# tonyzyl/ladcast

Measured on AMD Instinct MI355X. Metric: ensemble-member-steps/sec, higher is better.
Workload: dtype f32

## Files before the change

### include/ladcast_hip.h

```cpp
#ifndef LADCAST_HIP_H
#define LADCAST_HIP_H

#ifdef __cplusplus
extern "C" {
#endif

#define LDC_ABI_VERSION 5

#define LDC_OK 0
#define LDC_ERR_ARG (-1)
#define LDC_ERR_ALIGN (-2)
#define LDC_ERR_UNSUPPORTED (-3)

enum ldc_act { LDC_ACT_NONE = 0, LDC_ACT_SILU = 1, LDC_ACT_GELU_TANH = 2, LDC_ACT_RELU = 3 };
#define LDC_ACT_IN_TIMESTEP_SINCOS 16

int ldc_abi_version(void);
const char* ldc_build_arch(void);

typedef struct ldc_gemm_desc {
  int M, N, K, batch;
  int lda, ldw, ldc, ldr;
  long long a_bs, c_bs, r_bs;
  int gate_bs;
  int act;
  int flags;
  int reserved;
} ldc_gemm_desc;
#define LDC_GEMM_A_SPLIT 1
#define LDC_GEMM_C_SPLIT 2
#define LDC_GEMM_BF16_1TERM 4
#define LDC_GEMM_F32_REGSTAGE 8
#define LDC_FMT_F32 0
#define LDC_FMT_SPLIT 1
#define LDC_FMT_BF16 2
int ldc_sizeof_gemm_desc(void);
int ldc_gemm_bias_act(const float* A, const float* W, const float* bias, const float* gate,
                      const float* R, float* C, const ldc_gemm_desc* d, void* stream);

#define LDC_GEMM_MAX_PROBLEMS 4
typedef struct ldc_gemm_problem {
  const float* A;
  const float* W;
  const float* bias;
  const float* gate;
  const float* R;
  float* C;
  ldc_gemm_desc d;
} ldc_gemm_problem;
int ldc_sizeof_gemm_problem(void);
long long ldc_gemm_grouped_workspace_bytes(void);
int ldc_gemm_grouped_workspace_init(void* workspace, long long workspace_bytes, void* stream);
int ldc_gemm_grouped(const ldc_gemm_problem* problems, int n, void* workspace, long long workspace_bytes,
                     void* stream);

int ldc_gemm_grouped_bf16x3(const ldc_gemm_problem* problems, int n, void* workspace, long long workspace_bytes,
                            void* stream);
int ldc_pack_weight_bf16x2(const float* W, void* out, int N, int K, int ldw, void* stream);
int ldc_pack_weight_bf16(const float* W, void* out, int N, int K, int ldw, void* stream);

int ldc_linear_small(const float* x, int x_rows, const float* W, const float* bias,
                     const float* add, int add_rows, float* y, int rows, int N, int K,
                     int act_in, int act_out, void* stream);

int ldc_linear_small_mod(const float* x, int x_rows, const float* W, const float* bias, const float* add, int add_rows,
                         const float* mod, int mod_rows, float* y, int rows, int N, int K, int act_in, int act_out,
                         void* stream);

#define LDC_LINEAR_SMALL_MAX_GROUPED 4
typedef struct ldc_linear_small_problem {
  const float* x;
  const float* W;
  const float* bias;
  const float* add;
  float* y;
  int x_rows, add_rows, rows, N, K, act_in, act_out, reserved;
} ldc_linear_small_problem;
int ldc_linear_small_grouped(const ldc_linear_small_problem* problems, int n, void* stream);

int ldc_attn_fwd(const float* Q, const float* K, const float* V, float* O, int B, int S, int H,
                 int ld_qkv, long long qkv_bs, int ldo, long long o_bs, const float* key_bias, void* stream);
long long ldc_attn_fwd_workspace_bytes(void);
int ldc_attn_fwd_ws(const float* Q, const float* K, const float* V, float* O, int B, int S, int H, int ld_qkv, long long qkv_bs,
                    int ldo, long long o_bs, const float* key_bias, void* workspace, long long workspace_bytes, void* stream);
int ldc_attn_fwd_qrows(const float* Q, const float* K, const float* V, float* O, int B, int S, int Sq, int H, int ld_qkv,
                       long long qkv_bs, int ldo, long long o_bs, const float* key_bias, void* stream);
int ldc_attn_fwd_ws_qrows(const float* Q, const float* K, const float* V, float* O, int B, int S, int Sq, int H, int ld_qkv,
                          long long qkv_bs, int ldo, long long o_bs, const float* key_bias, void* workspace, long long workspace_bytes,
                          void* stream);

#define LDC_ATTN_OUT_SPLIT 1
#define LDC_ATTN_BF16_1TERM 2
#define LDC_ATTN_OUT_BF16 4

typedef struct ldc_qkv_epilogue {
  const float* wq;
  const float* wk;
  const float* rope;
  const float* reserved;
  float eps, qscale;
  int heads, rope_row0;
} ldc_qkv_epilogue;
int ldc_sizeof_qkv_epilogue(void);
int ldc_gemm_grouped_bf16x3_qkv(const ldc_gemm_problem* problems, const ldc_qkv_epilogue* epi, int n, void* workspace,
                                long long workspace_bytes, void* stream);
int ldc_gemm_grouped_qkv_f32(const ldc_gemm_problem* problems, const ldc_qkv_epilogue* epi, int n, void* workspace,
                             long long workspace_bytes, void* stream);
int ldc_attn_qkv_prepare_split(float* Q, float* K, float* V, int B, int S, int H, int ld_qkv, long long qkv_bs, int split_row,
                               const float* wq0, const float* wk0, const float* cos0, const float* sin0, const float* wq1,
                               const float* wk1, const float* cos1, const float* sin1, float eps, void* stream);
long long ldc_attn_fwd_split_workspace_bytes(int B, int S, int H);
long long ldc_attn_fwd_split_workspace_max_bytes(void);
int ldc_attn_fwd_split(const float* Q, const float* K, const float* V, float* O, int B, int S, int H, int ld_qkv,
                       long long qkv_bs, int ldo, long long o_bs, const float* key_bias, int flags, void* workspace,
                       long long workspace_bytes, void* stream);
long long ldc_attn_fwd_split_qrows_workspace_bytes(int B, int S, int Sq, int H);
int ldc_attn_fwd_split_qrows(const float* Q, const float* K, const float* V, float* O, int B, int S, int Sq, int H, int ld_qkv,
                             long long qkv_bs, int ldo, long long o_bs, const float* key_bias, int flags, void* workspace,
                             long long workspace_bytes, void* stream);

int ldc_qk_rmsnorm_rope(float* q, float* k, int B, int row0, int rows, int H, int ld, long long bs,
                        const float* wq, const float* wk, float eps, const float* cos_tab,
                        const float* sin_tab, void* stream);

int ldc_layernorm_mod(const float* x, float* y, int B, int rows, int D, int ldx, long long x_bs,
                      int ldy, long long y_bs, const float* scale, const float* shift, int mod_bs,
                      int mode, float eps, int out_split, void* stream);
int ldc_layernorm_mod2(const float* x, float* y, int B, int rows, int D, int ldx, long long x_bs,
                       int ldy, long long y_bs, const float* scale, const float* shift, int split_row,
                       const float* scale2, const float* shift2, int mod_bs, int mode, float eps,
                       int out_split, void* stream);

int ldc_mean_rows(const float* x, float* y, int B, int rows, int D, int ldx, long long x_bs, void* stream);
int ldc_mean_rows_split(const float* x, float* y, float* x_split, int B, int rows, int D, int ldx,
                        long long x_bs, int lds, long long s_bs, int fmt , void* stream);

int ldc_gate_residual(const float* resid, const float* y, const float* gate, float* out, int B,
                      int rows, int D, int ld_res, long long res_bs, int ld_y, long long y_bs,
                      int gate_bs, void* stream);
int ldc_gate_residual_layernorm(float* resid, const float* y, const float* gate, float* out, int B, int rows, int D, int ld_res,
                                long long res_bs, int ld_y, long long y_bs, int gate_bs, int ld_out, long long out_bs,
                                const float* weight, const float* bias, float eps, int out_split, void* stream);

int ldc_chan_to_token(const float* in, float* out, int B, int C, int N, int ldo, int fill_cols, void* stream);
int ldc_chan_to_token_split(const float* in, float* out, int B, int C, int N, int ldo, int fill_cols,
                            int out_split, void* stream);
int ldc_token_to_chan(const float* in, float* out, int B, int C, int N, int ldi, void* stream);

int ldc_timestep_embedding(const float* t, float* out, int n, void* stream);

int ldc_temb_modulate(float* temb, const float* te, int B, int D, int te_rows, void* stream);

int ldc_chan_affine(const float* x, float* y, const float* mean, const float* std_, float target_std,
                    long long outer, int C, long long inner, int inverse, void* stream);

int ldc_edm_scale_f64_to_f32(const double* x, double c_in, float* out, long long n, void* stream);
int ldc_edm_init_state(const float* noise, double sigma0, double* x, long long n, void* stream);
int ldc_edm_churn(const double* x_cur, const double* noise, double coef, double* x_hat, long long n, void* stream);
int ldc_edm_euler(const double* x_hat, const float* F, double c_skip, double c_out, double t_hat,
                  double dt, double* x_next, double* d_cur, long long n, void* stream);
int ldc_edm_heun(const double* x_hat, double* x_next, const float* F, const double* d_cur,
                 double c_skip, double c_out, double t_next, double dt, long long n, void* stream);
int ldc_f64_to_f32(const double* x, float* y, long long n, void* stream);
int ldc_dpm_step(const float* sample, const float* F, const float* m1, float* x0, float* prev,
                 float c_skip, float c_out, float a, float b, float inv_r0, int order, long long n,
                 void* stream);
int ldc_ddim_step(const float* sample, const float* F, const float* noise, float* x0, float* prev, float sqrt_alpha_t,
                  float sqrt_beta_t, float sqrt_alpha_prev, float dir_coef, float std_dev, float clip_range,
                  int prediction_type, int use_clipped_model_output, long long n, void* stream);
int ldc_ddpm_step(const float* sample, const float* F, const float* noise, float* x0, float* prev, float sqrt_alpha_t,
                  float sqrt_beta_t, float x0_coef, float sample_coef, float std_dev, float clip_range, int prediction_type,
                  long long n, void* stream);
int ldc_scale_f32(const float* x, float s, float* y, long long n, void* stream);
int ldc_axpby_f32(const float* x, float a, const float* y, float b, float* out, long long n, void* stream);

int ldc_edm_noise_inputs(const float* clean, const float* noise, const float* sigma, const float* c_in, float* noisy,
                         float* x_in, int B, long long n_per_sample, void* stream);
int ldc_edm_denoise(const float* noisy, const float* F, const float* c_skip, const float* c_out, float* denoised, int B,
                    int C, int T, int plane, int noisy_frames, int f_frames, int denoised_frames, void* stream);
int ldc_edm_denoise_loss(const float* noisy, const float* F, const float* target, const float* c_skip, const float* c_out,
                         const float* weight, const float* lat_weight, float* table, float* denoised, int B, int C, int T,
                         int H, int W, void* stream);

int ldc_sphere_conv_nhwc(const float* X, const float* Wt, const float* bias, const float* R, float* Y, int B,
                         int H, int W, int cin, int ldx, int cout, int ldy, int ldr, int ksize, int act,
                         void* stream);
int ldc_sphere_dwconv_nhwc(const float* x, const float* wt, const float* bias, float* y, int B, int H, int W,
                           int C, int ldx, int ldy, int ksize, int glu, void* stream);
int ldc_grouped_conv1x1_nhwc(const float* x, const float* wt, float* y, long long M, int groups, int ldx, int ldy,
                             void* stream);
int ldc_relu_linear_attn_nhwc(const float* qkv, float* y, int B, int P, int groups, int ldq, int ldy, float eps,
                              void* workspace, long long workspace_bytes, void* stream);
long long ldc_relu_linear_attn_workspace_bytes(int B, int P, int groups);
int ldc_rmsnorm_rows(const float* x, const float* w, const float* b, const float* resid, float* y, long long rows,
                     int C, int ldx, int ldr, int ldy, float eps, int act, void* stream);
int ldc_pixel_unshuffle_shortcut(const float* cv, const float* x, float* y, int B, int H2, int W2, int cout, int cin,
                                 void* stream);
int ldc_pixel_shuffle_shortcut(const float* cv, const float* x, float* y, int B, int H, int W, int cout, int cin,
                               void* stream);
int ldc_chan_regroup(const float* x, float* y, long long M, int cin, int cout, void* stream);

int ldc_sphere_conv_nhwc_split(const float* X, const void* Wp, const float* bias, const float* R, float* Y, int B, int H, int W,
                               int cin, int ldx, int cout, int ldy, int ldr, int ksize, int act, int in_fmt, int out_fmt,
                               void* workspace, long long workspace_bytes, void* stream);
int ldc_sphere_conv_plan(int B, int H, int W, int cin, int cout, int ksize, int in_fmt, int* tile_rows, int* tile_w);
int ldc_rmsnorm_rows_split(const float* x, const float* w, const float* b, const float* resid, float* y, float* ys, long long rows,
                           int C, int ldx, int ldr, int ldy, int lds, int fmt, float eps, int act, void* stream);
int ldc_pixel_unshuffle_shortcut_split(const float* cv, const float* x, float* y, float* ys, int B, int H2, int W2, int cout,
                                       int cin, int lds, int fmt, void* stream);
int ldc_pixel_shuffle_shortcut_split(const float* cv, const float* x, float* y, float* ys, int B, int H, int W, int cout, int cin,
                                     int lds, int fmt, void* stream);
int ldc_upsample_nearest2x_rows(const float* x, float* y, float* ys, int B, int H, int W, int C, int ldx, int ldy, int lds, int fmt, void* stream);
int ldc_pixel_shuffle_to_chan(const float* cv, float* out, int B, int H, int W, int cout, int keep, void* stream);
int ldc_split_rows(const float* x, float* ys, long long rows, int C, int ldx, int lds, int fmt, void* stream);
int ldc_sphere_dwconv_nhwc_fmt(const float* x, const float* wt, const float* bias, float* y, int B, int H, int W, int C, int ldx,
                               int ldy, int ksize, int glu, int out_fmt, void* stream);
int ldc_relu_linear_attn_nhwc_fmt(const float* qkv, float* y, int B, int P, int groups, int ldq, int ldy, float eps, int out_fmt,
                                  void* workspace, long long workspace_bytes, void* stream);

long long ldc_ensemble_scores_workspace_bytes(int C, int H, int W);
int ldc_ensemble_scores(const float* forecast, long long member_stride, long long channel_stride,
                        const float* truth, long long truth_channel_stride, const float* clim,
                        long long clim_channel_stride, const float* lat_weight, int M, int C, int H, int W,
                        int nan_channel, float* out, float* skill_map, float* spread_map, void* workspace,
                        long long workspace_bytes, void* stream);
long long ldc_rollout_scores_workspace_bytes(int C, int L, int H, int W);
int ldc_rollout_scores(const float* forecast, long long member_stride, long long lead_stride, long long channel_stride,
                       const float* mean, const float* std_, float target_std, const float* truth, long long truth_slot_stride,
                       long long truth_channel_stride, const int* truth_slot, const float* clim, long long clim_slot_stride,
                       long long clim_channel_stride, const int* clim_slot, const float* lat_weight, int M, int C, int L, int H,
                       int W, int nan_channel, float* out, int L_total, int l_off, void* workspace, long long workspace_bytes,
                       void* stream);
long long ldc_validation_scores_workspace_bytes(int C, int L, int H, int W);
int ldc_validation_scores(const float* forecast, long long member_stride, long long lead_stride, long long channel_stride,
                          const float* mean, const float* std_, float target_std, const float* truth, long long truth_slot_stride,
                          long long truth_channel_stride, const int* truth_slot, const float* lat_weight, int M, int C, int L, int H,
                          int W, float* out, int L_total, int l_off, void* workspace, long long workspace_bytes, void* stream);
long long ldc_rollout_reliability_workspace_bytes(int M, int C, int L, int H, int W);
int ldc_rollout_reliability(const float* forecast, long long member_stride, long long lead_stride, long long channel_stride,
                            const float* mean, const float* std_, float target_std, const float* truth, long long truth_slot_stride,
                            long long truth_channel_stride, const int* truth_slot, const float* lat_weight, int M, int C, int L, int H,
                            int W, int nan_channel, float* out, int* hist_count, float* hist_weight, int* n_invalid, int L_total,
                            int l_off, void* workspace, long long workspace_bytes, void* stream);
long long ldc_rollout_spectrum_workspace_bytes(int M, int C, int L, int H, int W);
int ldc_rollout_spectrum(const float* forecast, long long member_stride, long long lead_stride, long long channel_stride,
                         const float* mean, const float* std_, float target_std, const float* truth, long long truth_slot_stride,
                         long long truth_channel_stride, const int* truth_slot, const float* row_weight, int M, int C, int L, int H,
                         int W, float* out, int* n_invalid, int L_total, int l_off, void* workspace, long long workspace_bytes,
                         void* stream);
#define LDC_PRODUCTS_MAX_QUANTILES 16
#define LDC_PRODUCTS_MAX_THRESHOLDS 8
typedef struct ldc_products_desc {
  int n_quant;
  int n_thr;
  int q_lo[LDC_PRODUCTS_MAX_QUANTILES];
  float q_t[LDC_PRODUCTS_MAX_QUANTILES];
  int thr_dir[LDC_PRODUCTS_MAX_THRESHOLDS];
} ldc_products_desc;
int ldc_sizeof_products_desc(void);
int ldc_rollout_products(const float* forecast, long long member_stride, long long lead_stride, long long channel_stride,
// ... 54 lines not shown
```

### ladcast_amd/csrc/gemm_bf16x3_v3.hip

```cpp
#include <math.h>
#include <stdio.h>
#include <stdlib.h>

#include "common.h"

namespace {

#include "gemm_v3_common.inc"
#include "gemm_v3_kstep_f32.inc"

struct SKArgs {
  DevProblem pr[MAXP];
  int np;
  int G;
  long long U;
  long long tiles;
  float* ws;
  unsigned* counters;
  unsigned upg, urem;
};

__device__ __forceinline__ long long range_start(long long g, const SKArgs& a) {
  const unsigned gu = static_cast<unsigned>(g);
  return static_cast<long long>(gu * a.upg + (gu < a.urem ? gu : a.urem));
}

__device__ __forceinline__ int find_problem_by_unit(const SKArgs& a, long long u) {
  int pi = 0;
#pragma unroll
  for (int k = 1; k < MAXP; ++k)
    if (k < a.np && u >= a.pr[k].unit0) pi = k;
  return pi;
}

#ifdef LDC_GEMM_STAMPS
#define LDC_STAMP(i)                                                                                        \
  if (threadIdx.x == 0)                                                                                     \
    reinterpret_cast<unsigned long long*>(a.counters)[65536 + blockIdx.x * 16 + (i)] = __builtin_amdgcn_s_memrealtime();
#define LDC_STAMP_CLK(i)                                                                                    \
  if (threadIdx.x == 0)                                                                                     \
    reinterpret_cast<unsigned long long*>(a.counters)[65536 + blockIdx.x * 16 + (i)] = __builtin_amdgcn_s_memtime();
#else
#define LDC_STAMP(i)
#define LDC_STAMP_CLK(i)
#endif

template <int BM, int TERMS, bool CONV = false>
__global__ __launch_bounds__(512) void gemm_bf16x3_v3_kernel(SKArgs a) {
  constexpr int CPK = TERMS == 1 ? 2 * BK : BK;
  constexpr int RT = BM / 128;
  constexpr int NACC = RT * 8;
  constexpr int STAGE_B = (BM + BN) * ROW_B;
  constexpr int SLOT_FLOATS = BM * BN;
  constexpr int NAI = BM / 64;
  constexpr int ND = NAI + 2;
  constexpr int NDH = ND / 2;
  extern __shared__ __attribute__((aligned(16))) unsigned char smem[];
  const int wave = __builtin_amdgcn_readfirstlane(static_cast<int>(threadIdx.x) >> 6);
  LDC_STAMP(0)
  int seg_ = 0;
  (void)seg_;
  int g;
  {
    const int bid = blockIdx.x, G = a.G;
    const int q = G >> 3, r = G & 7, xcd = bid & 7;
    g = (xcd < r ? xcd * (q + 1) : r * (q + 1) + (xcd - r) * q) + (bid >> 3);
  }
  auto uniform64 = [](long long v) {
    const unsigned lo = __builtin_amdgcn_readfirstlane(static_cast<unsigned>(v));
    const unsigned hi = __builtin_amdgcn_readfirstlane(static_cast<unsigned>(static_cast<unsigned long long>(v) >> 32));
    return static_cast<long long>((static_cast<unsigned long long>(hi) << 32) | lo);
  };
  const long long u_begin = uniform64(range_start(g, a));
  const long long u_end = uniform64(range_start(g + 1, a));
  const unsigned smem_lds = lds_addr(smem);

  struct Seg {
    int pi, tile, k0, k1, b, bm, bn;
  };
  auto decode = [&](long long u_) {
    Seg sg;
    sg.pi = find_problem_by_unit(a, u_);
    const DevProblem& Q = a.pr[sg.pi];
    const unsigned local = static_cast<unsigned>(u_ - Q.unit0), kt_u = static_cast<unsigned>(Q.kt);
    sg.tile = __builtin_amdgcn_readfirstlane(static_cast<int>(local / kt_u));
    sg.k0 = static_cast<int>(local - static_cast<unsigned>(sg.tile) * kt_u);
    const long long left = u_end - u_;
    sg.k1 = (Q.kt - sg.k0 <= left) ? Q.kt : sg.k0 + static_cast<int>(left);
    const unsigned per_b = static_cast<unsigned>(Q.tm * Q.tn), tile_u = static_cast<unsigned>(sg.tile);
    const unsigned b_ = tile_u / per_b;
    const unsigned t_in = tile_u - b_ * per_b;
    const unsigned strip = static_cast<unsigned>(Q.rm * Q.tn);
    const unsigned sr = t_in / strip;
    const unsigned r_in = t_in - sr * strip;
    const int rest = Q.tm - static_cast<int>(sr) * Q.rm;
    const unsigned h_sr = static_cast<unsigned>(rest < Q.rm ? rest : Q.rm);
    const unsigned bn_ = r_in / h_sr;
    sg.b = __builtin_amdgcn_readfirstlane(static_cast<int>(b_));
    sg.bn = __builtin_amdgcn_readfirstlane(static_cast<int>(bn_));
    sg.bm = __builtin_amdgcn_readfirstlane(static_cast<int>(sr) * Q.rm + static_cast<int>(r_in - bn_ * h_sr));
    return sg;
  };
  auto prefetch_next = [&](const Seg& sg) __attribute__((always_inline)) {
    const DevProblem& Q = a.pr[sg.pi];
    const int ln = fresh_lane();
    const int lr_ = ln >> 3, lp_ = ln & 7;
    const float* __restrict__ An = Q.A + static_cast<long long>(sg.b) * Q.d.a_bs;
    const long long wrb = static_cast<long long>(Q.d.K) * (TERMS == 1 ? 2 : 4);
    unsigned char* dump = smem + NSTAGE * STAGE_B + wave * 1024;
#pragma unroll
    for (int j = 0; j < 2; ++j) {
      const bool live = sg.k0 + j < sg.k1;
      const long long koff = static_cast<long long>(live ? sg.k0 + j : sg.k1 - 1) * (BK * 4);
      unsigned char* sA = smem + j * STAGE_B;
      unsigned char* sW = sA + BM * ROW_B;
#pragma unroll
      for (int i = 0; i < NAI; ++i) {
        const int r = 8 * (wave + 8 * i) + lr_;
        int gm = sg.bm * BM + r;
        gm = gm < Q.d.M ? gm : Q.d.M - 1;
        dma16(reinterpret_cast<const unsigned char*>(An + static_cast<long long>(gm) * Q.d.lda) + ((lp_ ^ swz(r)) << 4) + koff,
              live ? sA + (wave + 8 * i) * 1024 : dump);
      }
#pragma unroll
      for (int i = 0; i < 2; ++i) {
        const int r = 8 * (wave + 8 * i) + lr_;
        int gn = sg.bn * BN + r;
        gn = gn < Q.d.N ? gn : Q.d.N - 1;
        dma16(Q.W + static_cast<long long>(gn) * wrb + ((lp_ ^ swz(r)) << 4) + koff, live ? sW + (wave + 8 * (i)) * 1024 : dump);
      }
    }
  };
  long long u = u_begin;
  Seg cur{};
  if (u < u_end) cur = decode(u);
  bool prefetched = false;
  while (u < u_end) {
    const int pi = cur.pi;
    const DevProblem& P = a.pr[pi];
    const int tile = cur.tile, k0 = cur.k0, k1 = cur.k1, b = cur.b, bm = cur.bm, bn = cur.bn;
    const int lane = fresh_lane();
    const int fr = lane & 15;
    const int kg = lane >> 4;
    const int lr = lane >> 3, lp = lane & 7;
    const unsigned f_r = swz(fr);
    const unsigned off_hi = fr * ROW_B + (((2 * kg) ^ f_r) << 4);
    const unsigned off_lo = fr * ROW_B + (((2 * kg + 1) ^ f_r) << 4);
    const unsigned a_hi = smem_lds + (16 * RT * wave) * ROW_B + off_hi;
    const unsigned a_lo = smem_lds + (16 * RT * wave) * ROW_B + off_lo;
    const unsigned w_hi = smem_lds + BM * ROW_B + off_hi;
    const unsigned w_lo = smem_lds + BM * ROW_B + off_lo;
    const int M = P.d.M, N = P.d.N, K = P.d.K;
    const bool wave_rows = bm * BM + 16 * RT * wave < M;
    const float* __restrict__ A = P.A + static_cast<long long>(b) * P.d.a_bs;
    const int lda = P.d.lda;
    const long long w_row_bytes = static_cast<long long>(K) * (TERMS == 1 ? 2 : 4);

#ifdef LDC_GEMM_STAMPS_PROLOGUE
    if (seg_ == 0) { LDC_STAMP(9) }
#endif
    const unsigned char* a_src[NAI];
    const unsigned char* w_src[2];
    int pix_b[NAI], pix_hw[NAI];
    const int cslot = lp ^ swz(8 * (wave & 1) + lr);
    auto conv_tap_base = [&](int i, int tap) {
      const int ky = tap / P.ks, kx = tap - ky * P.ks;
      const int src = pix_b[i] + ldc_sphere_src_pixel(pix_hw[i] >> 16, pix_hw[i] & 0xffff, ky, kx, P.cH, P.cW, P.ks);
      return reinterpret_cast<const unsigned char*>(A + static_cast<long long>(src) * lda) + (cslot << 4);
    };
#pragma unroll
    for (int i = 0; i < NAI; ++i) {
      const int r = 8 * (wave + 8 * i) + lr;
      int gm = bm * BM + r;
      gm = gm < M ? gm : M - 1;
      if constexpr (CONV) {
        const int hw = P.cH * P.cW;
        const int bimg = gm / hw;
        const int rem = gm - bimg * hw;
        const int h = rem / P.cW;
        pix_b[i] = bimg * hw;
        pix_hw[i] = (h << 16) | (rem - h * P.cW);
        a_src[i] = conv_tap_base(i, k0 >> P.kshift);
      } else {
        a_src[i] = reinterpret_cast<const unsigned char*>(A + static_cast<long long>(gm) * lda) + ((lp ^ swz(r)) << 4);
      }
    }
#pragma unroll
    for (int i = 0; i < 2; ++i) {
      const int r = 8 * (wave + 8 * i) + lr;
      int gn = bn * BN + r;
      gn = gn < N ? gn : N - 1;
      w_src[i] = P.W + static_cast<long long>(gn) * w_row_bytes + ((lp ^ swz(r)) << 4);
    }
    auto issue_one = [&](int kt_, int stage, int i) {
      const bool live = kt_ < k1;
      unsigned char* sA = smem + stage * STAGE_B;
      unsigned char* sW = sA + BM * ROW_B;
      unsigned char* dump = smem + NSTAGE * STAGE_B + wave * 1024;
      const int kt = live ? kt_ : k1 - 1;
      const long long koff = static_cast<long long>(kt) * (BK * 4);
#ifdef LDC_GEMM_DIAG_NODMA
      if (kt >= 0) return;
#endif
      if (i < NAI) {
        if constexpr (CONV) {
          const int chunk = kt & ((1 << P.kshift) - 1);
          if (chunk == 0) a_src[i] = conv_tap_base(i, kt >> P.kshift);
          const unsigned char* src = a_src[i] + chunk * (BK * 4);
          if (chunk * CPK + CPK > P.cin) {
            if (chunk * CPK + (TERMS == 0 ? 4 * cslot : 8 * (TERMS == 3 ? (cslot >> 1) : cslot)) >= P.cin) src = P.zero16;
          }
          dma16(src, live ? sA + (wave + 8 * i) * 1024 : dump);
        } else {
          dma16(a_src[i] + koff, live ? sA + (wave + 8 * i) * 1024 : dump);
        }
      } else {
        dma16(w_src[i - NAI] + koff, live ? sW + (wave + 8 * (i - NAI)) * 1024 : dump);
      }
    };

    f32x4 acc[NACC];
#pragma unroll
    for (int i = 0; i < NACC; ++i) acc[i] = f32x4{0.f, 0.f, 0.f, 0.f};

    i32x4v wh0, wl0, wh1, wl1, wh2, wl2, wh3, wl3;
    i32x4v ah0[RT], al0[RT], ah1[RT], al1[RT];

#define LDC_SB __builtin_amdgcn_sched_barrier(0)
#define LDC_RD_W(WH, WL, SBH, SBL, CT)                                           \
  {                                                                              \
    LDC_DS_READ(WH, SBH, (CT) * (16 * ROW_B));                                   \
    LDC_DS_READ(WL, SBL, (CT) * (16 * ROW_B));                                   \
  }
#define LDC_RD_A(AH, AL, SBH, SBL)                                               \
  {                                                                              \
    LDC_DS_READ(AH[0], SBH, 0);                                                  \
    LDC_DS_READ(AL[0], SBL, 0);                                                  \
    if constexpr (RT == 2) {                                                     \
      LDC_DS_READ(AH[RT - 1], SBH, 16 * ROW_B);                                  \
      LDC_DS_READ(AL[RT - 1], SBL, 16 * ROW_B);                                  \
    }                                                                            \
  }
#define LDC_MM(ACC, WF, AF)                                                                                  \
  ACC = __builtin_amdgcn_mfma_f32_16x16x32_bf16(__builtin_bit_cast(bf16x8, WF), __builtin_bit_cast(bf16x8, AF), ACC, 0, 0, 0); \
  LDC_SB;
#define LDC_MMF(ACC, WF, AF, J)                                                                               \
  ACC = __builtin_amdgcn_mfma_f32_16x16x4f32(__int_as_float(WF[J]), __int_as_float(AF[J]), ACC, 0, 0, 0);     \
  LDC_SB;
#define LDC_CT(CT, WH, WL, AH, AL)                                               \
  if (wave_rows) {                                                               \
    if constexpr (TERMS == 0) {                                                  \
      _Pragma("unroll") for (int j_ = 0; j_ < 4; ++j_) {                         \
        LDC_MMF(acc[(CT)], WH, AH[0], j_)                                        \
        if constexpr (RT == 2) {                                                 \
          LDC_MMF(acc[8 + (CT)], WH, AH[RT - 1], j_)                             \
        }                                                                        \
      }                                                                          \
      _Pragma("unroll") for (int j_ = 0; j_ < 4; ++j_) {                         \
        LDC_MMF(acc[(CT)], WL, AL[0], j_)                                        \
        if constexpr (RT == 2) {                                                 \
          LDC_MMF(acc[8 + (CT)], WL, AL[RT - 1], j_)                             \
        }                                                                        \
      }                                                                          \
    } else if constexpr (TERMS == 1) {                                           \
      LDC_MM(acc[(CT)], WH, AH[0])                                               \
      if constexpr (RT == 2) {                                                   \
        LDC_MM(acc[8 + (CT)], WH, AH[RT - 1])                                    \
      }                                                                          \
      LDC_MM(acc[(CT)], WL, AL[0])                                               \
      if constexpr (RT == 2) {                                                   \
        LDC_MM(acc[8 + (CT)], WL, AL[RT - 1])                                    \
      }                                                                          \
    } else if constexpr (RT == 2) {                                              \
      LDC_MM(acc[(CT)], WH, AL[0])                                               \
      LDC_MM(acc[8 + (CT)], WH, AL[RT - 1])                                      \
      LDC_MM(acc[(CT)], WL, AH[0])                                               \
      LDC_MM(acc[8 + (CT)], WL, AH[RT - 1])                                      \
      LDC_MM(acc[(CT)], WH, AH[0])                                               \
      LDC_MM(acc[8 + (CT)], WH, AH[RT - 1])                                      \
    } else {                                                                     \
      LDC_MM(acc[(CT)], WH, AL[0])                                               \
      LDC_MM(acc[(CT)], WL, AH[0])                                               \
      LDC_MM(acc[(CT)], WH, AH[0])                                               \
    }                                                                            \
  }
#ifdef LDC_GEMM_DIAG_NOBARRIER
#define LDC_KSTEP_BARRIER
#else
#define LDC_KSTEP_BARRIER __builtin_amdgcn_s_barrier();
#endif
#define LDC_WAIT(N, X, Y)                                                        \
  asm volatile("s_waitcnt lgkmcnt(6)" : "+v"(X), "+v"(Y));                       \
  LDC_SB;
#define LDC_KSTEP(AH, AL, AHN, ALN)                                                                          \
  {                                                                                                          \
    const int st1 = st == NSTAGE - 1 ? 0 : st + 1;                                                           \
    const int st2 = st1 == NSTAGE - 1 ? 0 : st1 + 1;                                                         \
    const unsigned sb1 = st1 * STAGE_B;                                                                      \
    const unsigned wch = w_hi + sb, wcl = w_lo + sb, wnh = w_hi + sb1, wnl = w_lo + sb1;                     \
    const unsigned anh = a_hi + sb1, anl = a_lo + sb1;                                                       \
    constexpr bool dma2 = true;              \
    constexpr bool dma3 = true;  \
        \
    if constexpr (RT == 2) {                                                                                 \
      asm volatile("s_waitcnt lgkmcnt(6)" : "+v"(AH[0]), "+v"(AL[0]), "+v"(AH[1]), "+v"(AL[1]), "+v"(wh0), "+v"(wl0)); \
    } else {                                                                                                 \
      asm volatile("s_waitcnt lgkmcnt(6)" : "+v"(AH[0]), "+v"(AL[0]), "+v"(wh0), "+v"(wl0));                 \
    }                                                                                                        \
    LDC_SB;                                                                                                  \
    LDC_CT(0, wh0, wl0, AH, AL)                                                                              \
    LDC_RD_W(wh0, wl0, wch, wcl, 4)                                                                                \
    if (dma2) issue_one(kt + 2, st2, NDH + 0);                                                               \
    LDC_WAIT(6, wh1, wl1)                                                                                    \
    LDC_CT(1, wh1, wl1, AH, AL)                                                                              \
    LDC_RD_W(wh1, wl1, wch, wcl, 5)                                                                                \
    if (dma2) issue_one(kt + 2, st2, NDH + 1);                                                               \
    LDC_WAIT(6, wh2, wl2)                                                                                    \
    LDC_CT(2, wh2, wl2, AH, AL)                                                                              \
    LDC_RD_W(wh2, wl2, wch, wcl, 6)                                                                                \
    if constexpr (NDH == 3) {                                                                                \
      if (dma2) issue_one(kt + 2, st2, NDH + 2);                                                             \
    }                                                                                                        \
    LDC_WAIT(6, wh3, wl3)                                                                                    \
    LDC_CT(3, wh3, wl3, AH, AL)                                                                              \
    LDC_RD_W(wh3, wl3, wch, wcl, 7)                                                                          \
    LDC_WAIT(6, wh0, wl0)                                                                                    \
    LDC_CT(4, wh0, wl0, AH, AL)                                                                              \
                                                                         \
    asm volatile("s_waitcnt lgkmcnt(0)" : "+v"(wh1), "+v"(wl1), "+v"(wh2), "+v"(wl2), "+v"(wh3), "+v"(wl3)); \
    if constexpr (ND == 6) {                                                                                 \
      asm volatile("s_waitcnt vmcnt(6)" ::: "memory");                                                       \
    } else {                                                                                                 \
      asm volatile("s_waitcnt vmcnt(4)" ::: "memory");                                                       \
    }                                                                                                        \
    LDC_KSTEP_BARRIER                                                                                        \
    LDC_SB;                                                                                                  \
                          \
    LDC_RD_A(AHN, ALN, anh, anl)                                                                             \
    LDC_RD_W(wh0, wl0, wnh, wnl, 0)                                                                          \
    if (dma3) issue_one(kt + 3, st, 0);                                                                      \
    LDC_SB;                                                                                                  \
    LDC_CT(5, wh1, wl1, AH, AL)                                                                              \
    LDC_RD_W(wh1, wl1, wnh, wnl, 1)                                                                               \
    if (dma3) issue_one(kt + 3, st, 1);                                                                      \
    LDC_SB;                                                                                                  \
    LDC_CT(6, wh2, wl2, AH, AL)                                                                              \
    LDC_RD_W(wh2, wl2, wnh, wnl, 2)                                                                               \
    if constexpr (NDH == 3) {                                                                                \
      if (dma3) issue_one(kt + 3, st, 2);                                                                    \
    }                                                                                                        \
    LDC_SB;                                                                                                  \
    LDC_CT(7, wh3, wl3, AH, AL)                                                                              \
    LDC_RD_W(wh3, wl3, wnh, wnl, 3)                                                                               \
    LDC_SB;                                                                                                  \
    st = st1;                                                                                                \
    sb = sb1;                                                                                                \
  }

#define LDC_MM_ON(ACC, WF, AF, J) LDC_MMF(ACC, WF, AF, J)
#define LDC_MM_OFF(ACC, WF, AF, J)
#if defined(LDC_AB_BUILD) && defined(LDC_GEMM_F32_NO_PAIRS)
  constexpr bool PAIRED = false;
#else
  constexpr bool PAIRED = TERMS == 0 && RT == 1;
#endif

#ifdef LDC_GEMM_STAMPS_PROLOGUE
    if (seg_ == 0) { LDC_STAMP(10) }
#endif
    if (!prefetched) {
#pragma unroll
      for (int i = 0; i < ND; ++i) issue_one(k0, 0, i);
#pragma unroll
      for (int i = 0; i < ND; ++i) issue_one(k0 + 1, 1, i);
    }
#ifdef LDC_GEMM_STAMPS_PROLOGUE
    if (seg_ == 0) { LDC_STAMP(11) }
#endif
    const long long u_next = u + (k1 - k0);
    Seg nxt = cur;
    if (u_next < u_end) nxt = decode(u_next);
    if constexpr (ND == 6) {
      asm volatile("s_waitcnt vmcnt(6)" ::: "memory");
    } else {
      asm volatile("s_waitcnt vmcnt(4)" ::: "memory");
    }
    __builtin_amdgcn_s_barrier();
    LDC_STAMP(1 + 4 * seg_)
    if (seg_ == 0) { LDC_STAMP_CLK(13) }
    if constexpr (PAIRED) {
      LDC_KSTEP_Q_PROLOGUE(ah0, al0)
    } else {
      LDC_RD_A(ah0, al0, a_hi, a_lo)
      LDC_RD_W(wh0, wl0, w_hi, w_lo, 0)
      LDC_RD_W(wh1, wl1, w_hi, w_lo, 1)
      LDC_RD_W(wh2, wl2, w_hi, w_lo, 2)
      LDC_RD_W(wh3, wl3, w_hi, w_lo, 3)
    }
#pragma unroll
    for (int i = 0; i < NDH; ++i) issue_one(k0 + 2, 2, i);
    LDC_SB;

    unsigned sb = 0;
    int st = 0;
    if constexpr (PAIRED) {
      static_assert(!PAIRED || ND == 4, "the interleaved k-step is written for the 128-row tile's 4 DMA pieces");
      if (wave_rows) {
        for (int kt = k0; kt < k1; ++kt) {
          LDC_KSTEP_Q(ah0, al0, ah1, al1, LDC_MM_ON)
          ++kt;
          if (kt >= k1) break;
          LDC_KSTEP_Q(ah1, al1, ah0, al0, LDC_MM_ON)
        }
      } else {
        for (int kt = k0; kt < k1; ++kt) {
          LDC_KSTEP_Q(ah0, al0, ah1, al1, LDC_MM_OFF)
          ++kt;
          if (kt >= k1) break;
          LDC_KSTEP_Q(ah1, al1, ah0, al0, LDC_MM_OFF)
        }
      }
    } else {
      for (int kt = k0; kt < k1; ++kt) {
        LDC_KSTEP(ah0, al0, ah1, al1)
        ++kt;
        if (kt >= k1) break;
        LDC_KSTEP(ah1, al1, ah0, al0)
      }
    }
    asm volatile("s_waitcnt lgkmcnt(0)" : "+v"(wh0), "+v"(wl0), "+v"(wh1), "+v"(wl1), "+v"(wh2), "+v"(wl2), "+v"(wh3), "+v"(wl3));
#pragma unroll
    for (int rt = 0; rt < RT; ++rt) asm volatile("" : "+v"(ah0[rt]), "+v"(al0[rt]), "+v"(ah1[rt]), "+v"(al1[rt]));
#undef LDC_KSTEP
#undef LDC_MM_ON
#undef LDC_MM_OFF
#undef LDC_WAIT
#undef LDC_CT
#undef LDC_MMF
#undef LDC_MM
#undef LDC_RD_A
#undef LDC_RD_W
#undef LDC_SB
    __builtin_amdgcn_s_barrier();
    prefetched = false;
    if constexpr (!CONV && TERMS == 0) {
#if !defined(LDC_GEMM_DIAG_NODMA) && !defined(LDC_GEMM_NO_PREFETCH)
      if (u_next < u_end) {
        prefetch_next(nxt);
        prefetched = true;
      }
#endif
    }
    if (seg_ == 0) { LDC_STAMP_CLK(14) }
    LDC_STAMP(2 + 4 * seg_)

    if (k0 == 0 && k1 == P.kt) {
      tile_epilogue<BM, !CONV, LinearRows<BM>, true, TERMS == 0>(P, b, bm, bn, acc, wave, lane);
    } else {
      const int lane_h = fresh_lane();
      float* slot = a.ws + (static_cast<long long>(2 * g) + (k0 > 0 ? 0 : 1)) * SLOT_FLOATS + lane_h;
#pragma unroll
      for (int i = 0; i < NACC; ++i)
#pragma unroll
        for (int r = 0; r < 4; ++r)
          __hip_atomic_store(slot + ((wave * NACC + i) * 4 + r) * 64, acc[i][r], __ATOMIC_RELAXED, __HIP_MEMORY_SCOPE_AGENT);
      asm volatile("s_waitcnt vmcnt(0)" ::: "memory");
      __builtin_amdgcn_s_barrier();
      const long long f = P.unit0 + static_cast<long long>(tile) * P.kt;
      const long long l = f + P.kt;
      long long g_first = g;
      while (g_first > 0 && range_start(g_first, a) > f) --g_first;
      long long g_last = g;
      while (g_last + 1 < a.G && range_start(g_last + 1, a) < l) ++g_last;
      const unsigned pieces = static_cast<unsigned>(g_last - g_first + 1);
      unsigned* cnt = a.counters + (P.tile0 + tile);
      unsigned* flag = reinterpret_cast<unsigned*>(smem + NSTAGE * STAGE_B);
      if (wave == 0 && lane_h == 0) {
        const unsigned ticket = __hip_atomic_fetch_add(cnt, 1u, __ATOMIC_RELAXED, __HIP_MEMORY_SCOPE_AGENT);
        const unsigned last = (ticket == pieces - 1) ? 1u : 0u;
        if (last) {
          __builtin_amdgcn_fence(__ATOMIC_ACQUIRE, "agent");
          asm volatile("s_waitcnt vmcnt(0)" ::: "memory");
          __hip_atomic_store(cnt, 0u, __ATOMIC_RELAXED, __HIP_MEMORY_SCOPE_AGENT);
        }
        *flag = last;
      }
      __syncthreads();
      LDC_STAMP(3 + 4 * seg_)
      const unsigned is_last = *flag;
      __syncthreads();
      if (is_last) {
#pragma unroll
        for (int i = 0; i < NACC; ++i) acc[i] = f32x4{0.f, 0.f, 0.f, 0.f};
        for (long long gp = g_first; gp <= g_last; ++gp) {
          const long long s = range_start(gp, a);
          const float* sl = a.ws + (2 * gp + (s > f ? 0 : 1)) * SLOT_FLOATS;
#pragma unroll
          for (int i = 0; i < NACC; ++i) {
#pragma unroll
            for (int r = 0; r < 4; ++r) acc[i][r] += sl[((wave * NACC + i) * 4 + r) * 64 + lane_h];
          }
        }
        tile_epilogue<BM, !CONV, LinearRows<BM>, true, TERMS == 0>(P, b, bm, bn, acc, wave, lane);
      }
    }
    u = u_next;
    cur = nxt;
    LDC_STAMP(4 + 4 * seg_)
#ifdef LDC_GEMM_STAMPS
    if (seg_ < 2) ++seg_;
#endif
  }
  LDC_STAMP(15)
}

struct ConvParams {
  int H, W, cin, ks, kshift;
};

constexpr int LDC_SPLIT_GROUP = -100;

template <int BM, int TERMS, bool CONV = false>
int launch_v3(const ldc_gemm_problem* problems, const ldc_qkv_epilogue* epi, int n, void* workspace, long long workspace_bytes,
              void* stream, const ConvParams* cp = nullptr, bool may_split_group = false) {
  constexpr int SLOT_FLOATS = BM * BN;
  constexpr int STAGE_B = (BM + BN) * ROW_B;
  constexpr int CUS = 256;
  SKArgs a{};
  a.np = n;
  long long U = 0, tiles = 0;
  for (int i = 0; i < n; ++i) {
    const ldc_gemm_problem& q = problems[i];
    LDC_CHECK_PTR(q.A);
    LDC_CHECK_PTR(q.W);
    LDC_CHECK_PTR(q.C);
    const ldc_gemm_desc& d = q.d;
    if (d.M <= 0 || d.N <= 0 || d.K <= 0 || d.batch <= 0) return LDC_ERR_ARG;
    if (d.K % (TERMS == 1 ? 2 * BK : BK)) return LDC_ERR_UNSUPPORTED;
    if constexpr (TERMS == 0) {
      if (d.flags != 0 || d.ldw != d.K) return LDC_ERR_UNSUPPORTED;
    } else {
      if (!(d.flags & LDC_GEMM_A_SPLIT)) return LDC_ERR_UNSUPPORTED;
    }
    LDC_CHECK_ALIGN16(q.A);
    LDC_CHECK_ALIGN16(q.W);
    if constexpr (TERMS == 0) {
      if ((d.lda & 3) || (d.a_bs & 3)) return LDC_ERR_UNSUPPORTED;
    } else {
      if ((d.lda & 7) || (d.a_bs & 7) || (reinterpret_cast<unsigned long long>(q.A) & 31ull)) return LDC_ERR_ALIGN;
    }
    if (d.act < LDC_ACT_NONE || d.act > LDC_ACT_RELU) return LDC_ERR_UNSUPPORTED;
    DevProblem& P = a.pr[i];
    P.A = q.A;
    P.W = reinterpret_cast<const unsigned char*>(q.W);
    P.bias = q.bias;
    P.gate = q.gate;
    P.R = q.R;
    P.C = q.C;
    P.d = d;
    {
      auto al16 = [](const void* q_) { return (reinterpret_cast<unsigned long long>(q_) & 15ull) == 0; };
      bool v4 = (d.N % 4 == 0) && (d.ldc % 4 == 0) && (d.c_bs % 4 == 0) && al16(q.C);
      if (q.bias) v4 = v4 && al16(q.bias);
      if (q.gate) v4 = v4 && al16(q.gate) && (d.gate_bs % 4 == 0);
      if (q.R) v4 = v4 && al16(q.R) && (d.ldr % 4 == 0) && (d.r_bs % 4 == 0);
      P.vec4 = v4 ? 1 : 0;
      P.c_split = (TERMS != 0 && (d.flags & LDC_GEMM_C_SPLIT)) ? (TERMS == 3 ? LDC_FMT_SPLIT : LDC_FMT_BF16) : 0;
      if (P.c_split && !(v4 && d.ldc % 8 == 0 && d.ldc >= ((d.N + 7) & ~7) &&
                         d.c_bs % 8 == 0 && (reinterpret_cast<unsigned long long>(q.C) & 31ull) == 0))
        return LDC_ERR_ALIGN;
    }
    if (epi != nullptr && epi[i].heads > 0) {
      const ldc_qkv_epilogue& e = epi[i];
      auto al16 = [](const void* q_) { return (reinterpret_cast<unsigned long long>(q_) & 15ull) == 0; };
      if (d.N != 3 * e.heads * BN || d.act != LDC_ACT_NONE || q.gate != nullptr || q.R != nullptr) return LDC_ERR_ARG;
      if ((e.wq == nullptr) != (e.wk == nullptr) || e.reserved != nullptr || e.rope_row0 < 0) return LDC_ERR_ARG;
      if constexpr (TERMS == 0) {
        if ((d.ldc & 3) || (d.c_bs & 3) || !al16(q.C)) return LDC_ERR_ALIGN;
      } else {
        if ((d.ldc & 7) || (d.c_bs & 7) || (reinterpret_cast<unsigned long long>(q.C) & 31ull)) return LDC_ERR_ALIGN;
      }
      if (!al16(e.wq) || !al16(e.wk) || !al16(e.rope) || (q.bias && !al16(q.bias))) return LDC_ERR_ALIGN;
      P.qkv_heads = e.heads;
      P.rope_row0 = e.rope_row0;
      P.qk_w[0] = e.wq;
      P.qk_w[1] = e.wk;
      P.rope_cs = e.rope;
      P.eps = e.eps;
      P.qscale = e.qscale != 0.f ? e.qscale : 0.08838834764831845f * 1.4426950408889634f;
    }
    if constexpr (CONV) {
      P.cH = cp->H; P.cW = cp->W; P.cin = cp->cin; P.ks = cp->ks; P.kshift = cp->kshift;
      P.zero16 = static_cast<const unsigned char*>(workspace) + LDC_GEMM_COUNTER_BYTES - 64;
    }
    P.tm = ldc_cdiv(d.M, BM);
    P.tn = ldc_cdiv(d.N, BN);
    P.kt = d.K / (TERMS == 1 ? 2 * BK : BK);
    P.unit0 = U;
    P.tile0 = tiles;
    {
      P.rm = P.tm;
      const double a_bytes = CONV ? static_cast<double>(d.M) * d.lda * 4.0 : static_cast<double>(d.batch) * d.M * d.K * 4.0;
      if (a_bytes >= 48e6) {
        const double t8 = static_cast<double>(d.batch) * P.tm * P.tn / 8.0;
        const double want = sqrt(t8 * BN / BM);
        int nsr = static_cast<int>(P.tm / (want > 1.0 ? want : 1.0) + 0.5);
        if (nsr < 1) nsr = 1;
        if (nsr > P.tm) nsr = P.tm;
        P.rm = ldc_cdiv(P.tm, nsr);
      }
      if (const char* e = LDC_AB_GETENV("LDC_BF16X3_RM")) {
        const int f = atoi(e);
        if (f >= 0) P.rm = (f == 0 || f > P.tm) ? P.tm : f;
      }
    }
    const long long t = static_cast<long long>(d.batch) * P.tm * P.tn;
    tiles += t;
    U += t * P.kt;
  }
  if (tiles > LDC_GEMM_COUNTER_BYTES / 4 - 16) return LDC_ERR_UNSUPPORTED;
  const long long slot_bytes = SLOT_FLOATS * static_cast<long long>(sizeof(float));
  long long G = CUS;
  {
    bool same_kt = true;
    for (int i = 1; i < n; ++i) same_kt = same_kt && (a.pr[i].kt == a.pr[0].kt);
    long long best = 0;
    if (same_kt) {
      const int kt = a.pr[0].kt;
      double best_score = 0.0;
      for (int sfac = 1; sfac <= 8; ++sfac) {
        if (kt % sfac || (sfac > 1 && kt / sfac < 8)) continue;
        const long long items = tiles * sfac;
        long long gd = items < CUS ? items : CUS;
        while (gd > 1 && items % gd) --gd;
        const double score = static_cast<double>(gd) * (1.0 - 0.02 * (sfac - 1));
        if (score > best_score) {
          best_score = score;
          best = gd;
        }
      }
    }
    long long few = 0;
    if (same_kt && best < 160) {
      const int kt = a.pr[0].kt;
      for (int sfac = 8; sfac >= 2; --sfac)
        if (kt % sfac == 0 && kt / sfac >= 8 && tiles * sfac <= CUS) {
          few = tiles * sfac;
          break;
        }
    }
    if (may_split_group && TERMS != 0 && n > 1 && best < 160 && few == 0) return LDC_SPLIT_GROUP;
    if (best >= 160) {
      G = best;
    } else if (few > 0) {
      G = few;
    } else {
      const double kt_avg = static_cast<double>(U) / static_cast<double>(tiles);
      long long umin = static_cast<long long>(sqrt(kt_avg * 8.0) + 0.5);
      if (umin < 1) umin = 1;
      const long long gmax = U / umin > 0 ? U / umin : 1;
      if (gmax < G) G = gmax;
    }
  }
  if constexpr (TERMS == 0) {
    if (U >= 4 * CUS) G = CUS;
  }
  static const char* const force_g = LDC_AB_GETENV("LDC_BF16X3_G");
  if (force_g) {
    const long long g_ = atoll(force_g);
    if (g_ > 0 && g_ <= CUS) G = g_;
  }
  if (U < G) G = U;
  if (workspace == nullptr) return LDC_ERR_ARG;
  if (workspace_bytes < LDC_GEMM_COUNTER_BYTES + 2 * slot_bytes) return LDC_ERR_ARG;
  {
    const long long fit = (workspace_bytes - LDC_GEMM_COUNTER_BYTES) / (2 * slot_bytes);
    if (fit < G) G = fit;
  }
  LDC_CHECK_ALIGN16(workspace);
  if (U >= (1LL << 31)) return LDC_ERR_UNSUPPORTED;
#ifdef LDC_AB_BUILD
  {
    static const bool dbg = getenv("LDC_GEMM_DEBUG_G") != nullptr;
    if (dbg)
      fprintf(stderr, "ldc_gemm cut: terms %d conv %d n %d tiles %lld kt0 %d BM %d G %lld U %lld %s\n", TERMS, int(CONV), n, tiles, a.pr[0].kt, BM, G, U,
              (U % G == 0 && (U / G) % a.pr[0].kt == 0) ? "whole tiles" : (U % G == 0 ? "equal ranges" : "UNALIGNED"));
  }
#endif
  a.G = static_cast<int>(G);
  a.U = U;
  a.upg = static_cast<unsigned>(U / G);
  a.urem = static_cast<unsigned>(U % G);
  a.tiles = tiles;
  a.ws = reinterpret_cast<float*>(static_cast<unsigned char*>(workspace) + LDC_GEMM_COUNTER_BYTES);
  a.counters = static_cast<unsigned*>(workspace);
  const size_t lds = NSTAGE * STAGE_B + 8 * 1024;
  static const bool attr_set = [&] {
    (void)hipFuncSetAttribute(reinterpret_cast<const void*>(gemm_bf16x3_v3_kernel<BM, TERMS, CONV>),
                              hipFuncAttributeMaxDynamicSharedMemorySize, static_cast<int>(lds));
    return true;
  }();
  (void)attr_set;
  hipLaunchKernelGGL((gemm_bf16x3_v3_kernel<BM, TERMS, CONV>), dim3(a.G), dim3(512), lds, static_cast<hipStream_t>(stream), a);
  return ldc_launch_status();
}

}

static int gemm_v3_dispatch(const ldc_gemm_problem* problems, const ldc_qkv_epilogue* epi, int n, void* workspace,
                            long long workspace_bytes, void* stream) {
  LDC_CHECK_PTR(problems);
  if (n <= 0 || n > MAXP) return LDC_ERR_ARG;
  long long tiles256 = 0;
  for (int i = 0; i < n; ++i) {
    const ldc_gemm_desc& d = problems[i].d;
    if (d.M <= 0 || d.N <= 0 || d.batch <= 0) return LDC_ERR_ARG;
    if (!(d.flags & LDC_GEMM_A_SPLIT)) return LDC_ERR_UNSUPPORTED;
    if (((d.flags ^ problems[0].d.flags) & LDC_GEMM_BF16_1TERM) != 0) return LDC_ERR_ARG;
    tiles256 += static_cast<long long>(d.batch) * ldc_cdiv(d.M, 256) * ldc_cdiv(d.N, BN);
  }
  static const char* const force_thr = LDC_AB_GETENV("LDC_BF16X3_SMALL_TILES");
  bool small = tiles256 < (force_thr ? atoll(force_thr) : 400);
  static const char* const force_bm = LDC_AB_GETENV("LDC_BF16X3_BM");
  if (force_bm) small = (atoi(force_bm) == 128);
  const bool one = (problems[0].d.flags & LDC_GEMM_BF16_1TERM) != 0;
  auto launch = [&](const ldc_gemm_problem* pr, const ldc_qkv_epilogue* ep, int cnt, bool sm, bool may_split) {
    if (one)
      return sm ? launch_v3<128, 1>(pr, ep, cnt, workspace, workspace_bytes, stream, nullptr, may_split)
                : launch_v3<256, 1>(pr, ep, cnt, workspace, workspace_bytes, stream, nullptr, may_split);
    return sm ? launch_v3<128, 3>(pr, ep, cnt, workspace, workspace_bytes, stream, nullptr, may_split)
              : launch_v3<256, 3>(pr, ep, cnt, workspace, workspace_bytes, stream, nullptr, may_split);
  };
  const int st = launch(problems, epi, n, small, true);
  if (st != LDC_SPLIT_GROUP) return st;
  for (int i = 0; i < n; ++i) {
    const ldc_gemm_desc& d = problems[i].d;
    bool sm = static_cast<long long>(d.batch) * ldc_cdiv(d.M, 256) * ldc_cdiv(d.N, BN) < (force_thr ? atoll(force_thr) : 400);
    if (force_bm) sm = (atoi(force_bm) == 128);
    const int sti = launch(problems + i, epi ? epi + i : nullptr, 1, sm, false);
    if (sti != LDC_OK) return sti;
  }
  return LDC_OK;
}

static int gemm_f32_ring(const ldc_gemm_problem* problems, const ldc_qkv_epilogue* epi, int n, void* workspace, long long workspace_bytes,
                         void* stream) {
  LDC_CHECK_PTR(problems);
  if (n <= 0 || n > MAXP) return LDC_ERR_ARG;
  for (int i = 0; i < n; ++i)
    if (problems[i].d.flags & LDC_GEMM_F32_REGSTAGE) return LDC_ERR_UNSUPPORTED;
  auto al16 = [](const void* q_) { return q_ != nullptr && (reinterpret_cast<unsigned long long>(q_) & 15ull) == 0; };
  if (!al16(workspace) || workspace_bytes < LDC_GEMM_COUNTER_BYTES + 2ll * 256 * BN * static_cast<long long>(sizeof(float)))
    return LDC_ERR_UNSUPPORTED;
  for (int i = 0; i < n; ++i) {
    const ldc_gemm_desc& d = problems[i].d;
    if (d.M <= 0 || d.N <= 0 || d.K <= 0 || d.batch <= 0) return LDC_ERR_ARG;
    if (!al16(problems[i].A) || !al16(problems[i].W)) return LDC_ERR_UNSUPPORTED;
  }
#ifdef LDC_AB_BUILD
  static const char* const force_bm = getenv("LDC_F32_RING_BM");
  if (force_bm && atoi(force_bm) == 256) return launch_v3<256, 0>(problems, epi, n, workspace, workspace_bytes, stream);
#endif
  return launch_v3<128, 0>(problems, epi, n, workspace, workspace_bytes, stream);
}

int ldc_gemm_grouped_f32_ring(const ldc_gemm_problem* problems, int n, void* workspace, long long workspace_bytes, void* stream) {
  return gemm_f32_ring(problems, nullptr, n, workspace, workspace_bytes, stream);
}

extern "C" int ldc_gemm_grouped_qkv_f32(const ldc_gemm_problem* problems, const ldc_qkv_epilogue* epi, int n, void* workspace,
                                        long long workspace_bytes, void* stream) {
  LDC_CHECK_PTR(epi);
  return gemm_f32_ring(problems, epi, n, workspace, workspace_bytes, stream);
}

int ldc_gemm_grouped_bf16x3_v3(const ldc_gemm_problem* problems, int n, void* workspace, long long workspace_bytes,
                               void* stream) {
  return gemm_v3_dispatch(problems, nullptr, n, workspace, workspace_bytes, stream);
}

extern "C" int ldc_gemm_grouped_bf16x3_qkv(const ldc_gemm_problem* problems, const ldc_qkv_epilogue* epi, int n, void* workspace,
                                           long long workspace_bytes, void* stream) {
  LDC_CHECK_PTR(epi);
  return gemm_v3_dispatch(problems, epi, n, workspace, workspace_bytes, stream);
}

extern "C" int ldc_sphere_conv_nhwc_split(const float* X, const void* Wp, const float* bias, const float* R, float* Y, int B, int H,
                                          int W, int cin, int ldx, int cout, int ldy, int ldr, int ksize, int act, int in_fmt,
                                          int out_fmt, void* workspace, long long workspace_bytes, void* stream) {
  LDC_CHECK_PTR(X);
  LDC_CHECK_PTR(Wp);
  LDC_CHECK_PTR(Y);
  if (B <= 0 || H <= 0 || W <= 0 || cin <= 0 || cout <= 0) return LDC_ERR_ARG;
  if (ksize != 1 && ksize != 3 && ksize != 5) return LDC_ERR_UNSUPPORTED;
  if (ksize > 1 && ((W & 1) || H < 2 || H < ksize / 2 || W / 2 < ksize / 2 || H > 32767 || W > 65535)) return LDC_ERR_UNSUPPORTED;
  if (in_fmt != LDC_FMT_SPLIT && in_fmt != LDC_FMT_BF16 && in_fmt != LDC_FMT_F32) return LDC_ERR_UNSUPPORTED;
  if (out_fmt != LDC_FMT_F32 && out_fmt != in_fmt) return LDC_ERR_UNSUPPORTED;
  if (in_fmt == LDC_FMT_F32) {
    if ((ldx & 3) || (cin & 3) || ldx < cin || ldy < cout) return LDC_ERR_ALIGN;
  } else if ((ldx & 7) || ldx < ((cin + 7) & ~7) || ldy < cout) {
    return LDC_ERR_ALIGN;
  }
  const long long M = static_cast<long long>(B) * H * W;
  if (M > 0x7fffffffLL) return LDC_ERR_UNSUPPORTED;
  const bool one = in_fmt == LDC_FMT_BF16;
  const int cpk = one ? 2 * BK : BK;
  ConvParams cp{H, W, cin, ksize, 0};
  int ktpt = ldc_cdiv(cin, cpk);
  while ((1 << cp.kshift) < ktpt) ++cp.kshift;
  ktpt = 1 << cp.kshift;
  ldc_gemm_problem q{};
  q.A = X;
  q.W = static_cast<const float*>(Wp);
  q.bias = bias;
  q.R = R;
  q.C = Y;
  q.d.M = static_cast<int>(M);
  q.d.N = cout;
  q.d.K = ksize * ksize * ktpt * cpk;
  q.d.batch = 1;
  q.d.lda = ldx;
  q.d.ldw = q.d.K;
  q.d.ldc = ldy;
  q.d.ldr = ldr;
  q.d.act = act;
  q.d.flags = LDC_GEMM_A_SPLIT | (out_fmt != LDC_FMT_F32 ? LDC_GEMM_C_SPLIT : 0) | (one ? LDC_GEMM_BF16_1TERM : 0);
  if (in_fmt == LDC_FMT_F32) {
    q.d.flags = 0;
    return launch_v3<128, 0, true>(&q, nullptr, 1, workspace, workspace_bytes, stream, &cp);
  }
  if (ksize == 3) {
    static const char* const halo_sw = LDC_AB_GETENV("LDC_CONV_HALO");
    if (!(halo_sw && atoi(halo_sw) == 0)) {
      if (workspace == nullptr || workspace_bytes < LDC_GEMM_COUNTER_BYTES) return LDC_ERR_ARG;
      const int hs = ldc_conv_halo_dispatch(X, Wp, bias, R, Y, B, H, W, cin, ldx, cout, ldy, ldr, act, in_fmt, out_fmt, workspace, workspace_bytes, stream);
      if (hs != LDC_ERR_UNSUPPORTED) return hs;
    }
  }
  const long long tiles256 = static_cast<long long>(ldc_cdiv(M, 256)) * ldc_cdiv(cout, BN);
  static const char* const force_thr = LDC_AB_GETENV("LDC_CONV_SMALL_TILES");
  const bool small = tiles256 < (force_thr ? atoll(force_thr) : 200);
  if (one)
    return small ? launch_v3<128, 1, true>(&q, nullptr, 1, workspace, workspace_bytes, stream, &cp)
                 : launch_v3<256, 1, true>(&q, nullptr, 1, workspace, workspace_bytes, stream, &cp);
  return small ? launch_v3<128, 3, true>(&q, nullptr, 1, workspace, workspace_bytes, stream, &cp)
               : launch_v3<256, 3, true>(&q, nullptr, 1, workspace, workspace_bytes, stream, &cp);
}
```

### ladcast_amd/csrc/gemm_streamk.hip

```cpp
#include <math.h>
#include <stdlib.h>
#include <string.h>

#include "common.h"

namespace {

constexpr int BM = 128, BN = 128, BK = 32;
constexpr int LDP = 36;
constexpr int STAGE_FLOATS = (BM + BN) * LDP;
constexpr int SLOT_FLOATS = BM * BN;
constexpr int MAXP = LDC_GEMM_MAX_PROBLEMS;

struct DevProblem {
  const float* A;
  const float* W;
  const float* bias;
  const float* gate;
  const float* R;
  float* C;
  ldc_gemm_desc d;
  int tm, tn, kt;
  long long unit0;
  long long tile0;
// ... 273 lines not shown

    const int srow0 = tid >> 2, srow1 = srow0 + 64, skc = tid & 3;
    const bool am0 = bm * BM + srow0 < M, am1 = bm * BM + srow1 < M;
    const bool wn0 = bn * BN + srow0 < N, wn1 = bn * BN + srow1 < N;
    const float* a_src0 = A + static_cast<long long>(am0 ? bm * BM + srow0 : 0) * lda + skc * 8;
    const float* a_src1 = A + static_cast<long long>(am1 ? bm * BM + srow1 : 0) * lda + skc * 8;
    const uint4* w_src0 = Wp + (static_cast<long long>(wn0 ? bn * BN + srow0 : 0) * kchunks + skc) * 2;
    const uint4* w_src1 = Wp + (static_cast<long long>(wn1 ? bn * BN + srow1 : 0) * kchunks + skc) * 2;
    float4 ra00, ra01, ra10, ra11;
    uint4 rw00, rw01, rw10, rw11;
    auto gload = [&](int kt) {
      const bool kin = kt * BK + skc * 8 < K;
      const int ko = kin ? kt * BK : 0;
      const float4* pa0 = reinterpret_cast<const float4*>(a_src0 + ko);
      const float4* pa1 = reinterpret_cast<const float4*>(a_src1 + ko);
      const uint4* pw0 = w_src0 + (ko >> 3) * 2;
      const uint4* pw1 = w_src1 + (ko >> 3) * 2;
      ra00 = pa0[0];
      ra01 = pa0[1];
      ra10 = pa1[0];
      ra11 = pa1[1];
      rw00 = pw0[0];
      rw01 = pw0[1];
      rw10 = pw1[0];
      rw11 = pw1[1];
      const unsigned m0a = (kin && am0) ? 0xffffffffu : 0u, m1a = (kin && am1) ? 0xffffffffu : 0u;
      const unsigned m0w = (kin && wn0) ? 0xffffffffu : 0u, m1w = (kin && wn1) ? 0xffffffffu : 0u;
#define LDC_MASKF4(v, m)                                 \
  v.x = __uint_as_float(__float_as_uint(v.x) & (m));     \
  v.y = __uint_as_float(__float_as_uint(v.y) & (m));     \
  v.z = __uint_as_float(__float_as_uint(v.z) & (m));     \
  v.w = __uint_as_float(__float_as_uint(v.w) & (m));
#define LDC_MASKU4(v, m) \
  v.x &= (m);            \
  v.y &= (m);            \
  v.z &= (m);            \
  v.w &= (m);
      LDC_MASKF4(ra00, m0a) LDC_MASKF4(ra01, m0a) LDC_MASKF4(ra10, m1a) LDC_MASKF4(ra11, m1a)
      LDC_MASKU4(rw00, m0w) LDC_MASKU4(rw01, m0w) LDC_MASKU4(rw10, m1w) LDC_MASKU4(rw11, m1w)
    };
    auto sstore = [&](int stage) {
      unsigned char* As = smem_b + stage * STAGE_BYTES_B;
      unsigned char* Bs = As + BM * PITCH_B;
      uint4 h, l;
      split8(ra00, ra01, h, l);
      *reinterpret_cast<uint4*>(As + srow0 * PITCH_B + skc * 16) = h;
      *reinterpret_cast<uint4*>(As + srow0 * PITCH_B + 64 + skc * 16) = l;
      split8(ra10, ra11, h, l);
      *reinterpret_cast<uint4*>(As + srow1 * PITCH_B + skc * 16) = h;
      *reinterpret_cast<uint4*>(As + srow1 * PITCH_B + 64 + skc * 16) = l;
      *reinterpret_cast<uint4*>(Bs + srow0 * PITCH_B + skc * 16) = rw00;
      *reinterpret_cast<uint4*>(Bs + srow0 * PITCH_B + 64 + skc * 16) = rw01;
      *reinterpret_cast<uint4*>(Bs + srow1 * PITCH_B + skc * 16) = rw10;
      *reinterpret_cast<uint4*>(Bs + srow1 * PITCH_B + 64 + skc * 16) = rw11;
    };

    f32x16 acc[2][2];
#pragma unroll
    for (int i = 0; i < 2; ++i)
#pragma unroll
      for (int j = 0; j < 2; ++j)
#pragma unroll
        for (int r = 0; r < 16; ++r) acc[i][j][r] = 0.f;

    gload(k0);
    sstore(0);
    __syncthreads();
    for (int kt = k0; kt < k1; ++kt) {
      const int st = (kt - k0) & 1;
      if (kt + 1 < k1) gload(kt + 1);
      const unsigned char* As = smem_b + st * STAGE_BYTES_B;
      const unsigned char* Bs = As + BM * PITCH_B;
      const unsigned char* a_base = As + (wm * 64 + frag_row) * PITCH_B + frag_h * 16;
      const unsigned char* b_base = Bs + (wn * 64 + frag_row) * PITCH_B + frag_h * 16;
#pragma unroll
      for (int s2 = 0; s2 < 2; ++s2) {
        const bf16x8 ah0 = *reinterpret_cast<const bf16x8*>(a_base + s2 * 32);
        const bf16x8 al0 = *reinterpret_cast<const bf16x8*>(a_base + 64 + s2 * 32);
        const bf16x8 ah1 = *reinterpret_cast<const bf16x8*>(a_base + 32 * PITCH_B + s2 * 32);
        const bf16x8 al1 = *reinterpret_cast<const bf16x8*>(a_base + 32 * PITCH_B + 64 + s2 * 32);
        const bf16x8 wh0 = *reinterpret_cast<const bf16x8*>(b_base + s2 * 32);
        const bf16x8 wl0 = *reinterpret_cast<const bf16x8*>(b_base + 64 + s2 * 32);
        const bf16x8 wh1 = *reinterpret_cast<const bf16x8*>(b_base + 32 * PITCH_B + s2 * 32);
        const bf16x8 wl1 = *reinterpret_cast<const bf16x8*>(b_base + 32 * PITCH_B + 64 + s2 * 32);
#define LDC_MFMA3(ACC, AH, AL, WH, WL)                                        \
  ACC = __builtin_amdgcn_mfma_f32_32x32x16_bf16(AL, WH, ACC, 0, 0, 0);        \
  ACC = __builtin_amdgcn_mfma_f32_32x32x16_bf16(AH, WL, ACC, 0, 0, 0);        \
  ACC = __builtin_amdgcn_mfma_f32_32x32x16_bf16(AH, WH, ACC, 0, 0, 0);
        LDC_MFMA3(acc[0][0], ah0, al0, wh0, wl0)
        LDC_MFMA3(acc[0][1], ah0, al0, wh1, wl1)
        LDC_MFMA3(acc[1][0], ah1, al1, wh0, wl0)
        LDC_MFMA3(acc[1][1], ah1, al1, wh1, wl1)
      }
      if (kt + 1 < k1) sstore(st ^ 1);
      __syncthreads();
    }

    if (k0 == 0 && k1 == P.kt) {
      tile_epilogue(P, b, bm, bn, acc, wm, wn, lane);
    } else {
      publish_or_reduce(a, P, g, tile, k0, b, bm, bn, acc, wave, wm, wn, lane, reinterpret_cast<unsigned*>(smem_b));
    }
    u += k1 - k0;
  }
}

__global__ __launch_bounds__(256) void pack_weight_bf16x2_kernel(const float* __restrict__ W, uint4* __restrict__ out,
                                                                 int N, int K, int ldw) {
  const long long idx = static_cast<long long>(blockIdx.x) * 256 + threadIdx.x;
  const int kchunks = K >> 3;
  if (idx >= static_cast<long long>(N) * kchunks) return;
  const int n = static_cast<int>(idx / kchunks), kc = static_cast<int>(idx - static_cast<long long>(n) * kchunks);
  const float4* src = reinterpret_cast<const float4*>(W + static_cast<long long>(n) * ldw + kc * 8);
  uint4 h, l;
  split8(src[0], src[1], h, l);
  out[idx * 2] = h;
  out[idx * 2 + 1] = l;
}

}

extern "C" int ldc_sizeof_gemm_problem(void) { return static_cast<int>(sizeof(ldc_gemm_problem)); }

extern "C" long long ldc_gemm_grouped_workspace_bytes(void) {
  return LDC_GEMM_COUNTER_BYTES + 2LL * 512 * SLOT_FLOATS * static_cast<long long>(sizeof(float));
}

extern "C" int ldc_gemm_grouped_workspace_init(void* workspace, long long workspace_bytes, void* stream) {
  LDC_CHECK_PTR(workspace);
  if (workspace_bytes < LDC_GEMM_COUNTER_BYTES) return LDC_ERR_ARG;
  hipError_t e = hipMemsetAsync(workspace, 0, LDC_GEMM_COUNTER_BYTES, static_cast<hipStream_t>(stream));
  return e == hipSuccess ? LDC_OK : -(1000 + static_cast<int>(e));
}

static int gemm_grouped_impl(const ldc_gemm_problem* problems, int n, void* workspace, long long workspace_bytes,
                             void* stream, bool split_bf16) {
  LDC_CHECK_PTR(problems);
  if (n <= 0 || n > MAXP) return LDC_ERR_ARG;
  SKArgs a{};
  a.np = n;
  long long U = 0, tiles = 0;
  for (int i = 0; i < n; ++i) {
    const ldc_gemm_problem& q = problems[i];
    LDC_CHECK_PTR(q.A);
    LDC_CHECK_PTR(q.W);
    LDC_CHECK_PTR(q.C);
    const ldc_gemm_desc& d = q.d;
    if (d.M <= 0 || d.N <= 0 || d.K <= 0 || d.batch <= 0) return LDC_ERR_ARG;
    LDC_CHECK_ALIGN16(q.A);
    LDC_CHECK_ALIGN16(q.W);
    if ((d.K & 3) || (d.lda & 3) || (d.a_bs & 3)) return LDC_ERR_ALIGN;
    if (split_bf16 ? (d.K & 7) != 0 : (d.ldw & 3) != 0) return LDC_ERR_ALIGN;
    if (d.act < LDC_ACT_NONE || d.act > LDC_ACT_RELU) return LDC_ERR_UNSUPPORTED;
    if ((d.flags & ~LDC_GEMM_F32_REGSTAGE) != 0) return LDC_ERR_UNSUPPORTED;
    DevProblem& P = a.pr[i];
    P.A = q.A;
    P.W = q.W;
    P.bias = q.bias;
    P.gate = q.gate;
    P.R = q.R;
    P.C = q.C;
    P.d = d;
    P.tm = ldc_cdiv(d.M, BM);
    P.tn = ldc_cdiv(d.N, BN);
    P.kt = ldc_cdiv(d.K, BK);
    P.unit0 = U;
    P.tile0 = tiles;
    const long long t = static_cast<long long>(d.batch) * P.tm * P.tn;
    tiles += t;
    U += t * P.kt;
  }
  if (tiles > LDC_GEMM_COUNTER_BYTES / 4 - 16) return LDC_ERR_UNSUPPORTED;
  const long long slot_bytes = SLOT_FLOATS * static_cast<long long>(sizeof(float));
  long long G = 512;
  {
    const double kt_avg = static_cast<double>(U) / static_cast<double>(tiles);
    long long umin = static_cast<long long>(sqrt(kt_avg * (split_bf16 ? 7.0 : 2.0)) + 0.5);
    if (umin < 1) umin = 1;
    const long long gmax = U / umin > 0 ? U / umin : 1;
    if (gmax < G) G = gmax;
  }
  if (U < G) G = U;
  if (workspace == nullptr || workspace_bytes < LDC_GEMM_COUNTER_BYTES + 2 * slot_bytes) return LDC_ERR_ARG;
  {
    const long long fit = (workspace_bytes - LDC_GEMM_COUNTER_BYTES) / (2 * slot_bytes);
    if (fit < G) G = fit;
  }
  LDC_CHECK_ALIGN16(workspace);
  a.G = static_cast<int>(G);
  a.U = U;
  a.tiles = tiles;
  a.ws = reinterpret_cast<float*>(static_cast<unsigned char*>(workspace) + LDC_GEMM_COUNTER_BYTES);
  a.counters = static_cast<unsigned*>(workspace);
  const size_t lds = split_bf16 ? 2 * STAGE_BYTES_B : 2 * STAGE_FLOATS * sizeof(float);
  static const bool attr_set = [&] {
    (void)hipFuncSetAttribute(reinterpret_cast<const void*>(gemm_streamk_kernel),
                              hipFuncAttributeMaxDynamicSharedMemorySize, static_cast<int>(2 * STAGE_FLOATS * sizeof(float)));
    (void)hipFuncSetAttribute(reinterpret_cast<const void*>(gemm_streamk_bf16x3_kernel),
                              hipFuncAttributeMaxDynamicSharedMemorySize, 2 * STAGE_BYTES_B);
    return true;
  }();
  (void)attr_set;
  hipStream_t s = static_cast<hipStream_t>(stream);
  if (split_bf16) hipLaunchKernelGGL(gemm_streamk_bf16x3_kernel, dim3(a.G), dim3(256), lds, s, a);
  else hipLaunchKernelGGL(gemm_streamk_kernel, dim3(a.G), dim3(256), lds, s, a);
  return ldc_launch_status();
}

int ldc_gemm_grouped_f32_ring(const ldc_gemm_problem* problems, int n, void* workspace, long long workspace_bytes,
                              void* stream);

extern "C" int ldc_gemm_grouped(const ldc_gemm_problem* problems, int n, void* workspace, long long workspace_bytes,
                                void* stream) {
  const int st = ldc_gemm_grouped_f32_ring(problems, n, workspace, workspace_bytes, stream);
  if (st != LDC_ERR_UNSUPPORTED) return st;
  return gemm_grouped_impl(problems, n, workspace, workspace_bytes, stream, false);
}

int ldc_gemm_grouped_bf16x3_v3(const ldc_gemm_problem* problems, int n, void* workspace, long long workspace_bytes,
                               void* stream);

extern "C" int ldc_gemm_grouped_bf16x3(const ldc_gemm_problem* problems, int n, void* workspace,
                                       long long workspace_bytes, void* stream) {
  int force = 0;
#ifdef LDC_AB_BUILD
  static const int force_env = [] {
    const char* e = getenv("LDC_BF16X3_KERNEL");
    return (e != nullptr && strcmp(e, "regstage") == 0) ? 1 : 0;
  }();
  force = force_env;
#endif
  if (force == 0) {
    const int st = ldc_gemm_grouped_bf16x3_v3(problems, n, workspace, workspace_bytes, stream);
    if (st != LDC_ERR_UNSUPPORTED) return st;
  }
  return gemm_grouped_impl(problems, n, workspace, workspace_bytes, stream, true);
}

namespace {
__global__ __launch_bounds__(256) void pack_weight_bf16_kernel(const float* __restrict__ W, uint2* __restrict__ out, long long N, int K4, int ldw) {
  const long long idx = static_cast<long long>(blockIdx.x) * 256 + threadIdx.x;
  if (idx >= N * K4) return;
  const long long n = idx / K4;
  const int c = static_cast<int>(idx - n * K4);
  const float4 v = reinterpret_cast<const float4*>(W + n * ldw)[c];
  out[idx] = make_uint2(ldc_pack_pair(v.x, v.y), ldc_pack_pair(v.z, v.w));
}
}

extern "C" int ldc_pack_weight_bf16(const float* W, void* out, int N, int K, int ldw, void* stream) {
  LDC_CHECK_PTR(W);
  LDC_CHECK_PTR(out);
  if (N <= 0 || K <= 0) return LDC_ERR_ARG;
  if ((K & 7) || (ldw & 3)) return LDC_ERR_ALIGN;
  LDC_CHECK_ALIGN16(W);
  LDC_CHECK_ALIGN16(out);
  const long long total = static_cast<long long>(N) * (K >> 2);
  hipLaunchKernelGGL(pack_weight_bf16_kernel, dim3(ldc_cdiv(total, 256)), dim3(256), 0, static_cast<hipStream_t>(stream), W,
                     static_cast<uint2*>(out), static_cast<long long>(N), K >> 2, ldw);
  return ldc_launch_status();
}

extern "C" int ldc_pack_weight_bf16x2(const float* W, void* out, int N, int K, int ldw, void* stream) {
  LDC_CHECK_PTR(W);
  LDC_CHECK_PTR(out);
  if (N <= 0 || K <= 0) return LDC_ERR_ARG;
  if ((K & 7) || (ldw & 3)) return LDC_ERR_ALIGN;
  LDC_CHECK_ALIGN16(W);
  LDC_CHECK_ALIGN16(out);
  const long long total = static_cast<long long>(N) * (K >> 3);
  hipLaunchKernelGGL(pack_weight_bf16x2_kernel, dim3(ldc_cdiv(total, 256)), dim3(256), 0, static_cast<hipStream_t>(stream),
                     W, static_cast<uint4*>(out), N, K, ldw);
  return ldc_launch_status();
}
```

### ladcast_amd/csrc/gemm_v3_common.inc

```
constexpr int BN = 128, BK = 32;
constexpr int ROW_B = 128;
constexpr int NSTAGE = 3;
constexpr int MAXP = LDC_GEMM_MAX_PROBLEMS;

typedef __bf16 bf16x8 __attribute__((ext_vector_type(8)));
typedef float f32x4 __attribute__((ext_vector_type(4)));
typedef int i32x4v __attribute__((ext_vector_type(4)));

template <int BM>
struct LinearRows {
  __device__ __forceinline__ int operator()(int bm, int r) const { return bm * BM + r; }
};

struct DevProblem {
  const float* A;
  const unsigned char* W;
  const float* bias;
  const float* gate;
  const float* R;
  float* C;
  ldc_gemm_desc d;
  int tm, tn, kt;
  int rm;
  long long unit0;
  long long tile0;
  int vec4;
  int c_split;
  int qkv_heads;
  int rope_row0;
  const float* qk_w[2];
  const float* rope_cs;
  float eps, qscale;
  int cH, cW, cin, ks, kshift;
  const unsigned char* zero16;
};


#ifdef LDC_GEMM_DIAG_NOLDS
#define LDC_DS_READ(dst, addr, off) asm volatile("; no read %0 %1" : "=v"(dst) : "v"(addr))
#else
#define LDC_DS_READ(dst, addr, off) asm volatile("ds_read_b128 %0, %1 offset:%2" : "=v"(dst) : "v"(addr), "n"(off))
#endif

__device__ __forceinline__ unsigned lds_addr(const void* p) {
  return static_cast<unsigned>(reinterpret_cast<unsigned long long>(p));
}
__device__ __forceinline__ void dma16(const void* gsrc, unsigned char* lds_dst_wave_base) {
  __builtin_amdgcn_global_load_lds((const __attribute__((address_space(1))) void*)gsrc,
                                   (__attribute__((address_space(3))) void*)lds_dst_wave_base, 16, 0, 0);
}
__device__ __forceinline__ int swz(int r) { return ((r >> 1) & 7) ^ ((((r >> 2) ^ (r >> 3)) & 1) << 1); }

__device__ __forceinline__ float xor16_add(float x) {
  const auto r = __builtin_amdgcn_permlane16_swap(__float_as_uint(x), __float_as_uint(x), false, false);
  return __uint_as_float(r[0]) + __uint_as_float(r[1]);
}
__device__ __forceinline__ float xor32_add(float x) {
  const auto r = __builtin_amdgcn_permlane32_swap(__float_as_uint(x), __float_as_uint(x), false, false);
  return __uint_as_float(r[0]) + __uint_as_float(r[1]);
}

__device__ __forceinline__ int fresh_lane() {
  int l;
  asm volatile("v_mbcnt_lo_u32_b32 %0, -1, 0\n\tv_mbcnt_hi_u32_b32 %0, -1, %0" : "=v"(l));
  return l;
}

template <int BM, bool F32OUT = false>
__device__ __forceinline__ void qkv_epilogue(const DevProblem& P, int b, int bm, int bn, const f32x4 (&acc)[BM / 16], int wave,
                                             int lane) {
  constexpr int RT = BM / 128;
  lane = fresh_lane();
  const int M = P.d.M;
  float* __restrict__ C = P.C + static_cast<long long>(b) * P.d.c_bs;
  const int which = bn / P.qkv_heads;
  const int nl = 4 * (lane >> 4);
  const float* __restrict__ w = which < 2 ? P.qk_w[which] : nullptr;
  const float* __restrict__ rope = which < 2 ? P.rope_cs : nullptr;
  float4 bv[8], wv[8];
  if (P.bias) {
#pragma unroll
    for (int ct = 0; ct < 8; ++ct) bv[ct] = *reinterpret_cast<const float4*>(P.bias + bn * BN + nl + 16 * ct);
  } else {
#pragma unroll
    for (int ct = 0; ct < 8; ++ct) bv[ct] = make_float4(0.f, 0.f, 0.f, 0.f);
  }
  if (w) {
#pragma unroll
    for (int ct = 0; ct < 8; ++ct) wv[ct] = *reinterpret_cast<const float4*>(w + 16 * ct + nl);
  } else {
#pragma unroll
    for (int ct = 0; ct < 8; ++ct) wv[ct] = make_float4(1.f, 1.f, 1.f, 1.f);
  }
  const float qs = which == 0 ? P.qscale : 1.f;
#pragma unroll
  for (int rt = 0; rt < RT; ++rt) {
    const int m = bm * BM + 16 * (RT * wave + rt) + (lane & 15);
#ifndef LDC_QKV_EPI_HOIST
    asm volatile("" ::: "memory");
#endif
    if (m >= M) continue;
    float4 tv[8];
    if (rope) {
      const float* __restrict__ cs = rope + static_cast<long long>(P.rope_row0 + m) * 128 + nl;
#pragma unroll
      for (int ct = 0; ct < 8; ++ct) tv[ct] = *reinterpret_cast<const float4*>(cs + 16 * ct);
    }
    float r = 1.f;
    if (w) {
      float ss = 0.f;
#pragma unroll
      for (int ct = 0; ct < 8; ++ct) {
        const f32x4 av = acc[rt * 8 + ct];
        const float a0 = av[0] + bv[ct].x, a1 = av[1] + bv[ct].y, a2 = av[2] + bv[ct].z, a3 = av[3] + bv[ct].w;
        ss += a0 * a0 + a1 * a1 + a2 * a2 + a3 * a3;
      }
      ss = xor32_add(xor16_add(ss));
      r = rsqrtf(ss * (1.0f / 128.0f) + P.eps);
    }
    unsigned char* row = reinterpret_cast<unsigned char*>(C + static_cast<long long>(m) * P.d.ldc + bn * BN);
#pragma unroll
    for (int ct = 0; ct < 8; ++ct) {
      const f32x4 av = acc[rt * 8 + ct];
      float x0 = av[0] + bv[ct].x, x1 = av[1] + bv[ct].y, x2 = av[2] + bv[ct].z, x3 = av[3] + bv[ct].w;
      if (w) {
        x0 = x0 * r * wv[ct].x; x1 = x1 * r * wv[ct].y; x2 = x2 * r * wv[ct].z; x3 = x3 * r * wv[ct].w;
      }
      if (rope) {
        const float4 t = tv[ct];
        const float o0 = x0 * t.x + (-x1) * t.y, o1 = x1 * t.x + x0 * t.y;
        const float o2 = x2 * t.z + (-x3) * t.w, o3 = x3 * t.z + x2 * t.w;
        x0 = o0; x1 = o1; x2 = o2; x3 = o3;
      }
      if (which == 0) { x0 *= qs; x1 *= qs; x2 *= qs; x3 *= qs; }
      const int n = 16 * ct + nl;
      if constexpr (F32OUT) {
        *reinterpret_cast<float4*>(reinterpret_cast<float*>(row) + n) = make_float4(x0, x1, x2, x3);
        continue;
      }
      float r0, r1, r2, r3;
      const unsigned hx = ldc_split_pair(x0, x1, r0, r1), hy = ldc_split_pair(x2, x3, r2, r3);
      const unsigned lx = ldc_pack_pair(r0, r1), ly = ldc_pack_pair(r2, r3);
      const auto sx = __builtin_amdgcn_permlane16_swap(hx, lx, false, false);
      const auto sy = __builtin_amdgcn_permlane16_swap(hy, ly, false, false);
      unsigned char* dst = which < 2 ? row + 4 * (n & ~7) + 4 * (n & 4)
                                     : row + 2 * (n & ~7) + ((n & 4) ? 256 : 0);
      *reinterpret_cast<uint4*>(dst) = make_uint4(sx[0], sy[0], sx[1], sy[1]);
    }
  }
}

template <int BM, int ACT, int FMT, class RM, bool GATE>
__device__ __forceinline__ void tile_epilogue_fast(const DevProblem& P, int b, int bm, int bn, const f32x4 (&acc)[BM / 16], int wave,
                                                   int lane, const RM& rowmap) {
  constexpr int RT = BM / 128;
  lane = fresh_lane();
  const int M = P.d.M;
  float* __restrict__ C = P.C + static_cast<long long>(b) * P.d.c_bs;
  const float* __restrict__ R = P.R ? P.R + static_cast<long long>(b) * P.d.r_bs : nullptr;
  const float* __restrict__ gate = P.gate ? P.gate + static_cast<long long>(b) * P.d.gate_bs : nullptr;
  const int n0 = bn * BN + 4 * (lane >> 4);
  float4 bv[8], gv[8];
  if (P.bias) {
#pragma unroll
    for (int ct = 0; ct < 8; ++ct) bv[ct] = *reinterpret_cast<const float4*>(P.bias + n0 + 16 * ct);
  } else {
#pragma unroll
    for (int ct = 0; ct < 8; ++ct) bv[ct] = make_float4(0.f, 0.f, 0.f, 0.f);
  }
  const bool mod = (GATE && gate != nullptr) || R != nullptr;
  if constexpr (GATE) {
    if (gate) {
#pragma unroll
      for (int ct = 0; ct < 8; ++ct) gv[ct] = *reinterpret_cast<const float4*>(gate + n0 + 16 * ct);
    } else {
#pragma unroll
// ... 151 lines not shown
```

### ladcast_amd/csrc/gemm_v3_kstep_f32.inc

```
#define LDC_KSTEP_Q(AH, AL, AHN, ALN, MM) \
  { \
    const int st1 = st == NSTAGE - 1 ? 0 : st + 1; \
    const int st2 = st1 == NSTAGE - 1 ? 0 : st1 + 1; \
    (void)st2; \
    const unsigned sb1 = st1 * STAGE_B; \
    const unsigned wch = w_hi + sb, wcl = w_lo + sb, wnh = w_hi + sb1, wnl = w_lo + sb1; \
    const unsigned anh = a_hi + sb1, anl = a_lo + sb1; \
    asm volatile("s_waitcnt lgkmcnt(2)" : "+v"(AH[0]), "+v"(AL[0]), "+v"(wh0), "+v"(wl0), "+v"(wh1), "+v"(wl1)); \
    LDC_SB; \
    MM(acc[0], wh0, AH[0], 0) \
    LDC_DS_READ(wl2, wcl, 2 * (16 * ROW_B)); \
    LDC_SB; \
    MM(acc[1], wh1, AH[0], 0) \
    MM(acc[0], wh0, AH[0], 1) \
    LDC_DS_READ(wl3, wcl, 3 * (16 * ROW_B)); \
    LDC_SB; \
    MM(acc[1], wh1, AH[0], 1) \
    MM(acc[0], wh0, AH[0], 2) \
    MM(acc[1], wh1, AH[0], 2) \
    MM(acc[0], wh0, AH[0], 3) \
    MM(acc[1], wh1, AH[0], 3) \
    MM(acc[0], wl0, AL[0], 0) \
    LDC_DS_READ(wh0, wch, 4 * (16 * ROW_B)); \
    LDC_SB; \
    MM(acc[1], wl1, AL[0], 0) \
    MM(acc[0], wl0, AL[0], 1) \
    LDC_DS_READ(wh1, wch, 5 * (16 * ROW_B)); \
    LDC_SB; \
    MM(acc[1], wl1, AL[0], 1) \
    MM(acc[0], wl0, AL[0], 2) \
    issue_one(kt + 2, st2, NDH + 0); \
    LDC_SB; \
    MM(acc[1], wl1, AL[0], 2) \
    MM(acc[0], wl0, AL[0], 3) \
    issue_one(kt + 2, st2, NDH + 1); \
    LDC_SB; \
    MM(acc[1], wl1, AL[0], 3) \
    asm volatile("s_waitcnt lgkmcnt(2)" : "+v"(wh2), "+v"(wh3), "+v"(wl2), "+v"(wl3)); \
    LDC_SB; \
    MM(acc[2], wh2, AH[0], 0) \
    LDC_DS_READ(wl0, wcl, 4 * (16 * ROW_B)); \
    LDC_SB; \
    MM(acc[3], wh3, AH[0], 0) \
    MM(acc[2], wh2, AH[0], 1) \
    LDC_DS_READ(wl1, wcl, 5 * (16 * ROW_B)); \
    LDC_SB; \
    MM(acc[3], wh3, AH[0], 1) \
    MM(acc[2], wh2, AH[0], 2) \
    MM(acc[3], wh3, AH[0], 2) \
    MM(acc[2], wh2, AH[0], 3) \
    MM(acc[3], wh3, AH[0], 3) \
    MM(acc[2], wl2, AL[0], 0) \
    LDC_DS_READ(wh2, wch, 6 * (16 * ROW_B)); \
    LDC_SB; \
    MM(acc[3], wl3, AL[0], 0) \
    MM(acc[2], wl2, AL[0], 1) \
    LDC_DS_READ(wh3, wch, 7 * (16 * ROW_B)); \
    LDC_SB; \
    MM(acc[3], wl3, AL[0], 1) \
    MM(acc[2], wl2, AL[0], 2) \
    MM(acc[3], wl3, AL[0], 2) \
    MM(acc[2], wl2, AL[0], 3) \
    MM(acc[3], wl3, AL[0], 3) \
    asm volatile("s_waitcnt lgkmcnt(2)" : "+v"(wh0), "+v"(wh1), "+v"(wl0), "+v"(wl1)); \
    LDC_SB; \
    MM(acc[4], wh0, AH[0], 0) \
    LDC_DS_READ(wl2, wcl, 6 * (16 * ROW_B)); \
    LDC_SB; \
    MM(acc[5], wh1, AH[0], 0) \
    MM(acc[4], wh0, AH[0], 1) \
    LDC_DS_READ(wl3, wcl, 7 * (16 * ROW_B)); \
    LDC_SB; \
    MM(acc[5], wh1, AH[0], 1) \
    MM(acc[4], wh0, AH[0], 2) \
    MM(acc[5], wh1, AH[0], 2) \
    MM(acc[4], wh0, AH[0], 3) \
    MM(acc[5], wh1, AH[0], 3) \
    MM(acc[4], wl0, AL[0], 0) \
    MM(acc[5], wl1, AL[0], 0) \
    MM(acc[4], wl0, AL[0], 1) \
    MM(acc[5], wl1, AL[0], 1) \
    MM(acc[4], wl0, AL[0], 2) \
    MM(acc[5], wl1, AL[0], 2) \
    MM(acc[4], wl0, AL[0], 3) \
    MM(acc[5], wl1, AL[0], 3) \
     \
    asm volatile("s_waitcnt lgkmcnt(0)" : "+v"(wh2), "+v"(wh3), "+v"(wl2), "+v"(wl3)); \
    asm volatile("s_waitcnt vmcnt(4)" ::: "memory"); \
    LDC_KSTEP_BARRIER \
    LDC_SB; \
    MM(acc[6], wh2, AH[0], 0) \
    LDC_DS_READ(AHN[0], anh, 0 * (16 * ROW_B)); \
    LDC_SB; \
    MM(acc[7], wh3, AH[0], 0) \
    LDC_DS_READ(ALN[0], anl, 0 * (16 * ROW_B)); \
    LDC_SB; \
    MM(acc[6], wh2, AH[0], 1) \
    LDC_DS_READ(wh0, wnh, 0 * (16 * ROW_B)); \
    LDC_SB; \
    MM(acc[7], wh3, AH[0], 1) \
    LDC_DS_READ(wl0, wnl, 0 * (16 * ROW_B)); \
    LDC_SB; \
    MM(acc[6], wh2, AH[0], 2) \
    LDC_DS_READ(wh1, wnh, 1 * (16 * ROW_B)); \
    LDC_SB; \
    MM(acc[7], wh3, AH[0], 2) \
    LDC_DS_READ(wl1, wnl, 1 * (16 * ROW_B)); \
    LDC_SB; \
    MM(acc[6], wh2, AH[0], 3) \
    issue_one(kt + 3, st, 0); \
    LDC_SB; \
    MM(acc[7], wh3, AH[0], 3) \
    issue_one(kt + 3, st, 1); \
    LDC_SB; \
    MM(acc[6], wl2, AL[0], 0) \
    LDC_DS_READ(wh2, wnh, 2 * (16 * ROW_B)); \
    LDC_SB; \
    MM(acc[7], wl3, AL[0], 0) \
    MM(acc[6], wl2, AL[0], 1) \
    LDC_DS_READ(wh3, wnh, 3 * (16 * ROW_B)); \
    LDC_SB; \
    MM(acc[7], wl3, AL[0], 1) \
    MM(acc[6], wl2, AL[0], 2) \
    MM(acc[7], wl3, AL[0], 2) \
    MM(acc[6], wl2, AL[0], 3) \
    MM(acc[7], wl3, AL[0], 3) \
    st = st1; \
    sb = sb1; \
  }
#define LDC_KSTEP_Q_PROLOGUE(AH, AL) \
  { \
    LDC_DS_READ(AH[0], a_hi, 0 * (16 * ROW_B)); \
    LDC_DS_READ(AL[0], a_lo, 0 * (16 * ROW_B)); \
    LDC_DS_READ(wh0, w_hi, 0 * (16 * ROW_B)); \
    LDC_DS_READ(wl0, w_lo, 0 * (16 * ROW_B)); \
    LDC_DS_READ(wh1, w_hi, 1 * (16 * ROW_B)); \
    LDC_DS_READ(wl1, w_lo, 1 * (16 * ROW_B)); \
    LDC_DS_READ(wh2, w_hi, 2 * (16 * ROW_B)); \
    LDC_DS_READ(wh3, w_hi, 3 * (16 * ROW_B)); \
  }
```

### ladcast_amd/hip.py

```python
from __future__ import annotations

import ctypes
import os
from ctypes import POINTER, Structure, c_char_p, c_double, c_float, c_int, c_longlong, c_void_p

import torch

_HERE = os.path.dirname(os.path.abspath(__file__))
LIB_PATH = os.environ.get("LDC_LIB_PATH") or os.path.join(_HERE, "libladcast_hip.so")

ACT_NONE, ACT_SILU, ACT_GELU_TANH, ACT_RELU = 0, 1, 2, 3
ACT_IN_TIMESTEP_SINCOS = 16
GEMM_A_SPLIT, GEMM_C_SPLIT, GEMM_BF16_1TERM = 1, 2, 4
GEMM_F32_REGSTAGE = 8
ATTN_OUT_SPLIT, ATTN_BF16_1TERM, ATTN_OUT_BF16 = 1, 2, 4
ABI_VERSION = 5
FMT_F32, FMT_SPLIT, FMT_BF16 = 0, 1, 2


class GemmDesc(Structure):
    _fields_ = [
        ("M", c_int), ("N", c_int), ("K", c_int), ("batch", c_int),
        ("lda", c_int), ("ldw", c_int), ("ldc", c_int), ("ldr", c_int),
        ("a_bs", c_longlong), ("c_bs", c_longlong), ("r_bs", c_longlong),
        ("gate_bs", c_int), ("act", c_int), ("flags", c_int), ("reserved", c_int),
    ]


class GemmProblem(Structure):
    _fields_ = [("A", c_void_p), ("W", c_void_p), ("bias", c_void_p), ("gate", c_void_p), ("R", c_void_p), ("C", c_void_p), ("d", GemmDesc)]


MAX_GROUPED = 4


class QkvEpilogue(Structure):
    _fields_ = [("wq", c_void_p), ("wk", c_void_p), ("rope", c_void_p), ("reserved", c_void_p), ("eps", c_float), ("qscale", c_float),
                ("heads", c_int), ("rope_row0", c_int)]


class LinearSmallProblem(Structure):
    _fields_ = [("x", c_void_p), ("W", c_void_p), ("bias", c_void_p), ("add", c_void_p), ("y", c_void_p), ("x_rows", c_int), ("add_rows", c_int),
                ("rows", c_int), ("N", c_int), ("K", c_int), ("act_in", c_int), ("act_out", c_int), ("reserved", c_int)]


PRODUCTS_MAX_QUANTILES, PRODUCTS_MAX_THRESHOLDS, PRODUCTS_MAX_MEMBERS, PRODUCTS_MAX_SORT_MEMBERS = 16, 8, 1024, 64


class ProductsDesc(Structure):
    _fields_ = [("n_quant", c_int), ("n_thr", c_int), ("q_lo", c_int * PRODUCTS_MAX_QUANTILES), ("q_t", c_float * PRODUCTS_MAX_QUANTILES),
                ("thr_dir", c_int * PRODUCTS_MAX_THRESHOLDS)]


EVENTS_MAX, EVENTS_MAX_MEMBERS = 32, 1024


class EventsDesc(Structure):
    _fields_ = [("n_events", c_int), ("channel", c_int * EVENTS_MAX), ("dir", c_int * EVENTS_MAX), ("anomaly", c_int * EVENTS_MAX),
                ("thr", c_float * EVENTS_MAX)]


def _load():
    if not os.path.exists(LIB_PATH):
        raise RuntimeError(
            f"{LIB_PATH} is missing: build it with `python -c 'import __graft_entry__ as g; g.build()'` "
            "(or `make -C ladcast_amd/csrc`).  ladcast_amd has no CPU fallback."
        )
    lib = ctypes.CDLL(LIB_PATH)
    P, I, L, F, D = c_void_p, c_int, c_longlong, c_float, c_double
    sig = {
        "ldc_abi_version": (I, []),
        "ldc_build_arch": (c_char_p, []),
        "ldc_sizeof_gemm_desc": (I, []),
        "ldc_gemm_bias_act": (I, [P, P, P, P, P, P, POINTER(GemmDesc), P]),
        "ldc_sizeof_gemm_problem": (I, []),
        "ldc_gemm_grouped_workspace_bytes": (L, []),
        "ldc_gemm_grouped_workspace_init": (I, [P, L, P]),
        "ldc_gemm_grouped": (I, [POINTER(GemmProblem), I, P, L, P]),
        "ldc_gemm_grouped_bf16x3": (I, [POINTER(GemmProblem), I, P, L, P]),
        "ldc_sizeof_qkv_epilogue": (I, []),
        "ldc_gemm_grouped_bf16x3_qkv": (I, [POINTER(GemmProblem), POINTER(QkvEpilogue), I, P, L, P]),
        "ldc_gemm_grouped_qkv_f32": (I, [POINTER(GemmProblem), POINTER(QkvEpilogue), I, P, L, P]),
        "ldc_attn_qkv_prepare_split": (I, [P, P, P, I, I, I, I, L, I, P, P, P, P, P, P, P, P, F, P]),
        "ldc_attn_fwd_split_workspace_bytes": (L, [I, I, I]),
        "ldc_attn_fwd_split_workspace_max_bytes": (L, []),
        "ldc_attn_fwd_split": (I, [P, P, P, P, I, I, I, I, L, I, L, P, I, P, L, P]),
        "ldc_attn_fwd_split_qrows_workspace_bytes": (L, [I, I, I, I]),
        "ldc_attn_fwd_split_qrows": (I, [P, P, P, P, I, I, I, I, I, L, I, L, P, I, P, L, P]),
        "ldc_pack_weight_bf16x2": (I, [P, P, I, I, I, P]),
        "ldc_pack_weight_bf16": (I, [P, P, I, I, I, P]),
        "ldc_linear_small": (I, [P, I, P, P, P, I, P, I, I, I, I, I, P]),
        "ldc_linear_small_grouped": (I, [POINTER(LinearSmallProblem), I, P]),
        "ldc_linear_small_mod": (I, [P, I, P, P, P, I, P, I, P, I, I, I, I, I, P]),
        "ldc_gate_residual_layernorm": (I, [P, P, P, P, I, I, I, I, L, I, L, I, I, L, P, P, F, I, P]),
        "ldc_attn_fwd": (I, [P, P, P, P, I, I, I, I, L, I, L, P, P]),
        "ldc_attn_fwd_ws": (I, [P, P, P, P, I, I, I, I, L, I, L, P, P, L, P]),
        "ldc_attn_fwd_qrows": (I, [P, P, P, P, I, I, I, I, I, L, I, L, P, P]),
        "ldc_attn_fwd_ws_qrows": (I, [P, P, P, P, I, I, I, I, I, L, I, L, P, P, L, P]),
        "ldc_attn_fwd_workspace_bytes": (L, []),
        "ldc_qk_rmsnorm_rope": (I, [P, P, I, I, I, I, I, L, P, P, F, P, P, P]),
        "ldc_sphere_conv_nhwc_split": (I, [P, P, P, P, P, I, I, I, I, I, I, I, I, I, I, I, I, P, L, P]),
        "ldc_sphere_conv_plan": (I, [I, I, I, I, I, I, I, P, P]),
        "ldc_rmsnorm_rows_split": (I, [P, P, P, P, P, P, L, I, I, I, I, I, I, F, I, P]),
        "ldc_pixel_unshuffle_shortcut_split": (I, [P, P, P, P, I, I, I, I, I, I, I, P]),
        "ldc_pixel_shuffle_shortcut_split": (I, [P, P, P, P, I, I, I, I, I, I, I, P]),
        "ldc_pixel_shuffle_to_chan": (I, [P, P, I, I, I, I, I, P]),
        "ldc_split_rows": (I, [P, P, L, I, I, I, I, P]),
        "ldc_upsample_nearest2x_rows": (I, [P, P, P, I, I, I, I, I, I, I, I, P]),
        "ldc_sphere_dwconv_nhwc_fmt": (I, [P, P, P, P, I, I, I, I, I, I, I, I, I, P]),
        "ldc_relu_linear_attn_nhwc_fmt": (I, [P, P, I, I, I, I, I, F, I, P, L, P]),
        "ldc_ensemble_scores_workspace_bytes": (L, [I, I, I]),
        "ldc_ensemble_scores": (I, [P, L, L, P, L, P, L, P, I, I, I, I, I, P, P, P, P, L, P]),
        "ldc_rollout_scores_workspace_bytes": (L, [I, I, I, I]),
        "ldc_rollout_scores": (I, [P, L, L, L, P, P, F, P, L, L, P, P, L, L, P, P, I, I, I, I, I, I, P, I, I, P, L, P]),
        "ldc_validation_scores_workspace_bytes": (L, [I, I, I, I]),
        "ldc_validation_scores": (I, [P, L, L, L, P, P, F, P, L, L, P, P, I, I, I, I, I, P, I, I, P, L, P]),
        "ldc_rollout_reliability_workspace_bytes": (L, [I, I, I, I, I]),
        "ldc_rollout_reliability": (I, [P, L, L, L, P, P, F, P, L, L, P, P, I, I, I, I, I, I, P, P, P, P, I, I, P, L, P]),
        "ldc_rollout_spectrum_workspace_bytes": (L, [I, I, I, I, I]),
        "ldc_rollout_spectrum": (I, [P, L, L, L, P, P, F, P, L, L, P, P, I, I, I, I, I, P, P, I, I, P, L, P]),
        "ldc_sizeof_products_desc": (I, []),
        "ldc_rollout_products": (I, [P, L, L, L, P, P, F, P, I, I, I, I, I, I, POINTER(ProductsDesc), P, P, P, P, I, I, P]),
        "ldc_sizeof_events_desc": (I, []),
        "ldc_rollout_events_workspace_bytes": (L, [I, I, I, I, I]),
        "ldc_rollout_events": (I, [P, L, L, L, P, P, F, P, L, L, P, P, L, L, P, P, I, I, I, I, I, POINTER(EventsDesc), P, P, P, I, I, P, L, P]),
        "ldc_layernorm_mod": (I, [P, P, I, I, I, I, L, I, L, P, P, I, I, F, I, P]),
        "ldc_layernorm_mod2": (I, [P, P, I, I, I, I, L, I, L, P, P, I, P, P, I, I, F, I, P]),
        "ldc_mean_rows": (I, [P, P, I, I, I, I, L, P]),
        "ldc_mean_rows_split": (I, [P, P, P, I, I, I, I, L, I, L, I, P]),
        "ldc_chan_to_token_split": (I, [P, P, I, I, I, I, I, I, P]),
        "ldc_gate_residual": (I, [P, P, P, P, I, I, I, I, L, I, L, I, P]),
        "ldc_chan_to_token": (I, [P, P, I, I, I, I, I, P]),
        "ldc_token_to_chan": (I, [P, P, I, I, I, I, P]),
        "ldc_timestep_embedding": (I, [P, P, I, P]),
        "ldc_temb_modulate": (I, [P, P, I, I, I, P]),
        "ldc_chan_affine": (I, [P, P, P, P, F, L, I, L, I, P]),
        "ldc_edm_scale_f64_to_f32": (I, [P, D, P, L, P]),
        "ldc_edm_init_state": (I, [P, D, P, L, P]),
        "ldc_edm_euler": (I, [P, P, D, D, D, D, P, P, L, P]),
        "ldc_edm_churn": (I, [P, P, c_double, P, L, P]),
        "ldc_edm_heun": (I, [P, P, P, P, D, D, D, D, L, P]),
        "ldc_f64_to_f32": (I, [P, P, L, P]),
        "ldc_dpm_step": (I, [P, P, P, P, P, F, F, F, F, F, I, L, P]),
        "ldc_ddim_step": (I, [P, P, P, P, P, F, F, F, F, F, F, I, I, L, P]),
        "ldc_ddpm_step": (I, [P, P, P, P, P, F, F, F, F, F, F, I, L, P]),
        "ldc_scale_f32": (I, [P, F, P, L, P]),
        "ldc_axpby_f32": (I, [P, F, P, F, P, L, P]),
        "ldc_edm_noise_inputs": (I, [P, P, P, P, P, P, I, L, P]),
        "ldc_edm_denoise": (I, [P, P, P, P, P, I, I, I, I, I, I, I, P]),
        "ldc_edm_denoise_loss": (I, [P, P, P, P, P, P, P, P, P, I, I, I, I, I, P]),
        "ldc_sphere_conv_nhwc": (I, [P, P, P, P, P, I, I, I, I, I, I, I, I, I, I, P]),
        "ldc_sphere_dwconv_nhwc": (I, [P, P, P, P, I, I, I, I, I, I, I, I, P]),
        "ldc_grouped_conv1x1_nhwc": (I, [P, P, P, L, I, I, I, P]),
        "ldc_relu_linear_attn_nhwc": (I, [P, P, I, I, I, I, I, F, P, L, P]),
        "ldc_relu_linear_attn_workspace_bytes": (L, [I, I, I]),
        "ldc_rmsnorm_rows": (I, [P, P, P, P, P, L, I, I, I, I, F, I, P]),
        "ldc_pixel_unshuffle_shortcut": (I, [P, P, P, I, I, I, I, I, P]),
        "ldc_pixel_shuffle_shortcut": (I, [P, P, P, I, I, I, I, I, P]),
        "ldc_chan_regroup": (I, [P, P, L, I, I, P]),
        "ldc_track_gather": (I, [P, L, L, L, I, I, L, POINTER(c_int), I, P, P, F, P, I, I, P]),
        "ldc_track_nanmean": (I, [P, L, I, L, P, P]),
        "ldc_track_storms": (I, [P, L, L, L, L, P, P, I, P, I, P, P, I, I, POINTER(c_int), I, I, P, P, P, P]),
        "ldc_track_local_min": (I, [P, L, P, P, I, P, I, P, P, P, I, P, P, P, P, P]),
        "ldc_recon_preprocess": (I, [P, L, L, L, I, I, I, I, P, P, I, P, P, P]),
        "ldc_recon_scores_workspace_bytes": (L, [I, I, I, I]),
        "ldc_recon_scores": (I, [P, P, P, L, P, P, P, P, I, I, I, I, I, I, P, P, P, P, L, P]),
        "ldc_field_moments_workspace_bytes": (L, [I, I, I, I]),
        "ldc_field_moments": (I, [P, L, L, L, I, I, I, I, P, I, P, L, P]),
    }
    for name, (res, args) in sig.items():
        fn = getattr(lib, name)
        fn.restype = res
        fn.argtypes = args
    if lib.ldc_abi_version() != ABI_VERSION:
        raise RuntimeError("libladcast_hip.so ABI version mismatch")
    if lib.ldc_sizeof_gemm_desc() != ctypes.sizeof(GemmDesc) or lib.ldc_sizeof_gemm_problem() != ctypes.sizeof(GemmProblem):
        raise RuntimeError("ldc_gemm_desc / ldc_gemm_problem layout mismatch between header and binding")
    if lib.ldc_sizeof_qkv_epilogue() != ctypes.sizeof(QkvEpilogue):
        raise RuntimeError("ldc_qkv_epilogue layout mismatch between header and binding")
    if lib.ldc_sizeof_products_desc() != ctypes.sizeof(ProductsDesc):
        raise RuntimeError("ldc_products_desc layout mismatch between header and binding")
    if lib.ldc_sizeof_events_desc() != ctypes.sizeof(EventsDesc):
        raise RuntimeError("ldc_events_desc layout mismatch between header and binding")
    return lib, sig


lib, SIGNATURES = _load()


def _check(status: int, what: str):
    if status != 0:
        raise RuntimeError(f"{what} failed with status {status}")


def upload_nonblocking(t, device):
    device = torch.device(device)
    if device.type != "cuda" or t.device.type != "cpu":
        return t.to(device)
    return (t if t.is_pinned() else t.pin_memory()).to(device, non_blocking=True)


def _p(t):
    return None if t is None else c_void_p(t.data_ptr())


def _stream():
    return c_void_p(torch.cuda.current_stream().cuda_stream)


def _dev(*ts):
    for t in ts:
        if t is not None and not t.is_cuda:
            raise RuntimeError("ladcast_amd kernels need device tensors (no CPU fallback)")


def gemm(A, W, C, *, M, N, K, batch=1, lda=None, ldw=None, ldc=None, a_bs=0, c_bs=0, bias=None, gate=None,
         gate_bs=0, R=None, ldr=0, r_bs=0, act=ACT_NONE):
    _dev(A, W, C, bias, gate, R)
    d = GemmDesc(M, N, K, batch, lda if lda is not None else K, ldw if ldw is not None else K,
                 ldc if ldc is not None else N, ldr, a_bs, c_bs, r_bs, gate_bs, act, 0, 0)
    _check(lib.ldc_gemm_bias_act(_p(A), _p(W), _p(bias), _p(gate), _p(R), _p(C), ctypes.byref(d), _stream()), "ldc_gemm_bias_act")


_workspaces = {}
_outgrown = []


def _workspace(name, device, nbytes, init=None, grow=False):
    key = (name, str(device), torch.cuda.current_stream(device).cuda_stream)
    ws = _workspaces.get(key)
    if ws is None or (grow and ws.numel() * 4 < nbytes):
        if not grow and torch.cuda.is_current_stream_capturing():
            raise RuntimeError(f"{name}: the first call on a stream must be made outside a graph capture (run one warm-up forward)")
        if ws is not None:
            _outgrown.append(ws)
# ... 669 lines not shown
```

### ladcast_amd/models/LaDCast_3D_model.py

```python
from __future__ import annotations

from types import SimpleNamespace
from typing import Optional, Tuple

import numpy as np
import torch
import torch.nn as nn

from .. import graphs, hip
from .embeddings import get_year_sincos_embedding, rope_tables_from_grid, rotary_1d
from .modeling_utils import ModelMixin


class _RMSNormP(nn.Module):
    def __init__(self, dim, eps):
        super().__init__()
        self.eps = eps
        self.weight = nn.Parameter(torch.ones(dim))

    def forward(self, x):
        var = x.to(torch.float32).pow(2).mean(-1, keepdim=True)
        return x * torch.rsqrt(var + self.eps) * self.weight


# ... 219 lines not shown
        assert sum(conditioning_tensor_rope_axes_dim) == hd
        self.transformer_blocks = nn.ModuleList([_DualBlockP(heads, hd, mlp_ratio) for _ in range(num_layers)])
        self.single_transformer_blocks = nn.ModuleList([_SingleBlockP(heads, hd, mlp_ratio) for _ in range(num_single_layers)])
        self.norm_out = _AdaLinearP(d, 2 * d)
        self.proj_out = nn.Linear(d, self._patch_vol * out_channels)
        self.requires_grad_(False)
        self.scale_attn_by_lat = bool(scale_attn_by_lat)
        self.attn_lat_weights = None
        if scale_attn_by_lat:
            w = np.cos(np.deg2rad(np.linspace(-83.25, 84.75, 15)))
            w = w / w.mean()
            self.attn_lat_weights = torch.from_numpy(w / w.sum()).float().repeat_interleave(30).view(1, 1, 1, -1)
        self._kbias = {}
        self._plan = None
        self._plan_gen = 0
        self._ws = {}
        self._rope = {}
        self._te_cache = None
        self._te_buf = {}
        self._graphs = {}
        self._capture_stream = None
        self.use_hip_graph = False
        self.gemm_precision = "fp32"

    def enable_hip_graph(self, flag: bool = True):
        if flag and self._foreign_processors():
            raise NotImplementedError("hipGraph capture is for the built-in attention path; a user-supplied attention processor runs eagerly")
        self.use_hip_graph = bool(flag)
        if not flag:
            self._drop_graphs()
        return self

    def _drop_graphs(self):
        self._graphs = {}

    def _drop_plan(self, device_caches=False):
        self._plan = None
        self._drop_graphs()
        if device_caches:
            self._ws, self._rope, self._te_buf, self._kbias = {}, {}, {}, {}
            self._te_cache = None

    def set_attn_lat_weights(self, weights: torch.Tensor):
        self.attn_lat_weights = weights.detach().float().reshape(1, 1, 1, -1).cpu()
        self._kbias = {}
        self._drop_graphs()
        return self

    def _key_bias(self, frames, dev):
        if not self.scale_attn_by_lat:
            return None
        key = (frames, str(dev))
        if key not in self._kbias:
            self._kbias[key] = hip.pad_key_bias(self.attn_lat_weights.reshape(-1).repeat(frames).to(dev))
        return self._kbias[key]

    def set_gemm_precision(self, mode: str):
        if mode not in ("fp32", "bf16x3", "bf16"):
            raise ValueError("gemm precision must be 'fp32', 'bf16x3' or 'bf16'")
        if mode != self.gemm_precision:
            self.gemm_precision = mode
            self._drop_plan()
        return self

    @property
    def attn_processors(self):
        out = {}
        for name, mod in self.named_modules():
            if isinstance(mod, _AttentionP):
                out[f"{name}.processor"] = mod.get_processor()
        return out

    def set_attn_processor(self, processor):
        mods = {f"{n}.processor": m for n, m in self.named_modules() if isinstance(m, _AttentionP)}
        if isinstance(processor, dict):
            if len(processor) != len(mods):
                raise ValueError(
                    f"A dict of processors was passed, but the number of processors {len(processor)} does not match the"
                    f" number of attention layers: {len(mods)}. Please make sure to pass {len(mods)} processor classes."
                )
            for k, m in mods.items():
                m.set_processor(processor[k])
        else:
            for m in mods.values():
                m.set_processor(processor)
        if self._foreign_processors():
            if self.use_hip_graph:
                self.enable_hip_graph(False)
            self._drop_graphs()

    def _foreign_processors(self):
        return [m for m in self.modules() if isinstance(m, _AttentionP) and m.foreign_processor is not None]

    def _call_processor(self, attn, hidden_states, encoder_hidden_states, attention_mask, image_rotary_emb, cond_image_rotary_emb):
        import inspect

        proc = attn.foreign_processor
        kw = dict(encoder_hidden_states=encoder_hidden_states, attention_mask=attention_mask, image_rotary_emb=image_rotary_emb,
                  cond_image_rotary_emb=cond_image_rotary_emb)
        params = inspect.signature(proc.__call__).parameters
        if not any(p.kind is inspect.Parameter.VAR_KEYWORD for p in params.values()):
            kw = {k: v for k, v in kw.items() if k in params}
        out = proc(attn, hidden_states, **kw)
        if not (isinstance(out, tuple) and len(out) == 2):
            raise TypeError("an attention processor must return (hidden_states, encoder_hidden_states) (models/LaDCast_3D_model.py:78-86,221)")
        return out

    def _apply(self, fn, *a, **k):
        self._drop_plan(device_caches=True)
        return super()._apply(fn, *a, **k)

    def load_state_dict(self, *a, **k):
        self._drop_plan()
        return super().load_state_dict(*a, **k)

    @staticmethod
    def _fuse_qkv(q, k, v):
        return (
            torch.cat([q.weight, k.weight, v.weight], dim=0).contiguous(),
            torch.cat([q.bias, k.bias, v.bias], dim=0).contiguous(),
        )

    def _build_plan(self):
        self._upcast_to_fp32()
        if not next(self.parameters()).is_cuda:
            raise RuntimeError("LaDCastTransformer3DModel must live on a HIP device (no CPU fallback)")
        plan = SimpleNamespace(attn={})
        for name, mod in self.named_modules():
            if isinstance(mod, _AttentionP):
                e = SimpleNamespace()
                e.wqkv, e.bqkv = self._fuse_qkv(mod.to_q, mod.to_k, mod.to_v)
                if mod.add_q_proj is not None:
                    e.wqkv_c, e.bqkv_c = self._fuse_qkv(mod.add_q_proj, mod.add_k_proj, mod.add_v_proj)
                plan.attn[id(mod)] = e
        d = self.inner_dim
        plan.wx = self.x_embedder.proj.weight.reshape(d, -1).contiguous()
        plan.wc = self.context_embedder.proj.weight.reshape(d, -1).contiguous()
        kq = 64 if self.gemm_precision == "bf16" else 32
        plan.kx_pad = -(-plan.wx.shape[1] // kq) * kq
        plan.kc_pad = -(-plan.wc.shape[1] // kq) * kq
        mods = []
        for blk in self.transformer_blocks:
            mods += [blk.norm1.linear, blk.norm1_context.linear]
        mods += [blk.norm.linear for blk in self.single_transformer_blocks]
        mods.append(self.norm_out.linear)
        plan.mod_w = torch.cat([m.weight for m in mods], dim=0).contiguous()
        plan.mod_b = torch.cat([m.bias for m in mods], dim=0).contiguous()
        plan.mod_off, off = {}, 0
        for m in mods:
            plan.mod_off[id(m)] = off
            off += m.weight.shape[0]
        plan.split = self.gemm_precision in ("bf16x3", "bf16")
        plan.one_term = self.gemm_precision == "bf16"
        plan.packed = {}
        if plan.split:
            ws = [e.wqkv for e in plan.attn.values()] + [e.wqkv_c for e in plan.attn.values() if hasattr(e, "wqkv_c")]
            ws.append(self.context_refiner.proj_in.weight)
            ws.append(self.proj_out.weight)
            for blk in self.context_refiner.token_refiner.refiner_blocks:
                ws += [blk.ff.net[0].proj.weight, blk.ff.net[2].weight]
            for blk in self.transformer_blocks:
                ws += [blk.attn.to_out[0].weight, blk.attn.to_add_out.weight, blk.ff.net[0].proj.weight, blk.ff.net[2].weight,
                       blk.ff_context.net[0].proj.weight, blk.ff_context.net[2].weight]
            for blk in self.single_transformer_blocks:
                ws += [blk.proj_mlp.weight, blk.proj_out.weight]
            pack = hip.pack_weight_bf16 if plan.one_term else hip.pack_weight_bf16x2
            for w in ws:
                plan.packed[id(w)] = pack(w)
            for w, kp in ((plan.wx, plan.kx_pad), (plan.wc, plan.kc_pad)):
                wp = torch.zeros(w.shape[0], kp, device=w.device, dtype=w.dtype)
                wp[:, : w.shape[1]] = w
                plan.packed[id(w)] = pack(wp)
        self._plan = plan
        self._plan_gen += 1

    def _patches(self, x):
        p, pt = self.config.patch_size, self.config.patch_size_t
        if p == 1 and pt == 1:
            return x
        B, C, T, H, W = x.shape
        if T % pt or H % p or W % p:
            raise ValueError(f"a (T, H, W) = {(T, H, W)} tensor is not a whole number of ({pt}, {p}, {p}) patches")
        return x.reshape(B, C, T // pt, pt, H // p, p, W // p, p).permute(0, 1, 3, 5, 7, 2, 4, 6).reshape(B, C * pt * p * p, T // pt, H // p, W // p).contiguous()

    def _unpatch(self, y, C_out):
        p, pt = self.config.patch_size, self.config.patch_size_t
        if p == 1 and pt == 1:
            return y
        B, _, T, H, W = y.shape
        return y.reshape(B, C_out, pt, p, p, T, H, W).permute(0, 1, 5, 2, 6, 3, 7, 4).reshape(B, C_out, T * pt, H * p, W * p).contiguous()

    def _rope_tables(self, r, t_in, h, w, dev):
        key = (r, t_in, h, w, str(dev))
        if key not in self._rope:
            c = self.config
            cond_t = torch.arange(-t_in + 1, 1, dtype=torch.float32)
            pred_t = torch.arange(1, r + 1, dtype=torch.float32)
            lat = torch.linspace(self.rope_spatial_grid_start_pos[0], self.rope_spatial_grid_end_pos[0], steps=h, dtype=torch.float32)
            lon = torch.linspace(self.rope_spatial_grid_start_pos[1], self.rope_spatial_grid_end_pos[1], steps=w, dtype=torch.float32)
            if getattr(c, "nope", False):
                n = h * w
                pc, ps = (t.repeat_interleave(n, dim=0).contiguous() for t in rotary_1d(c.attention_head_dim, pred_t, c.rope_theta))
                cc, cs = (t.repeat_interleave(n, dim=0).contiguous() for t in rotary_1d(c.attention_head_dim, cond_t, c.rope_theta))
            else:
                pc, ps = rope_tables_from_grid(c.rope_axes_dim, [pred_t, lat, lon], c.rope_theta)
                cc, cs = rope_tables_from_grid(c.conditioning_tensor_rope_axes_dim, [cond_t, lat, lon], c.rope_theta)
            pc, ps, cc, cs = (t.to(dev) for t in (pc, ps, cc, cs))
            pk, ck = hip.compact_rope_table(pc, ps), hip.compact_rope_table(cc, cs)
            jk = torch.cat([pk, ck], dim=0).contiguous()
            self._rope[key] = (pc, ps, cc, cs, pk, ck, jk)
        return self._rope[key]

    def _time_elapsed_embedding(self, time_elapsed, dev):
        key = (time_elapsed.data_ptr(), time_elapsed._version, tuple(time_elapsed.shape), str(time_elapsed.device))
        if self._te_cache is not None and self._te_cache[0] == key:
            return self._te_cache[1]
        stamps = getattr(time_elapsed, "host_values", None)
        if stamps is None or len(stamps) != time_elapsed.numel():
            stamps = time_elapsed.reshape(-1).tolist()
        stamps = [int(v) for v in stamps]
        n, d2 = len(stamps), 2 * self.inner_dim
        emb = get_year_sincos_embedding(stamps, 256)
        emb = hip.upload_nonblocking(emb, dev)
        te = self.time_elapsed_embed
        if n not in self._te_buf:
            self._te_buf[n] = (torch.empty(n, d2, device=dev, dtype=torch.float32), torch.empty(n, d2, device=dev, dtype=torch.float32))
        mid, out = self._te_buf[n]
        hip.linear_small(emb, te.linear_1.weight, mid, rows=n, N=d2, K=256, bias=te.linear_1.bias, act_out=hip.ACT_SILU)
        hip.linear_small(mid, te.linear_2.weight, out, rows=n, N=d2, K=d2, bias=te.linear_2.bias)
        self._te_cache = (key, out, time_elapsed)
        return out

    def _timestep_mlps(self, timestep, Bt, pooled, B, ws):
        D = self.inner_dim
        r, m = self.context_refiner.time_text_embed, self.time_text_embed
        P = hip.linear_small_problem
        TS = hip.ACT_IN_TIMESTEP_SINCOS
        hip.linear_small_grouped([
            P(timestep, r.timestep_embedder.linear_1.weight, ws.t1, rows=Bt, N=D, K=256, bias=r.timestep_embedder.linear_1.bias, act_in=TS, act_out=hip.ACT_SILU),
            P(timestep, m.timestep_embedder.linear_1.weight, ws.t1m, rows=Bt, N=D, K=256, bias=m.timestep_embedder.linear_1.bias, act_in=TS, act_out=hip.ACT_SILU),
            P(pooled, r.text_embedder.linear_1.weight, ws.p1, rows=B, N=D, K=D, bias=r.text_embedder.linear_1.bias, act_out=hip.ACT_SILU),
        ])
        hip.linear_small_grouped([
            P(ws.t1, r.timestep_embedder.linear_2.weight, ws.t2, rows=Bt, N=D, K=D, bias=r.timestep_embedder.linear_2.bias),
            P(ws.t1m, m.timestep_embedder.linear_2.weight, ws.t2m, rows=Bt, N=D, K=D, bias=m.timestep_embedder.linear_2.bias),
        ])
        tx = r.text_embedder
        hip.linear_small(ws.p1, tx.linear_2.weight, ws.temb_r, rows=B, N=D, K=D, bias=tx.linear_2.bias, add=ws.t2, add_rows=Bt)

    def _text_mlp(self, emb, pooled, B, Bt, t2, ws, out, te=None):
        D = self.inner_dim
        tx = emb.text_embedder
        hip.linear_small(pooled, tx.linear_1.weight, ws.p1, rows=B, N=D, K=D, bias=tx.linear_1.bias, act_out=hip.ACT_SILU)
        hip.linear_small(ws.p1, tx.linear_2.weight, out, rows=B, N=D, K=D, bias=tx.linear_2.bias, add=t2, add_rows=Bt, mod=te,
                         mod_rows=1 if te is None else te.shape[0])

    def _attention(self, ws, B, row0, Sx, Sc, out, ldo, o_bs, seg_x, seg_c, out_split=False, key_bias=None, normed=False, Sq=None):
        D, H = self.inner_dim, self.config.num_attention_heads
        qkv = ws.qkv
        full = qkv.shape[1]
        S = Sx + Sc
        q = qkv[:, row0:, 0:D]
        k = qkv[:, row0:, D : 2 * D]
        v = qkv[:, row0:, 2 * D : 3 * D]
        if self.gemm_precision in ("bf16x3", "bf16"):
            hip.attn_fwd_split(q, k, v, out, B=B, S=S, H=H, ld_qkv=3 * D, qkv_bs=full * 3 * D, ldo=ldo, o_bs=o_bs, out_split=out_split,
                               one_term=self.gemm_precision == "bf16", key_bias=key_bias, Sq=Sq)
            return
        segs = [] if normed else [sg for sg in ((Sx, seg_x), (Sc, seg_c)) if sg[0] > 0]
        r0 = row0
        for rows, (nq, nk, c, s_) in segs:
            hip.qk_rmsnorm_rope(qkv[:, :, 0:D], qkv[:, :, D : 2 * D], B=B, row0=r0, rows=rows, H=H, ld=3 * D, bs=full * 3 * D,
                                wq=nq.weight, wk=nk.weight, eps=nq.eps, cos=c, sin=s_)
            r0 += rows
        hip.attn_fwd(q, k, v, out, B=B, S=S, H=H, ld_qkv=3 * D, qkv_bs=full * 3 * D, ldo=ldo, o_bs=o_bs, key_bias=key_bias, Sq=Sq)

    def _qkv_epi(self, norm_q, norm_k, rope):
        if norm_q.eps != norm_k.eps:
            raise NotImplementedError("the fused QKV epilogue takes one RMSNorm eps for q and k")
        return hip.qkv_epilogue(norm_q.weight, norm_k.weight, rope, eps=norm_q.eps, heads=self.config.num_attention_heads,
                                qscale=0.0 if self.gemm_precision in ("bf16x3", "bf16") else 1.0)

    @torch.no_grad()
    def forward(
        self,
        hidden_states: torch.Tensor,
        timestep: torch.Tensor,
        conditioning_tensors: torch.Tensor,
        time_elapsed: Optional[torch.Tensor] = None,
        attention_kwargs=None,
        return_dict: bool = True,
        coords=None,
        conditioning=None,
    ):
        if self._plan is None:
            self._build_plan()
        plan = self._plan
        dev = self.device
        cfg = self.config
        D, H = self.inner_dim, cfg.num_attention_heads
        B, C_in, R, Hh, Ww = hidden_states.shape
        T_in = conditioning_tensors.shape[2]
        Cc = conditioning_tensors.shape[1]
        Nx, Nc = R * Hh * Ww, T_in * Hh * Ww
        S = Nx + Nc
        C_out = cfg.out_channels or cfg.in_channels
        hidden_states = hidden_states.to(device=dev, dtype=torch.float32).contiguous()
        conditioning_tensors = conditioning_tensors.to(device=dev, dtype=torch.float32)
        if conditioning_tensors.shape[0] != B:
            conditioning_tensors = conditioning_tensors.expand(B, -1, -1, -1, -1)
        conditioning_tensors = conditioning_tensors.contiguous()
        timestep = timestep.to(device=dev, dtype=torch.float32).reshape(-1).contiguous()
        Bt = timestep.shape[0]
        if Bt not in (1, B):
            raise ValueError(f"timestep must have 1 or {B} entries, got {Bt}")
        te = None
        if time_elapsed is not None and self.time_elapsed_embed is not None:
            te = self._time_elapsed_embedding(time_elapsed, dev)
            if te.shape[0] not in (1, B):
                raise ValueError("time_elapsed must have 1 or batch entries")

        if conditioning is not None:
            pack, idx = conditioning
            if tuple(pack.shape) != (B,) + tuple(conditioning_tensors.shape[1:]) or not 0 <= idx < pack.levels:
                raise ValueError("`conditioning` was prepared for another batch / conditioning shape")
            out = self._main_device(hidden_states, pack, idx)
            return (out,) if not return_dict else SimpleNamespace(sample=out)
        if self.use_hip_graph:
            gkey = (B, Bt, C_in, R, T_in, Hh, Ww, None if te is None else (te.data_ptr(), te.shape[0]), bool(self.skip_unread_rows))
            inputs = [hidden_states, timestep, conditioning_tensors]
            ent = self._graphs.get(gkey)
            if ent is None:
                ent = self._graphs[gkey] = graphs.capture(lambda x, t, k: self._forward_device(x, t, k, te), inputs, dev, self.capture_stream())
            out = ent.replay(*inputs)
        else:
            out = self._forward_device(hidden_states, timestep, conditioning_tensors, te)
        if not return_dict:
            return (out,)
        return SimpleNamespace(sample=out)

    def time_elapsed_embedding(self, time_elapsed):
        if time_elapsed is None or self.time_elapsed_embed is None:
            return None
        if self._plan is None:
            self._build_plan()
        return self._time_elapsed_embedding(time_elapsed, self.device)

    def plan_identity(self):
        if self._plan is None:
            self._build_plan()
        return self._plan_gen

    def capture_stream(self):
        if self._capture_stream is None:
            self._capture_stream = torch.cuda.Stream(device=self.device)
        return self._capture_stream

    @torch.no_grad()
    def forward_launch_only(self, hidden_states, timestep, conditioning_tensors, te, conditioning=None):
        if self._plan is None:
            self._build_plan()
        if hidden_states.dtype != torch.float32 or not hidden_states.is_cuda or not hidden_states.is_contiguous():
            raise TypeError("forward_launch_only takes a contiguous fp32 device tensor (use forward() for anything else)")
        if conditioning is not None:
            return self._main_device(hidden_states, conditioning[0], conditioning[1])
        return self._forward_device(hidden_states, timestep.reshape(-1), conditioning_tensors, te)

    batch_conditioning = True
    skip_unread_rows = True
    COND_MAX_ROWS = 96

    @torch.no_grad()
    def prepare_conditioning(self, timesteps, conditioning_tensors, te=None):
        if self._plan is None:
            self._build_plan()
        dev = self.device
        timesteps = timesteps.to(device=dev, dtype=torch.float32).reshape(-1)
        conditioning_tensors = conditioning_tensors.to(device=dev, dtype=torch.float32)
        if conditioning_tensors.dim() != 5:
            raise ValueError("conditioning_tensors must be (B, C, T_in, h, w)")
        N, B = timesteps.shape[0], conditioning_tensors.shape[0]
        shape = tuple(conditioning_tensors.shape)
        per = max(1, self.COND_MAX_ROWS // B)
        if per >= N:
            pk = self._conditioning_device(timesteps.repeat_interleave(B).contiguous(),
                                           conditioning_tensors.unsqueeze(0).expand(N, *shape).reshape(N * B, *shape[1:]).contiguous(), te)
            return SimpleNamespace(ctx=pk.ctx, mods=pk.mods, shape=shape, levels=N)
        Nc, D, NM = shape[2] * shape[3] * shape[4] // self._patch_vol, self.inner_dim, self._plan.mod_w.shape[0]
        key = ("pack", N, B, Nc)
        if key not in self._ws:
            self._ws[key] = (torch.empty(N * B, Nc, D, device=dev, dtype=torch.float32), torch.empty(N * B, NM, device=dev, dtype=torch.float32))
        ctx, mods = self._ws[key]
        for n0 in range(0, N, per):
            n = min(per, N - n0)
            pk = self._conditioning_device(timesteps[n0 : n0 + n].repeat_interleave(B).contiguous(),
                                           conditioning_tensors.unsqueeze(0).expand(n, *shape).reshape(n * B, *shape[1:]).contiguous(), te)
            ctx[n0 * B : (n0 + n) * B].copy_(pk.ctx)
            mods[n0 * B : (n0 + n) * B].copy_(pk.mods)
        return SimpleNamespace(ctx=ctx, mods=mods, shape=shape, levels=N)

    @staticmethod
    def _launchers(plan):
        split, packed = plan.split, plan.packed
        AS = (hip.GEMM_A_SPLIT | (hip.GEMM_BF16_1TERM if plan.one_term else 0)) if split else 0
        CS = hip.GEMM_C_SPLIT if split else 0
        fmt = hip.FMT_BF16 if plan.one_term else hip.FMT_SPLIT if split else hip.FMT_F32

        def G(A, W, C, **kw):
            return hip.gemm_problem(A, packed[id(W)] if split else W, C, **kw)

        def run(problems):
            hip.gemm_grouped(problems, split_bf16=split)

        def run1(A, W, C, **kw):
            hip.gemm_grouped([G(A, W, C, **kw)], split_bf16=split)

        def run_qkv(problems, epis):
            if split:
                hip.gemm_grouped_qkv(problems, epis)
                return True
            if hip.gemm_grouped_qkv_f32(problems, epis):
                return True
            hip.gemm_grouped(problems, split_bf16=False)
            return False

        return AS, CS, fmt, G, run, run1, run_qkv

    def _forward_device(self, hidden_states, timestep, conditioning_tensors, te):
        pack = self._conditioning_device(timestep, conditioning_tensors, te)
        return self._main_device(hidden_states, SimpleNamespace(ctx=pack.ctx, mods=pack.mods, shape=tuple(conditioning_tensors.shape), levels=1), 0)

    def _conditioning_device(self, timestep, conditioning_tensors, te):
        plan = self._plan
        dev = self.device
        cfg = self.config
        D, H = self.inner_dim, cfg.num_attention_heads
        conditioning_tensors = self._patches(conditioning_tensors)
        B, Cc, T_in, Hh, Ww = conditioning_tensors.shape
        Nx, Nc = 0, T_in * Hh * Ww
        S = Nc
        Bt = timestep.shape[0]
        kpad = max(plan.kx_pad, plan.kc_pad)
        key = ("cond", B, Bt, Nc, kpad)
        if key not in self._ws:
            self._ws[key] = _Workspace(dev, B, Bt, 0, Nc, D, kpad, 4, plan.mod_w.shape[0])
        ws = self._ws[key]
        _, _, cc, cs, _, ck, _ = self._rope_tables(1, T_in, Hh, Ww, dev)
        SD = S * D
        h_c, nh_c = ws.h, ws.nh
        split = plan.split

        AS, CS, fmt, G, run, run1, run_qkv = self._launchers(plan)

        if split:
            KC = plan.kc_pad
            ctok = ws.ctok.view(-1)[: B * Nc * KC].view(B, Nc, KC)
            hip.chan_to_token(conditioning_tensors, ctok, B=B, C=Cc, N=Nc, ldo=KC, fill_cols=KC, out_split=fmt)
            run1(ctok, plan.wc, ws.ctx0, M=Nc, N=D, K=KC, batch=B, a_bs=Nc * KC, c_bs=Nc * D, bias=self.context_embedder.proj.bias, flags=AS)
        else:
            hip.chan_to_token(conditioning_tensors, ws.ctok.view(-1)[: B * Nc * Cc].view(B, Nc, Cc), B=B, C=Cc, N=Nc, ldo=Cc)
            hip.gemm(ws.ctok, plan.wc, ws.ctx0, M=Nc, N=D, K=Cc, batch=B, a_bs=Nc * Cc, c_bs=Nc * D, bias=self.context_embedder.proj.bias)

        kb_cond = None
        if self.scale_attn_by_lat:
            if Hh * Ww != self.attn_lat_weights.numel():
                raise ValueError("scale_attn_by_lat is hard-wired to the 15 x 30 latent grid (models/LaDCast_3D_model.py:684-692)")
            kb_cond = self._key_bias(T_in, dev)
        foreign = bool(self._foreign_processors())
        m_cond = None
        if foreign:
            if split:
                raise NotImplementedError("a user-supplied attention processor runs on the fp32 path: call set_gemm_precision('fp32') "
                                          "(or change the attention arithmetic through the C ABI, include/ladcast_hip.h)")
            if torch.cuda.is_current_stream_capturing():
                raise NotImplementedError("a user-supplied attention processor cannot be captured into a hipGraph")
            if self.scale_attn_by_lat:
                w = self.attn_lat_weights.to(dev)
                m_cond = w.repeat(1, 1, 1, T_in)

        ref = self.context_refiner
        if split:
            hip.mean_rows(ws.ctx0, ws.pooled, B=B, rows=Nc, D=D, ldx=D, x_bs=Nc * D, x_split=nh_c, lds=D, s_bs=SD, fmt=fmt)
        else:
            hip.mean_rows(ws.ctx0, ws.pooled, B=B, rows=Nc, D=D, ldx=D, x_bs=Nc * D)
        self._timestep_mlps(timestep, Bt, ws.pooled, B, ws)
        if split:
            run1(nh_c, ref.proj_in.weight, h_c, M=Nc, N=D, K=D, batch=B, a_bs=SD, c_bs=SD, bias=ref.proj_in.bias, flags=AS)
        else:
            run1(ws.ctx0, ref.proj_in.weight, h_c, M=Nc, N=D, K=D, batch=B, a_bs=Nc * D, c_bs=SD, bias=ref.proj_in.bias)
        for blk in ref.token_refiner.refiner_blocks:
            pa = plan.attn[id(blk.attn)]
            hip.layernorm_mod(h_c, nh_c, B=B, rows=Nc, D=D, ldx=D, x_bs=SD, ldy=D, y_bs=SD, scale=blk.norm1.weight, shift=blk.norm1.bias, mode=1, eps=blk.norm1.eps, out_split=fmt)
            if blk.attn.foreign_processor is not None:
                a, _ = self._call_processor(blk.attn, nh_c, None, m_cond, (cc, cs), None)
                ws.att.copy_(a)
            else:
                nd = run_qkv([G(nh_c, pa.wqkv, ws.qkv, M=Nc, N=3 * D, K=D, batch=B, a_bs=SD, c_bs=S * 3 * D, bias=pa.bqkv, flags=AS)],
                             [self._qkv_epi(blk.attn.norm_q, blk.attn.norm_k, ck)])
                self._attention(ws, B, Nx, Nc, 0, ws.att, D, SD, (blk.attn.norm_q, blk.attn.norm_k, cc, cs), None, key_bias=kb_cond, normed=nd)
            hip.linear_small(ws.temb_r, blk.norm_out.linear.weight, ws.mod_a, rows=B, N=2 * D, K=D, bias=blk.norm_out.linear.bias, act_in=hip.ACT_SILU)
            hip.gate_residual_layernorm(h_c, ws.att, ws.mod_a, nh_c, B=B, rows=Nc, D=D, ld_res=D, res_bs=SD, ld_y=D, y_bs=SD, gate_bs=2 * D,
                                        ld_out=D, out_bs=SD, weight=blk.norm2.weight, bias=blk.norm2.bias, eps=blk.norm2.eps, out_split=fmt)
            f0, f2 = blk.ff.net[0].proj, blk.ff.net[2]
            F = f0.weight.shape[0]
            run1(nh_c, f0.weight, ws.cat, M=Nc, N=F, K=D, batch=B, a_bs=SD, c_bs=Nc * F, bias=f0.bias, act=hip.ACT_SILU, flags=AS | CS)
            run1(ws.cat, f2.weight, h_c, M=Nc, N=D, K=F, batch=B, a_bs=Nc * F, c_bs=SD, bias=f2.bias,
                        gate=ws.mod_a[:, D:], gate_bs=2 * D, R=h_c, ldr=D, r_bs=SD, flags=AS)

        hip.mean_rows(h_c, ws.pooled, B=B, rows=Nc, D=D, ldx=D, x_bs=SD)
        self._text_mlp(self.time_text_embed, ws.pooled, B, Bt, ws.t2m, ws, ws.temb, te=te)
        NM = plan.mod_w.shape[0]
        hip.linear_small(ws.temb, plan.mod_w, ws.mods, rows=B, N=NM, K=D, bias=plan.mod_b, act_in=hip.ACT_SILU)

        return SimpleNamespace(ctx=ws.h, mods=ws.mods, rows=B, shape=(B, Cc, T_in, Hh, Ww))

    def _main_device(self, hidden_states, pack, idx):
        plan = self._plan
        dev = self.device
        cfg = self.config
        D, H = self.inner_dim, cfg.num_attention_heads
        hidden_states = self._patches(hidden_states)
        B, C_in, R, Hh, Ww = hidden_states.shape
        T_in = pack.shape[2] // cfg.patch_size_t
        Nx, Nc = R * Hh * Ww, T_in * Hh * Ww
        S = Nx + Nc
        C_out = (cfg.out_channels or cfg.in_channels) * self._patch_vol
        kpad = max(plan.kx_pad, plan.kc_pad)
        key = (B, Nx, Nc, kpad)
        if key not in self._ws:
            self._ws[key] = _Workspace(dev, B, 1, Nx, Nc, D, kpad, C_out, 4)
        ws = self._ws[key]
        pc, ps, cc, cs, pk, ck, jk = self._rope_tables(R, T_in, Hh, Ww, dev)
        SD = S * D
        h_x, h_c = ws.h[:, :Nx], ws.h[:, Nx:]
        nh_x, nh_c = ws.nh[:, :Nx], ws.nh[:, Nx:]
        NM = plan.mod_w.shape[0]
        mods = pack.mods[idx * B : (idx + 1) * B]
        split = plan.split

        AS, CS, fmt, G, run, run1, run_qkv = self._launchers(plan)

        if split:
            KX = plan.kx_pad
            xtok = ws.xtok.view(-1)[: B * Nx * KX].view(B, Nx, KX)
            hip.chan_to_token(hidden_states, xtok, B=B, C=C_in, N=Nx, ldo=KX, fill_cols=KX, out_split=fmt)
            run1(xtok, plan.wx, h_x, M=Nx, N=D, K=KX, batch=B, a_bs=Nx * KX, c_bs=SD, bias=self.x_embedder.proj.bias, flags=AS)
        else:
            hip.chan_to_token(hidden_states, ws.xtok.view(-1)[: B * Nx * C_in].view(B, Nx, C_in), B=B, C=C_in, N=Nx, ldo=C_in)
            hip.gemm(ws.xtok, plan.wx, h_x, M=Nx, N=D, K=C_in, batch=B, a_bs=Nx * C_in, c_bs=SD, bias=self.x_embedder.proj.bias)
        h_c.copy_(pack.ctx[idx * B : (idx + 1) * B])

        kb_all = None
        if self.scale_attn_by_lat:
            if Hh * Ww != self.attn_lat_weights.numel():
                raise ValueError("scale_attn_by_lat is hard-wired to the 15 x 30 latent grid (models/LaDCast_3D_model.py:684-692)")
            kb_all = self._key_bias(R + T_in, dev)
        foreign = bool(self._foreign_processors())
        m_all = None
        if foreign:
            if split:
                raise NotImplementedError("a user-supplied attention processor runs on the fp32 path: call set_gemm_precision('fp32') "
# ... 80 lines not shown
```

Before: 3.221.

## Skip padded MFMA slabs in ragged last row tile and cost-weight stream-K cut

For the f32 GEMM path with 128-row tiles, the last partial row tile now runs specialized k-step loops that only compute the 16-row slabs actually present (1-7), using a transposed accumulator layout fixed up through shared memory before the epilogue. The stream-K split across workgroups is also reweighted with per-k-step cost estimates so ragged tiles, which are cheaper, receive proportionally more units. The aim is to stop spending MFMA and LDS work on padded rows and to balance the load across CUs. In exchange the kernel gains code size and register pressure, an extra transpose with barriers, and hand-tuned cost constants that may not match real timings.

```diff
diff --git a/include/ladcast_hip.h b/include/ladcast_hip.h
--- a/include/ladcast_hip.h
+++ b/include/ladcast_hip.h
@@ -31,6 +31,8 @@
 #define LDC_GEMM_C_SPLIT 2
 #define LDC_GEMM_BF16_1TERM 4
 #define LDC_GEMM_F32_REGSTAGE 8
+#define LDC_GEMM_F32_RAGGED_LEGACY 16
+#define LDC_GEMM_F32_RAGGED_UNIT_CUT 32
 #define LDC_FMT_F32 0
 #define LDC_FMT_SPLIT 1
 #define LDC_FMT_BF16 2
@@ -106,6 +108,7 @@
                                 long long workspace_bytes, void* stream);
 int ldc_gemm_grouped_qkv_f32(const ldc_gemm_problem* problems, const ldc_qkv_epilogue* epi, int n, void* workspace,
                              long long workspace_bytes, void* stream);
+int ldc_gemm_f32_ring_cut(const ldc_gemm_desc* descs, int n, unsigned* starts, int starts_len, long long* run_units, int* run_cost);
 int ldc_attn_qkv_prepare_split(float* Q, float* K, float* V, int B, int S, int H, int ld_qkv, long long qkv_bs, int split_row,
                                const float* wq0, const float* wk0, const float* cos0, const float* sin0, const float* wq1,
                                const float* wk1, const float* cos1, const float* sin1, float eps, void* stream);
diff --git a/ladcast_amd/csrc/gemm_bf16x3_v3.hip b/ladcast_amd/csrc/gemm_bf16x3_v3.hip
--- a/ladcast_amd/csrc/gemm_bf16x3_v3.hip
+++ b/ladcast_amd/csrc/gemm_bf16x3_v3.hip
@@ -8,6 +8,11 @@
 
 #include "gemm_v3_common.inc"
 #include "gemm_v3_kstep_f32.inc"
+
+constexpr int MAX_RANGES = 256;
+
+constexpr int WHOLE_KSTEP_COST = 64;
+constexpr int RAGGED_KSTEP_COST[8] = {0, 18, 22, 29, 37, 45, 52, 60};
 
 struct SKArgs {
   DevProblem pr[MAXP];
@@ -18,11 +23,23 @@
   float* ws;
   unsigned* counters;
   unsigned upg, urem;
+  int ragged_cols;
+  int weighted;
+  unsigned starts[MAX_RANGES + 1];
 };
 
+template <bool WEIGHTED = false>
 __device__ __forceinline__ long long range_start(long long g, const SKArgs& a) {
   const unsigned gu = static_cast<unsigned>(g);
+  if constexpr (WEIGHTED) {
+    if (a.weighted) return static_cast<long long>(a.starts[gu]);
+  }
   return static_cast<long long>(gu * a.upg + (gu < a.urem ? gu : a.urem));
+}
+
+inline long long range_start_host(long long g, const SKArgs& a) {
+  if (a.weighted) return static_cast<long long>(a.starts[g]);
+  return g * a.upg + (g < a.urem ? g : a.urem);
 }
 
 __device__ __forceinline__ int find_problem_by_unit(const SKArgs& a, long long u) {
@@ -55,6 +72,7 @@
   constexpr int NAI = BM / 64;
   constexpr int ND = NAI + 2;
   constexpr int NDH = ND / 2;
+  constexpr bool RAGGED = BM == 128 && TERMS == 0 && !CONV;
   extern __shared__ __attribute__((aligned(16))) unsigned char smem[];
   const int wave = __builtin_amdgcn_readfirstlane(static_cast<int>(threadIdx.x) >> 6);
   LDC_STAMP(0)
@@ -71,8 +89,8 @@
     const unsigned hi = __builtin_amdgcn_readfirstlane(static_cast<unsigned>(static_cast<unsigned long long>(v) >> 32));
     return static_cast<long long>((static_cast<unsigned long long>(hi) << 32) | lo);
   };
-  const long long u_begin = uniform64(range_start(g, a));
-  const long long u_end = uniform64(range_start(g + 1, a));
+  const long long u_begin = uniform64(range_start<RAGGED>(g, a));
+  const long long u_end = uniform64(range_start<RAGGED>(g + 1, a));
   const unsigned smem_lds = lds_addr(smem);
 
   struct Seg {
@@ -87,13 +105,24 @@
     sg.k0 = static_cast<int>(local - static_cast<unsigned>(sg.tile) * kt_u);
     const long long left = u_end - u_;
     sg.k1 = (Q.kt - sg.k0 <= left) ? Q.kt : sg.k0 + static_cast<int>(left);
-    const unsigned per_b = static_cast<unsigned>(Q.tm * Q.tn), tile_u = static_cast<unsigned>(sg.tile);
+    if constexpr (RAGGED) {
+      if (sg.tile >= Q.wt) {
+        const unsigned t_ = static_cast<unsigned>(sg.tile - Q.wt), tn_ = static_cast<unsigned>(Q.tn);
+        const unsigned b_ = t_ / tn_;
+        sg.b = __builtin_amdgcn_readfirstlane(static_cast<int>(b_));
+        sg.bn = __builtin_amdgcn_readfirstlane(static_cast<int>(t_ - b_ * tn_));
+        sg.bm = __builtin_amdgcn_readfirstlane(Q.tm - 1);
+        return sg;
+      }
+    }
+    const int tm_ = RAGGED ? Q.tmw : Q.tm;
+    const unsigned per_b = static_cast<unsigned>(tm_ * Q.tn), tile_u = static_cast<unsigned>(sg.tile);
     const unsigned b_ = tile_u / per_b;
     const unsigned t_in = tile_u - b_ * per_b;
     const unsigned strip = static_cast<unsigned>(Q.rm * Q.tn);
     const unsigned sr = t_in / strip;
     const unsigned r_in = t_in - sr * strip;
-    const int rest = Q.tm - static_cast<int>(sr) * Q.rm;
+    const int rest = tm_ - static_cast<int>(sr) * Q.rm;
     const unsigned h_sr = static_cast<unsigned>(rest < Q.rm ? rest : Q.rm);
     const unsigned bn_ = r_in / h_sr;
     sg.b = __builtin_amdgcn_readfirstlane(static_cast<int>(b_));
@@ -152,6 +181,9 @@
     const unsigned w_lo = smem_lds + BM * ROW_B + off_lo;
     const int M = P.d.M, N = P.d.N, K = P.d.K;
     const bool wave_rows = bm * BM + 16 * RT * wave < M;
+    const int rs = (RAGGED && a.ragged_cols && bm == P.tm - 1) ? P.rs : 0;
+    const unsigned ra_hi = smem_lds + off_hi, ra_lo = smem_lds + off_lo;
+    const unsigned rw_hi = w_hi + (16 * wave) * ROW_B, rw_lo = w_lo + (16 * wave) * ROW_B;
     const float* __restrict__ A = P.A + static_cast<long long>(b) * P.d.a_bs;
     const int lda = P.d.lda;
     const long long w_row_bytes = static_cast<long long>(K) * (TERMS == 1 ? 2 : 4);
@@ -225,6 +257,7 @@
 
     i32x4v wh0, wl0, wh1, wl1, wh2, wl2, wh3, wl3;
     i32x4v ah0[RT], al0[RT], ah1[RT], al1[RT];
+    i32x4v rx0, rx1, rx2, rx3;
 
 #define LDC_SB __builtin_amdgcn_sched_barrier(0)
 #define LDC_RD_W(WH, WL, SBH, SBL, CT)                                           \
@@ -389,7 +422,9 @@
     LDC_STAMP(1 + 4 * seg_)
     if (seg_ == 0) { LDC_STAMP_CLK(13) }
     if constexpr (PAIRED) {
-      LDC_KSTEP_Q_PROLOGUE(ah0, al0)
+      if (rs == 0) {
+        LDC_KSTEP_Q_PROLOGUE(ah0, al0)
+      }
     } else {
       LDC_RD_A(ah0, al0, a_hi, a_lo)
       LDC_RD_W(wh0, wl0, w_hi, w_lo, 0)
@@ -405,7 +440,27 @@
     int st = 0;
     if constexpr (PAIRED) {
       static_assert(!PAIRED || ND == 4, "the interleaved k-step is written for the 128-row tile's 4 DMA pieces");
-      if (wave_rows) {
+      if constexpr (RAGGED) {
+        if (rs != 0) {
+#define LDC_RAGGED_LOOP(S) \
+  case S:                  \
+    for (int kt = k0; kt < k1; ++kt) LDC_KSTEP_R##S break;
+          switch (rs) {
+            LDC_RAGGED_LOOP(1)
+            LDC_RAGGED_LOOP(2)
+            LDC_RAGGED_LOOP(3)
+            LDC_RAGGED_LOOP(4)
+            LDC_RAGGED_LOOP(5)
+            LDC_RAGGED_LOOP(6)
+            default:
+              for (int kt = k0; kt < k1; ++kt) LDC_KSTEP_R7
+              break;
+          }
+#undef LDC_RAGGED_LOOP
+        }
+      }
+      if (rs != 0) {
+      } else if (wave_rows) {
         for (int kt = k0; kt < k1; ++kt) {
           LDC_KSTEP_Q(ah0, al0, ah1, al1, LDC_MM_ON)
           ++kt;
@@ -431,6 +486,7 @@
     asm volatile("s_waitcnt lgkmcnt(0)" : "+v"(wh0), "+v"(wl0), "+v"(wh1), "+v"(wl1), "+v"(wh2), "+v"(wl2), "+v"(wh3), "+v"(wl3));
 #pragma unroll
     for (int rt = 0; rt < RT; ++rt) asm volatile("" : "+v"(ah0[rt]), "+v"(al0[rt]), "+v"(ah1[rt]), "+v"(al1[rt]));
+    (void)rx0; (void)rx1; (void)rx2; (void)rx3; (void)ra_hi; (void)ra_lo; (void)rw_hi; (void)rw_lo;
 #undef LDC_KSTEP
 #undef LDC_MM_ON
 #undef LDC_MM_OFF
@@ -455,23 +511,50 @@
     LDC_STAMP(2 + 4 * seg_)
 
     if (k0 == 0 && k1 == P.kt) {
+      if constexpr (RAGGED) {
+        if (rs != 0) {
+          float* tr = reinterpret_cast<float*>(smem + 2 * STAGE_B);
+          const int lane_t = fresh_lane();
+          static_assert(8 * 7 * 2 * 64 * 4 <= STAGE_B, "the transposition buffer is one ring stage");
+#pragma unroll
+          for (int p = 0; p < 2; ++p) {
+#pragma unroll
+            for (int j = 0; j < 7; ++j)
+              if (j < rs) {
+                tr[((wave * 7 + j) * 2 + 0) * 64 + lane_t] = acc[j][2 * p];
+                tr[((wave * 7 + j) * 2 + 1) * 64 + lane_t] = acc[j][2 * p + 1];
+              }
+            __syncthreads();
+#pragma unroll
+            for (int ct = 0; ct < 8; ++ct) {
+              const float v0 = wave < rs ? tr[((ct * 7 + wave) * 2 + 0) * 64 + lane_t] : 0.f;
+              const float v1 = wave < rs ? tr[((ct * 7 + wave) * 2 + 1) * 64 + lane_t] : 0.f;
+              acc[ct][2 * p] = v0;
+              acc[ct][2 * p + 1] = v1;
+            }
+            __syncthreads();
+          }
+        }
+      }
       tile_epilogue<BM, !CONV, LinearRows<BM>, true, TERMS == 0>(P, b, bm, bn, acc, wave, lane);
     } else {
       const int lane_h = fresh_lane();
       float* slot = a.ws + (static_cast<long long>(2 * g) + (k0 > 0 ? 0 : 1)) * SLOT_FLOATS + lane_h;
 #pragma unroll
       for (int i = 0; i < NACC; ++i)
-#pragma unroll
-        for (int r = 0; r < 4; ++r)
-          __hip_atomic_store(slot + ((wave * NACC + i) * 4 + r) * 64, acc[i][r], __ATOMIC_RELAXED, __HIP_MEMORY_SCOPE_AGENT);
+        if (rs == 0 || i < rs) {
+#pragma unroll
+          for (int r = 0; r < 4; ++r)
+            __hip_atomic_store(slot + ((wave * NACC + i) * 4 + r) * 64, acc[i][r], __ATOMIC_RELAXED, __HIP_MEMORY_SCOPE_AGENT);
+        }
       asm volatile("s_waitcnt vmcnt(0)" ::: "memory");
       __builtin_amdgcn_s_barrier();
       const long long f = P.unit0 + static_cast<long long>(tile) * P.kt;
       const long long l = f + P.kt;
       long long g_first = g;
-      while (g_first > 0 && range_start(g_first, a) > f) --g_first;
+      while (g_first > 0 && range_start<RAGGED>(g_first, a) > f) --g_first;
       long long g_last = g;
-      while (g_last + 1 < a.G && range_start(g_last + 1, a) < l) ++g_last;
+      while (g_last + 1 < a.G && range_start<RAGGED>(g_last + 1, a) < l) ++g_last;
       const unsigned pieces = static_cast<unsigned>(g_last - g_first + 1);
       unsigned* cnt = a.counters + (P.tile0 + tile);
       unsigned* flag = reinterpret_cast<unsigned*>(smem + NSTAGE * STAGE_B);
@@ -493,8 +576,18 @@
 #pragma unroll
         for (int i = 0; i < NACC; ++i) acc[i] = f32x4{0.f, 0.f, 0.f, 0.f};
         for (long long gp = g_first; gp <= g_last; ++gp) {
-          const long long s = range_start(gp, a);
+          const long long s = range_start<RAGGED>(gp, a);
           const float* sl = a.ws + (2 * gp + (s > f ? 0 : 1)) * SLOT_FLOATS;
+          if (rs != 0) {
+            if (wave < rs) {
+#pragma unroll
+              for (int i = 0; i < NACC; ++i) {
+#pragma unroll
+                for (int r = 0; r < 4; ++r) acc[i][r] += sl[((i * NACC + wave) * 4 + r) * 64 + lane_h];
+              }
+            }
+            continue;
+          }
 #pragma unroll
           for (int i = 0; i < NACC; ++i) {
 #pragma unroll
@@ -522,7 +615,9 @@
 
 template <int BM, int TERMS, bool CONV = false>
 int launch_v3(const ldc_gemm_problem* problems, const ldc_qkv_epilogue* epi, int n, void* workspace, long long workspace_bytes,
-              void* stream, const ConvParams* cp = nullptr, bool may_split_group = false) {
+              void* stream, const ConvParams* cp = nullptr, bool may_split_group = false, SKArgs* dry = nullptr) {
+  constexpr bool RAGGED = BM == 128 && TERMS == 0 && !CONV;
+  int ragged_flags = 0;
   constexpr int SLOT_FLOATS = BM * BN;
   constexpr int STAGE_B = (BM + BN) * ROW_B;
   constexpr int CUS = 256;
@@ -538,7 +633,9 @@
     if (d.M <= 0 || d.N <= 0 || d.K <= 0 || d.batch <= 0) return LDC_ERR_ARG;
     if (d.K % (TERMS == 1 ? 2 * BK : BK)) return LDC_ERR_UNSUPPORTED;
     if constexpr (TERMS == 0) {
-      if (d.flags != 0 || d.ldw != d.K) return LDC_ERR_UNSUPPORTED;
+      constexpr int allowed = RAGGED ? (LDC_GEMM_F32_RAGGED_LEGACY | LDC_GEMM_F32_RAGGED_UNIT_CUT) : 0;
+      if ((d.flags & ~allowed) != 0 || d.ldw != d.K) return LDC_ERR_UNSUPPORTED;
+      ragged_flags |= d.flags;
     } else {
       if (!(d.flags & LDC_GEMM_A_SPLIT)) return LDC_ERR_UNSUPPORTED;
     }
@@ -615,12 +712,24 @@
       }
     }
     const long long t = static_cast<long long>(d.batch) * P.tm * P.tn;
+    P.wt = t > 0x7fffffffLL ? 0x7fffffff : static_cast<int>(t);
+    P.tmw = P.tm;
+    P.rs = 0;
+    if constexpr (RAGGED) {
+      const int slabs = ldc_cdiv(d.M - (P.tm - 1) * BM, 16);
+      if (slabs < 8 && !(ragged_flags & LDC_GEMM_F32_RAGGED_LEGACY)) P.rs = slabs;
+    }
     tiles += t;
     U += t * P.kt;
+  }
+  if constexpr (RAGGED) {
+    if (ragged_flags & LDC_GEMM_F32_RAGGED_LEGACY)
+      for (int i = 0; i < n; ++i) a.pr[i].rs = 0;
   }
   if (tiles > LDC_GEMM_COUNTER_BYTES / 4 - 16) return LDC_ERR_UNSUPPORTED;
   const long long slot_bytes = SLOT_FLOATS * static_cast<long long>(sizeof(float));
   long long G = CUS;
+  bool aligned_cut = false;
   {
     bool same_kt = true;
     for (int i = 1; i < n; ++i) same_kt = same_kt && (a.pr[i].kt == a.pr[0].kt);
@@ -652,7 +761,9 @@
     if (may_split_group && TERMS != 0 && n > 1 && best < 160 && few == 0) return LDC_SPLIT_GROUP;
     if (best >= 160) {
       G = best;
+      aligned_cut = true;
     } else if (few > 0) {
+      aligned_cut = true;
       G = few;
     } else {
       const double kt_avg = static_cast<double>(U) / static_cast<double>(tiles);
@@ -663,12 +774,18 @@
     }
   }
   if constexpr (TERMS == 0) {
-    if (U >= 4 * CUS) G = CUS;
+    if (U >= 4 * CUS) {
+      G = CUS;
+      aligned_cut = false;
+    }
   }
   static const char* const force_g = LDC_AB_GETENV("LDC_BF16X3_G");
   if (force_g) {
     const long long g_ = atoll(force_g);
-    if (g_ > 0 && g_ <= CUS) G = g_;
+    if (g_ > 0 && g_ <= CUS) {
+      G = g_;
+      aligned_cut = false;
+    }
   }
   if (U < G) G = U;
   if (workspace == nullptr) return LDC_ERR_ARG;
@@ -691,6 +808,57 @@
   a.U = U;
   a.upg = static_cast<unsigned>(U / G);
   a.urem = static_cast<unsigned>(U % G);
+  if constexpr (RAGGED) {
+    bool any = false;
+    for (int i = 0; i < n; ++i) any = any || a.pr[i].rs != 0;
+    a.ragged_cols = any ? 1 : 0;
+    if (any && !aligned_cut && !(ragged_flags & LDC_GEMM_F32_RAGGED_UNIT_CUT) && G <= MAX_RANGES) {
+      long long run_units[2 * MAXP], run_cost[2 * MAXP], total = 0;
+      for (int i = 0; i < n; ++i) {
+        DevProblem& P = a.pr[i];
+        if (P.rs != 0) {
+          P.tmw = P.tm - 1;
+          P.wt = P.d.batch * P.tmw * P.tn;
+          if (P.tmw > 0 && P.rm > P.tmw) P.rm = P.tmw;
+        }
+        const long long all = static_cast<long long>(P.d.batch) * P.tm * P.tn;
+        const long long whole = P.rs != 0 ? P.wt : all;
+        run_units[2 * i] = whole * P.kt;
+        run_cost[2 * i] = WHOLE_KSTEP_COST;
+        run_units[2 * i + 1] = (all - whole) * P.kt;
+        run_cost[2 * i + 1] = RAGGED_KSTEP_COST[P.rs];
+        total += run_units[2 * i] * run_cost[2 * i] + run_units[2 * i + 1] * run_cost[2 * i + 1];
+      }
+      int r = 0;
+      long long r_u0 = 0, r_c0 = 0;
+      a.starts[0] = 0;
+      for (long long g_ = 1; g_ < G; ++g_) {
+        const long long num = g_ * total;
+        while (r < 2 * n - 1 && (r_c0 + run_units[r] * run_cost[r]) * G <= num) {
+          r_c0 += run_units[r] * run_cost[r];
+          r_u0 += run_units[r];
+          ++r;
+        }
+        long long in_run = 0;
+        if (run_units[r] > 0) {
+          const long long den = G * run_cost[r];
+          in_run = (2 * (num - r_c0 * G) + den) / (2 * den);
+          if (in_run < 0) in_run = 0;
+          if (in_run > run_units[r]) in_run = run_units[r];
+        }
+        long long st_ = r_u0 + in_run;
+        if (st_ < static_cast<long long>(a.starts[g_ - 1]) + 1) st_ = static_cast<long long>(a.starts[g_ - 1]) + 1;
+        if (st_ > U - (G - g_)) st_ = U - (G - g_);
+        a.starts[g_] = static_cast<unsigned>(st_);
+      }
+      a.starts[G] = static_cast<unsigned>(U);
+      a.weighted = 1;
+    }
+  }
+  if (dry) {
+    *dry = a;
+    return LDC_OK;
+  }
   a.tiles = tiles;
   a.ws = reinterpret_cast<float*>(static_cast<unsigned char*>(workspace) + LDC_GEMM_COUNTER_BYTES);
   a.counters = static_cast<unsigned*>(workspace);
@@ -762,6 +930,35 @@
   if (force_bm && atoi(force_bm) == 256) return launch_v3<256, 0>(problems, epi, n, workspace, workspace_bytes, stream);
 #endif
   return launch_v3<128, 0>(problems, epi, n, workspace, workspace_bytes, stream);
+}
+
+extern "C" int ldc_gemm_f32_ring_cut(const ldc_gemm_desc* descs, int n, unsigned* starts, int starts_len, long long* run_units, int* run_cost) {
+  LDC_CHECK_PTR(descs);
+  LDC_CHECK_PTR(starts);
+  LDC_CHECK_PTR(run_units);
+  LDC_CHECK_PTR(run_cost);
+  if (n <= 0 || n > MAXP || starts_len < MAX_RANGES + 1) return LDC_ERR_ARG;
+  ldc_gemm_problem pr[MAXP] = {};
+  float* const fake = reinterpret_cast<float*>(static_cast<unsigned long long>(1) << 20);
+  for (int i = 0; i < n; ++i) {
+    pr[i].A = pr[i].W = fake;
+    pr[i].C = fake;
+    pr[i].d = descs[i];
+  }
+  static SKArgs a;
+  const int st = launch_v3<128, 0>(pr, nullptr, n, fake, 1ll << 40, nullptr, nullptr, false, &a);
+  if (st != LDC_OK) return st;
+  for (int g = 0; g <= a.G; ++g) starts[g] = static_cast<unsigned>(range_start_host(g, a));
+  for (int i = 0; i < n; ++i) {
+    const DevProblem& P = a.pr[i];
+    const long long all = static_cast<long long>(P.d.batch) * P.tm * P.tn;
+    const long long whole = a.weighted && P.rs != 0 ? P.wt : (P.rs != 0 ? all - static_cast<long long>(P.d.batch) * P.tn : all);
+    run_units[2 * i] = whole * P.kt;
+    run_cost[2 * i] = WHOLE_KSTEP_COST;
+    run_units[2 * i + 1] = (all - whole) * P.kt;
+    run_cost[2 * i + 1] = P.rs != 0 ? RAGGED_KSTEP_COST[P.rs] : WHOLE_KSTEP_COST;
+  }
+  return a.G;
 }
 
 int ldc_gemm_grouped_f32_ring(const ldc_gemm_problem* problems, int n, void* workspace, long long workspace_bytes, void* stream) {
diff --git a/ladcast_amd/csrc/gemm_streamk.hip b/ladcast_amd/csrc/gemm_streamk.hip
--- a/ladcast_amd/csrc/gemm_streamk.hip
+++ b/ladcast_amd/csrc/gemm_streamk.hip
@@ -449,7 +449,7 @@
     if ((d.K & 3) || (d.lda & 3) || (d.a_bs & 3)) return LDC_ERR_ALIGN;
     if (split_bf16 ? (d.K & 7) != 0 : (d.ldw & 3) != 0) return LDC_ERR_ALIGN;
     if (d.act < LDC_ACT_NONE || d.act > LDC_ACT_RELU) return LDC_ERR_UNSUPPORTED;
-    if ((d.flags & ~LDC_GEMM_F32_REGSTAGE) != 0) return LDC_ERR_UNSUPPORTED;
+    if ((d.flags & ~(LDC_GEMM_F32_REGSTAGE | LDC_GEMM_F32_RAGGED_LEGACY | LDC_GEMM_F32_RAGGED_UNIT_CUT)) != 0) return LDC_ERR_UNSUPPORTED;
     DevProblem& P = a.pr[i];
     P.A = q.A;
     P.W = q.W;
diff --git a/ladcast_amd/csrc/gemm_v3_common.inc b/ladcast_amd/csrc/gemm_v3_common.inc
--- a/ladcast_amd/csrc/gemm_v3_common.inc
+++ b/ladcast_amd/csrc/gemm_v3_common.inc
@@ -22,6 +22,9 @@
   ldc_gemm_desc d;
   int tm, tn, kt;
   int rm;
+  int wt;
+  int tmw;
+  int rs;
   long long unit0;
   long long tile0;
   int vec4;
diff --git a/ladcast_amd/csrc/gemm_v3_kstep_f32.inc b/ladcast_amd/csrc/gemm_v3_kstep_f32.inc
--- a/ladcast_amd/csrc/gemm_v3_kstep_f32.inc
+++ b/ladcast_amd/csrc/gemm_v3_kstep_f32.inc
@@ -139,3 +139,469 @@
     LDC_DS_READ(wh2, w_hi, 2 * (16 * ROW_B)); \
     LDC_DS_READ(wh3, w_hi, 3 * (16 * ROW_B)); \
   }
+#define LDC_KSTEP_R1 \
+  { \
+    const int st1 = st == NSTAGE - 1 ? 0 : st + 1; \
+    const int st2 = st1 == NSTAGE - 1 ? 0 : st1 + 1; \
+    const unsigned sb1 = st1 * STAGE_B; \
+    const unsigned rwh = rw_hi + sb, rwl = rw_lo + sb, rah = ra_hi + sb, ral = ra_lo + sb; \
+    LDC_DS_READ(wh0, rwh, 0); \
+    LDC_DS_READ(wl0, rwl, 0); \
+    LDC_DS_READ(ah0[0], rah, 0 * (16 * ROW_B)); \
+    LDC_DS_READ(al0[0], ral, 0 * (16 * ROW_B)); \
+    LDC_SB; \
+    issue_one(kt + 2, st2, NDH + 0); \
+    issue_one(kt + 2, st2, NDH + 1); \
+    LDC_SB; \
+    asm volatile("s_waitcnt lgkmcnt(0)" : "+v"(wh0), "+v"(wl0), "+v"(ah0[0]), "+v"(al0[0])); \
+    LDC_SB; \
+    LDC_MMF(acc[0], wh0, ah0[0], 0) \
+    LDC_MMF(acc[0], wh0, ah0[0], 1) \
+    LDC_MMF(acc[0], wh0, ah0[0], 2) \
+    LDC_MMF(acc[0], wh0, ah0[0], 3) \
+    LDC_MMF(acc[0], wl0, al0[0], 0) \
+    LDC_MMF(acc[0], wl0, al0[0], 1) \
+    LDC_MMF(acc[0], wl0, al0[0], 2) \
+    LDC_MMF(acc[0], wl0, al0[0], 3) \
+     \
+    asm volatile("s_waitcnt vmcnt(4)" ::: "memory"); \
+    LDC_KSTEP_BARRIER \
+    LDC_SB; \
+    issue_one(kt + 3, st, 0); \
+    issue_one(kt + 3, st, 1); \
+    LDC_SB; \
+    st = st1; \
+    sb = sb1; \
+  }
+#define LDC_KSTEP_R2 \
+  { \
+    const int st1 = st == NSTAGE - 1 ? 0 : st + 1; \
+    const int st2 = st1 == NSTAGE - 1 ? 0 : st1 + 1; \
+    const unsigned sb1 = st1 * STAGE_B; \
+    const unsigned rwh = rw_hi + sb, rwl = rw_lo + sb, rah = ra_hi + sb, ral = ra_lo + sb; \
+    LDC_DS_READ(wh0, rwh, 0); \
+    LDC_DS_READ(wl0, rwl, 0); \
+    LDC_DS_READ(ah0[0], rah, 0 * (16 * ROW_B)); \
+    LDC_DS_READ(al0[0], ral, 0 * (16 * ROW_B)); \
+    LDC_DS_READ(ah1[0], rah, 1 * (16 * ROW_B)); \
+    LDC_DS_READ(al1[0], ral, 1 * (16 * ROW_B)); \
+    LDC_SB; \
+    issue_one(kt + 2, st2, NDH + 0); \
+    issue_one(kt + 2, st2, NDH + 1); \
+    LDC_SB; \
+    asm volatile("s_waitcnt lgkmcnt(0)" : "+v"(wh0), "+v"(wl0), "+v"(ah0[0]), "+v"(al0[0]), "+v"(ah1[0]), "+v"(al1[0])); \
+    LDC_SB; \
+    LDC_MMF(acc[0], wh0, ah0[0], 0) \
+    LDC_MMF(acc[1], wh0, ah1[0], 0) \
+    LDC_MMF(acc[0], wh0, ah0[0], 1) \
+    LDC_MMF(acc[1], wh0, ah1[0], 1) \
+    LDC_MMF(acc[0], wh0, ah0[0], 2) \
+    LDC_MMF(acc[1], wh0, ah1[0], 2) \
+    LDC_MMF(acc[0], wh0, ah0[0], 3) \
+    LDC_MMF(acc[1], wh0, ah1[0], 3) \
+    LDC_MMF(acc[0], wl0, al0[0], 0) \
+    LDC_MMF(acc[1], wl0, al1[0], 0) \
+    LDC_MMF(acc[0], wl0, al0[0], 1) \
+    LDC_MMF(acc[1], wl0, al1[0], 1) \
+    LDC_MMF(acc[0], wl0, al0[0], 2) \
+    LDC_MMF(acc[1], wl0, al1[0], 2) \
+    LDC_MMF(acc[0], wl0, al0[0], 3) \
+    LDC_MMF(acc[1], wl0, al1[0], 3) \
+     \
+    asm volatile("s_waitcnt vmcnt(4)" ::: "memory"); \
+    LDC_KSTEP_BARRIER \
+    LDC_SB; \
+    issue_one(kt + 3, st, 0); \
+    issue_one(kt + 3, st, 1); \
+    LDC_SB; \
+    st = st1; \
+    sb = sb1; \
+  }
+#define LDC_KSTEP_R3 \
+  { \
+    const int st1 = st == NSTAGE - 1 ? 0 : st + 1; \
+    const int st2 = st1 == NSTAGE - 1 ? 0 : st1 + 1; \
+    const unsigned sb1 = st1 * STAGE_B; \
+    const unsigned rwh = rw_hi + sb, rwl = rw_lo + sb, rah = ra_hi + sb, ral = ra_lo + sb; \
+    LDC_DS_READ(wh0, rwh, 0); \
+    LDC_DS_READ(wl0, rwl, 0); \
+    LDC_DS_READ(ah0[0], rah, 0 * (16 * ROW_B)); \
+    LDC_DS_READ(al0[0], ral, 0 * (16 * ROW_B)); \
+    LDC_DS_READ(ah1[0], rah, 1 * (16 * ROW_B)); \
+    LDC_DS_READ(al1[0], ral, 1 * (16 * ROW_B)); \
+    LDC_DS_READ(wh1, rah, 2 * (16 * ROW_B)); \
+    LDC_DS_READ(wl1, ral, 2 * (16 * ROW_B)); \
+    LDC_SB; \
+    issue_one(kt + 2, st2, NDH + 0); \
+    issue_one(kt + 2, st2, NDH + 1); \
+    LDC_SB; \
+    asm volatile("s_waitcnt lgkmcnt(2)" : "+v"(wh0), "+v"(wl0), "+v"(ah0[0]), "+v"(al0[0]), "+v"(ah1[0]), "+v"(al1[0])); \
+    LDC_SB; \
+    LDC_MMF(acc[0], wh0, ah0[0], 0) \
+    LDC_MMF(acc[1], wh0, ah1[0], 0) \
+    LDC_MMF(acc[0], wh0, ah0[0], 1) \
+    LDC_MMF(acc[1], wh0, ah1[0], 1) \
+    LDC_MMF(acc[0], wh0, ah0[0], 2) \
+    LDC_MMF(acc[1], wh0, ah1[0], 2) \
+    LDC_MMF(acc[0], wh0, ah0[0], 3) \
+    LDC_MMF(acc[1], wh0, ah1[0], 3) \
+    LDC_MMF(acc[0], wl0, al0[0], 0) \
+    LDC_MMF(acc[1], wl0, al1[0], 0) \
+    LDC_MMF(acc[0], wl0, al0[0], 1) \
+    LDC_MMF(acc[1], wl0, al1[0], 1) \
+    LDC_MMF(acc[0], wl0, al0[0], 2) \
+    LDC_MMF(acc[1], wl0, al1[0], 2) \
+    LDC_MMF(acc[0], wl0, al0[0], 3) \
+    LDC_MMF(acc[1], wl0, al1[0], 3) \
+    asm volatile("s_waitcnt lgkmcnt(0)" : "+v"(wh1), "+v"(wl1)); \
+    LDC_SB; \
+    LDC_MMF(acc[2], wh0, wh1, 0) \
+    LDC_MMF(acc[2], wh0, wh1, 1) \
+    LDC_MMF(acc[2], wh0, wh1, 2) \
+    LDC_MMF(acc[2], wh0, wh1, 3) \
+    LDC_MMF(acc[2], wl0, wl1, 0) \
+    LDC_MMF(acc[2], wl0, wl1, 1) \
+    LDC_MMF(acc[2], wl0, wl1, 2) \
+    LDC_MMF(acc[2], wl0, wl1, 3) \
+     \
+    asm volatile("s_waitcnt vmcnt(4)" ::: "memory"); \
+    LDC_KSTEP_BARRIER \
+    LDC_SB; \
+    issue_one(kt + 3, st, 0); \
+    issue_one(kt + 3, st, 1); \
+    LDC_SB; \
+    st = st1; \
+    sb = sb1; \
+  }
+#define LDC_KSTEP_R4 \
+  { \
+    const int st1 = st == NSTAGE - 1 ? 0 : st + 1; \
+    const int st2 = st1 == NSTAGE - 1 ? 0 : st1 + 1; \
+    const unsigned sb1 = st1 * STAGE_B; \
+    const unsigned rwh = rw_hi + sb, rwl = rw_lo + sb, rah = ra_hi + sb, ral = ra_lo + sb; \
+    LDC_DS_READ(wh0, rwh, 0); \
+    LDC_DS_READ(wl0, rwl, 0); \
+    LDC_DS_READ(ah0[0], rah, 0 * (16 * ROW_B)); \
+    LDC_DS_READ(al0[0], ral, 0 * (16 * ROW_B)); \
+    LDC_DS_READ(ah1[0], rah, 1 * (16 * ROW_B)); \
+    LDC_DS_READ(al1[0], ral, 1 * (16 * ROW_B)); \
+    LDC_DS_READ(wh1, rah, 2 * (16 * ROW_B)); \
+    LDC_DS_READ(wl1, ral, 2 * (16 * ROW_B)); \
+    LDC_DS_READ(wh2, rah, 3 * (16 * ROW_B)); \
+    LDC_DS_READ(wl2, ral, 3 * (16 * ROW_B)); \
+    LDC_SB; \
+    issue_one(kt + 2, st2, NDH + 0); \
+    issue_one(kt + 2, st2, NDH + 1); \
+    LDC_SB; \
+    asm volatile("s_waitcnt lgkmcnt(4)" : "+v"(wh0), "+v"(wl0), "+v"(ah0[0]), "+v"(al0[0]), "+v"(ah1[0]), "+v"(al1[0])); \
+    LDC_SB; \
+    LDC_MMF(acc[0], wh0, ah0[0], 0) \
+    LDC_MMF(acc[1], wh0, ah1[0], 0) \
+    LDC_MMF(acc[0], wh0, ah0[0], 1) \
+    LDC_MMF(acc[1], wh0, ah1[0], 1) \
+    LDC_MMF(acc[0], wh0, ah0[0], 2) \
+    LDC_MMF(acc[1], wh0, ah1[0], 2) \
+    LDC_MMF(acc[0], wh0, ah0[0], 3) \
+    LDC_MMF(acc[1], wh0, ah1[0], 3) \
+    LDC_MMF(acc[0], wl0, al0[0], 0) \
+    LDC_MMF(acc[1], wl0, al1[0], 0) \
+    LDC_MMF(acc[0], wl0, al0[0], 1) \
+    LDC_MMF(acc[1], wl0, al1[0], 1) \
+    LDC_MMF(acc[0], wl0, al0[0], 2) \
+    LDC_MMF(acc[1], wl0, al1[0], 2) \
+    LDC_MMF(acc[0], wl0, al0[0], 3) \
+    LDC_MMF(acc[1], wl0, al1[0], 3) \
+    asm volatile("s_waitcnt lgkmcnt(0)" : "+v"(wh1), "+v"(wl1), "+v"(wh2), "+v"(wl2)); \
+    LDC_SB; \
+    LDC_MMF(acc[2], wh0, wh1, 0) \
+    LDC_MMF(acc[3], wh0, wh2, 0) \
+    LDC_MMF(acc[2], wh0, wh1, 1) \
+    LDC_MMF(acc[3], wh0, wh2, 1) \
+    LDC_MMF(acc[2], wh0, wh1, 2) \
+    LDC_MMF(acc[3], wh0, wh2, 2) \
+    LDC_MMF(acc[2], wh0, wh1, 3) \
+    LDC_MMF(acc[3], wh0, wh2, 3) \
+    LDC_MMF(acc[2], wl0, wl1, 0) \
+    LDC_MMF(acc[3], wl0, wl2, 0) \
+    LDC_MMF(acc[2], wl0, wl1, 1) \
+    LDC_MMF(acc[3], wl0, wl2, 1) \
+    LDC_MMF(acc[2], wl0, wl1, 2) \
+    LDC_MMF(acc[3], wl0, wl2, 2) \
+    LDC_MMF(acc[2], wl0, wl1, 3) \
+    LDC_MMF(acc[3], wl0, wl2, 3) \
+     \
+    asm volatile("s_waitcnt vmcnt(4)" ::: "memory"); \
+    LDC_KSTEP_BARRIER \
+    LDC_SB; \
+    issue_one(kt + 3, st, 0); \
+    issue_one(kt + 3, st, 1); \
+    LDC_SB; \
+    st = st1; \
+    sb = sb1; \
+  }
+#define LDC_KSTEP_R5 \
+  { \
+    const int st1 = st == NSTAGE - 1 ? 0 : st + 1; \
+    const int st2 = st1 == NSTAGE - 1 ? 0 : st1 + 1; \
+    const unsigned sb1 = st1 * STAGE_B; \
+    const unsigned rwh = rw_hi + sb, rwl = rw_lo + sb, rah = ra_hi + sb, ral = ra_lo + sb; \
+    LDC_DS_READ(wh0, rwh, 0); \
+    LDC_DS_READ(wl0, rwl, 0); \
+    LDC_DS_READ(ah0[0], rah, 0 * (16 * ROW_B)); \
+    LDC_DS_READ(al0[0], ral, 0 * (16 * ROW_B)); \
+    LDC_DS_READ(ah1[0], rah, 1 * (16 * ROW_B)); \
+    LDC_DS_READ(al1[0], ral, 1 * (16 * ROW_B)); \
+    LDC_DS_READ(wh1, rah, 2 * (16 * ROW_B)); \
+    LDC_DS_READ(wl1, ral, 2 * (16 * ROW_B)); \
+    LDC_DS_READ(wh2, rah, 3 * (16 * ROW_B)); \
+    LDC_DS_READ(wl2, ral, 3 * (16 * ROW_B)); \
+    LDC_DS_READ(wh3, rah, 4 * (16 * ROW_B)); \
+    LDC_DS_READ(wl3, ral, 4 * (16 * ROW_B)); \
+    LDC_SB; \
+    issue_one(kt + 2, st2, NDH + 0); \
+    issue_one(kt + 2, st2, NDH + 1); \
+    LDC_SB; \
+    asm volatile("s_waitcnt lgkmcnt(6)" : "+v"(wh0), "+v"(wl0), "+v"(ah0[0]), "+v"(al0[0]), "+v"(ah1[0]), "+v"(al1[0])); \
+    LDC_SB; \
+    LDC_MMF(acc[0], wh0, ah0[0], 0) \
+    LDC_MMF(acc[1], wh0, ah1[0], 0) \
+    LDC_MMF(acc[0], wh0, ah0[0], 1) \
+    LDC_MMF(acc[1], wh0, ah1[0], 1) \
+    LDC_MMF(acc[0], wh0, ah0[0], 2) \
+    LDC_MMF(acc[1], wh0, ah1[0], 2) \
+    LDC_MMF(acc[0], wh0, ah0[0], 3) \
+    LDC_MMF(acc[1], wh0, ah1[0], 3) \
+    LDC_MMF(acc[0], wl0, al0[0], 0) \
+    LDC_MMF(acc[1], wl0, al1[0], 0) \
+    LDC_MMF(acc[0], wl0, al0[0], 1) \
+    LDC_MMF(acc[1], wl0, al1[0], 1) \
+    LDC_MMF(acc[0], wl0, al0[0], 2) \
+    LDC_MMF(acc[1], wl0, al1[0], 2) \
+    LDC_MMF(acc[0], wl0, al0[0], 3) \
+    LDC_MMF(acc[1], wl0, al1[0], 3) \
+    asm volatile("s_waitcnt lgkmcnt(2)" : "+v"(wh1), "+v"(wl1), "+v"(wh2), "+v"(wl2)); \
+    LDC_SB; \
+    LDC_MMF(acc[2], wh0, wh1, 0) \
+    LDC_MMF(acc[3], wh0, wh2, 0) \
+    LDC_MMF(acc[2], wh0, wh1, 1) \
+    LDC_MMF(acc[3], wh0, wh2, 1) \
+    LDC_MMF(acc[2], wh0, wh1, 2) \
+    LDC_MMF(acc[3], wh0, wh2, 2) \
+    LDC_MMF(acc[2], wh0, wh1, 3) \
+    LDC_MMF(acc[3], wh0, wh2, 3) \
+    LDC_MMF(acc[2], wl0, wl1, 0) \
+    LDC_MMF(acc[3], wl0, wl2, 0) \
+    LDC_MMF(acc[2], wl0, wl1, 1) \
+    LDC_MMF(acc[3], wl0, wl2, 1) \
+    LDC_MMF(acc[2], wl0, wl1, 2) \
+    LDC_MMF(acc[3], wl0, wl2, 2) \
+    LDC_MMF(acc[2], wl0, wl1, 3) \
+    LDC_MMF(acc[3], wl0, wl2, 3) \
+    asm volatile("s_waitcnt lgkmcnt(0)" : "+v"(wh3), "+v"(wl3)); \
+    LDC_SB; \
+    LDC_MMF(acc[4], wh0, wh3, 0) \
+    LDC_MMF(acc[4], wh0, wh3, 1) \
+    LDC_MMF(acc[4], wh0, wh3, 2) \
+    LDC_MMF(acc[4], wh0, wh3, 3) \
+    LDC_MMF(acc[4], wl0, wl3, 0) \
+    LDC_MMF(acc[4], wl0, wl3, 1) \
+    LDC_MMF(acc[4], wl0, wl3, 2) \
+    LDC_MMF(acc[4], wl0, wl3, 3) \
+     \
+    asm volatile("s_waitcnt vmcnt(4)" ::: "memory"); \
+    LDC_KSTEP_BARRIER \
+    LDC_SB; \
+    issue_one(kt + 3, st, 0); \
+    issue_one(kt + 3, st, 1); \
+    LDC_SB; \
+    st = st1; \
+    sb = sb1; \
+  }
+#define LDC_KSTEP_R6 \
+  { \
+    const int st1 = st == NSTAGE - 1 ? 0 : st + 1; \
+    const int st2 = st1 == NSTAGE - 1 ? 0 : st1 + 1; \
+    const unsigned sb1 = st1 * STAGE_B; \
+    const unsigned rwh = rw_hi + sb, rwl = rw_lo + sb, rah = ra_hi + sb, ral = ra_lo + sb; \
+    LDC_DS_READ(wh0, rwh, 0); \
+    LDC_DS_READ(wl0, rwl, 0); \
+    LDC_DS_READ(ah0[0], rah, 0 * (16 * ROW_B)); \
+    LDC_DS_READ(al0[0], ral, 0 * (16 * ROW_B)); \
+    LDC_DS_READ(ah1[0], rah, 1 * (16 * ROW_B)); \
+    LDC_DS_READ(al1[0], ral, 1 * (16 * ROW_B)); \
+    LDC_DS_READ(wh1, rah, 2 * (16 * ROW_B)); \
+    LDC_DS_READ(wl1, ral, 2 * (16 * ROW_B)); \
+    LDC_DS_READ(wh2, rah, 3 * (16 * ROW_B)); \
+    LDC_DS_READ(wl2, ral, 3 * (16 * ROW_B)); \
+    LDC_DS_READ(wh3, rah, 4 * (16 * ROW_B)); \
+    LDC_DS_READ(wl3, ral, 4 * (16 * ROW_B)); \
+    LDC_DS_READ(rx0, rah, 5 * (16 * ROW_B)); \
+    LDC_DS_READ(rx1, ral, 5 * (16 * ROW_B)); \
+    LDC_SB; \
+    issue_one(kt + 2, st2, NDH + 0); \
+    issue_one(kt + 2, st2, NDH + 1); \
+    LDC_SB; \
+    asm volatile("s_waitcnt lgkmcnt(8)" : "+v"(wh0), "+v"(wl0), "+v"(ah0[0]), "+v"(al0[0]), "+v"(ah1[0]), "+v"(al1[0])); \
+    LDC_SB; \
+    LDC_MMF(acc[0], wh0, ah0[0], 0) \
+    LDC_MMF(acc[1], wh0, ah1[0], 0) \
+    LDC_MMF(acc[0], wh0, ah0[0], 1) \
+    LDC_MMF(acc[1], wh0, ah1[0], 1) \
+    LDC_MMF(acc[0], wh0, ah0[0], 2) \
+    LDC_MMF(acc[1], wh0, ah1[0], 2) \
+    LDC_MMF(acc[0], wh0, ah0[0], 3) \
+    LDC_MMF(acc[1], wh0, ah1[0], 3) \
+    LDC_MMF(acc[0], wl0, al0[0], 0) \
+    LDC_MMF(acc[1], wl0, al1[0], 0) \
+    LDC_MMF(acc[0], wl0, al0[0], 1) \
+    LDC_MMF(acc[1], wl0, al1[0], 1) \
+    LDC_MMF(acc[0], wl0, al0[0], 2) \
+    LDC_MMF(acc[1], wl0, al1[0], 2) \
+    LDC_MMF(acc[0], wl0, al0[0], 3) \
+    LDC_MMF(acc[1], wl0, al1[0], 3) \
+    asm volatile("s_waitcnt lgkmcnt(4)" : "+v"(wh1), "+v"(wl1), "+v"(wh2), "+v"(wl2)); \
+    LDC_SB; \
+    LDC_MMF(acc[2], wh0, wh1, 0) \
+    LDC_MMF(acc[3], wh0, wh2, 0) \
+    LDC_MMF(acc[2], wh0, wh1, 1) \
+    LDC_MMF(acc[3], wh0, wh2, 1) \
+    LDC_MMF(acc[2], wh0, wh1, 2) \
+    LDC_MMF(acc[3], wh0, wh2, 2) \
+    LDC_MMF(acc[2], wh0, wh1, 3) \
+    LDC_MMF(acc[3], wh0, wh2, 3) \
+    LDC_MMF(acc[2], wl0, wl1, 0) \
+    LDC_MMF(acc[3], wl0, wl2, 0) \
+    LDC_MMF(acc[2], wl0, wl1, 1) \
+    LDC_MMF(acc[3], wl0, wl2, 1) \
+    LDC_MMF(acc[2], wl0, wl1, 2) \
+    LDC_MMF(acc[3], wl0, wl2, 2) \
+    LDC_MMF(acc[2], wl0, wl1, 3) \
+    LDC_MMF(acc[3], wl0, wl2, 3) \
+    asm volatile("s_waitcnt lgkmcnt(0)" : "+v"(wh3), "+v"(wl3), "+v"(rx0), "+v"(rx1)); \
+    LDC_SB; \
+    LDC_MMF(acc[4], wh0, wh3, 0) \
+    LDC_MMF(acc[5], wh0, rx0, 0) \
+    LDC_MMF(acc[4], wh0, wh3, 1) \
+    LDC_MMF(acc[5], wh0, rx0, 1) \
+    LDC_MMF(acc[4], wh0, wh3, 2) \
+    LDC_MMF(acc[5], wh0, rx0, 2) \
+    LDC_MMF(acc[4], wh0, wh3, 3) \
+    LDC_MMF(acc[5], wh0, rx0, 3) \
+    LDC_MMF(acc[4], wl0, wl3, 0) \
+    LDC_MMF(acc[5], wl0, rx1, 0) \
+    LDC_MMF(acc[4], wl0, wl3, 1) \
+    LDC_MMF(acc[5], wl0, rx1, 1) \
+    LDC_MMF(acc[4], wl0, wl3, 2) \
+    LDC_MMF(acc[5], wl0, rx1, 2) \
+    LDC_MMF(acc[4], wl0, wl3, 3) \
+    LDC_MMF(acc[5], wl0, rx1, 3) \
+     \
+    asm volatile("s_waitcnt vmcnt(4)" ::: "memory"); \
+    LDC_KSTEP_BARRIER \
+    LDC_SB; \
+    issue_one(kt + 3, st, 0); \
+    issue_one(kt + 3, st, 1); \
+    LDC_SB; \
+    st = st1; \
+    sb = sb1; \
+  }
+#define LDC_KSTEP_R7 \
+  { \
+    const int st1 = st == NSTAGE - 1 ? 0 : st + 1; \
+    const int st2 = st1 == NSTAGE - 1 ? 0 : st1 + 1; \
+    const unsigned sb1 = st1 * STAGE_B; \
+    const unsigned rwh = rw_hi + sb, rwl = rw_lo + sb, rah = ra_hi + sb, ral = ra_lo + sb; \
+    LDC_DS_READ(wh0, rwh, 0); \
+    LDC_DS_READ(wl0, rwl, 0); \
+    LDC_DS_READ(ah0[0], rah, 0 * (16 * ROW_B)); \
+    LDC_DS_READ(al0[0], ral, 0 * (16 * ROW_B)); \
+    LDC_DS_READ(ah1[0], rah, 1 * (16 * ROW_B)); \
+    LDC_DS_READ(al1[0], ral, 1 * (16 * ROW_B)); \
+    LDC_DS_READ(wh1, rah, 2 * (16 * ROW_B)); \
+    LDC_DS_READ(wl1, ral, 2 * (16 * ROW_B)); \
+    LDC_DS_READ(wh2, rah, 3 * (16 * ROW_B)); \
+    LDC_DS_READ(wl2, ral, 3 * (16 * ROW_B)); \
+    LDC_DS_READ(wh3, rah, 4 * (16 * ROW_B)); \
+    LDC_DS_READ(wl3, ral, 4 * (16 * ROW_B)); \
+    LDC_DS_READ(rx0, rah, 5 * (16 * ROW_B)); \
+    LDC_DS_READ(rx1, ral, 5 * (16 * ROW_B)); \
+    LDC_DS_READ(rx2, rah, 6 * (16 * ROW_B)); \
+    LDC_DS_READ(rx3, ral, 6 * (16 * ROW_B)); \
+    LDC_SB; \
+    issue_one(kt + 2, st2, NDH + 0); \
+    issue_one(kt + 2, st2, NDH + 1); \
+    LDC_SB; \
+    asm volatile("s_waitcnt lgkmcnt(10)" : "+v"(wh0), "+v"(wl0), "+v"(ah0[0]), "+v"(al0[0]), "+v"(ah1[0]), "+v"(al1[0])); \
+    LDC_SB; \
+    LDC_MMF(acc[0], wh0, ah0[0], 0) \
+    LDC_MMF(acc[1], wh0, ah1[0], 0) \
+    LDC_MMF(acc[0], wh0, ah0[0], 1) \
+    LDC_MMF(acc[1], wh0, ah1[0], 1) \
+    LDC_MMF(acc[0], wh0, ah0[0], 2) \
+    LDC_MMF(acc[1], wh0, ah1[0], 2) \
+    LDC_MMF(acc[0], wh0, ah0[0], 3) \
+    LDC_MMF(acc[1], wh0, ah1[0], 3) \
+    LDC_MMF(acc[0], wl0, al0[0], 0) \
+    LDC_MMF(acc[1], wl0, al1[0], 0) \
+    LDC_MMF(acc[0], wl0, al0[0], 1) \
+    LDC_MMF(acc[1], wl0, al1[0], 1) \
+    LDC_MMF(acc[0], wl0, al0[0], 2) \
+    LDC_MMF(acc[1], wl0, al1[0], 2) \
+    LDC_MMF(acc[0], wl0, al0[0], 3) \
+    LDC_MMF(acc[1], wl0, al1[0], 3) \
+    asm volatile("s_waitcnt lgkmcnt(6)" : "+v"(wh1), "+v"(wl1), "+v"(wh2), "+v"(wl2)); \
+    LDC_SB; \
+    LDC_MMF(acc[2], wh0, wh1, 0) \
+    LDC_MMF(acc[3], wh0, wh2, 0) \
+    LDC_MMF(acc[2], wh0, wh1, 1) \
+    LDC_MMF(acc[3], wh0, wh2, 1) \
+    LDC_MMF(acc[2], wh0, wh1, 2) \
+    LDC_MMF(acc[3], wh0, wh2, 2) \
+    LDC_MMF(acc[2], wh0, wh1, 3) \
+    LDC_MMF(acc[3], wh0, wh2, 3) \
+    LDC_MMF(acc[2], wl0, wl1, 0) \
+    LDC_MMF(acc[3], wl0, wl2, 0) \
+    LDC_MMF(acc[2], wl0, wl1, 1) \
+    LDC_MMF(acc[3], wl0, wl2, 1) \
+    LDC_MMF(acc[2], wl0, wl1, 2) \
+    LDC_MMF(acc[3], wl0, wl2, 2) \
+    LDC_MMF(acc[2], wl0, wl1, 3) \
+    LDC_MMF(acc[3], wl0, wl2, 3) \
+    asm volatile("s_waitcnt lgkmcnt(2)" : "+v"(wh3), "+v"(wl3), "+v"(rx0), "+v"(rx1)); \
+    LDC_SB; \
+    LDC_MMF(acc[4], wh0, wh3, 0) \
+    LDC_MMF(acc[5], wh0, rx0, 0) \
+    LDC_MMF(acc[4], wh0, wh3, 1) \
+    LDC_MMF(acc[5], wh0, rx0, 1) \
+    LDC_MMF(acc[4], wh0, wh3, 2) \
+    LDC_MMF(acc[5], wh0, rx0, 2) \
+    LDC_MMF(acc[4], wh0, wh3, 3) \
+    LDC_MMF(acc[5], wh0, rx0, 3) \
+    LDC_MMF(acc[4], wl0, wl3, 0) \
+    LDC_MMF(acc[5], wl0, rx1, 0) \
+    LDC_MMF(acc[4], wl0, wl3, 1) \
+    LDC_MMF(acc[5], wl0, rx1, 1) \
+    LDC_MMF(acc[4], wl0, wl3, 2) \
+    LDC_MMF(acc[5], wl0, rx1, 2) \
+    LDC_MMF(acc[4], wl0, wl3, 3) \
+    LDC_MMF(acc[5], wl0, rx1, 3) \
+    asm volatile("s_waitcnt lgkmcnt(0)" : "+v"(rx2), "+v"(rx3)); \
+    LDC_SB; \
+    LDC_MMF(acc[6], wh0, rx2, 0) \
+    LDC_MMF(acc[6], wh0, rx2, 1) \
+    LDC_MMF(acc[6], wh0, rx2, 2) \
+    LDC_MMF(acc[6], wh0, rx2, 3) \
+    LDC_MMF(acc[6], wl0, rx3, 0) \
+    LDC_MMF(acc[6], wl0, rx3, 1) \
+    LDC_MMF(acc[6], wl0, rx3, 2) \
+    LDC_MMF(acc[6], wl0, rx3, 3) \
+     \
+    asm volatile("s_waitcnt vmcnt(4)" ::: "memory"); \
+    LDC_KSTEP_BARRIER \
+    LDC_SB; \
+    issue_one(kt + 3, st, 0); \
+    issue_one(kt + 3, st, 1); \
+    LDC_SB; \
+    st = st1; \
+    sb = sb1; \
+  }
diff --git a/ladcast_amd/hip.py b/ladcast_amd/hip.py
--- a/ladcast_amd/hip.py
+++ b/ladcast_amd/hip.py
@@ -13,6 +13,8 @@
 ACT_IN_TIMESTEP_SINCOS = 16
 GEMM_A_SPLIT, GEMM_C_SPLIT, GEMM_BF16_1TERM = 1, 2, 4
 GEMM_F32_REGSTAGE = 8
+GEMM_F32_RAGGED_LEGACY = 16
+GEMM_F32_RAGGED_UNIT_CUT = 32
 ATTN_OUT_SPLIT, ATTN_BF16_1TERM, ATTN_OUT_BF16 = 1, 2, 4
 ABI_VERSION = 5
 FMT_F32, FMT_SPLIT, FMT_BF16 = 0, 1, 2
@@ -81,6 +83,7 @@
         "ldc_sizeof_qkv_epilogue": (I, []),
         "ldc_gemm_grouped_bf16x3_qkv": (I, [POINTER(GemmProblem), POINTER(QkvEpilogue), I, P, L, P]),
         "ldc_gemm_grouped_qkv_f32": (I, [POINTER(GemmProblem), POINTER(QkvEpilogue), I, P, L, P]),
+        "ldc_gemm_f32_ring_cut": (I, [P, I, P, I, P, P]),
         "ldc_attn_qkv_prepare_split": (I, [P, P, P, I, I, I, I, L, I, P, P, P, P, P, P, P, P, F, P]),
         "ldc_attn_fwd_split_workspace_bytes": (L, [I, I, I]),
         "ldc_attn_fwd_split_workspace_max_bytes": (L, []),
diff --git a/ladcast_amd/models/LaDCast_3D_model.py b/ladcast_amd/models/LaDCast_3D_model.py
--- a/ladcast_amd/models/LaDCast_3D_model.py
+++ b/ladcast_amd/models/LaDCast_3D_model.py
@@ -395,6 +395,7 @@
             off += m.weight.shape[0]
         plan.split = self.gemm_precision in ("bf16x3", "bf16")
         plan.one_term = self.gemm_precision == "bf16"
+        plan.f32_flags = hip.GEMM_F32_RAGGED_LEGACY if self.legacy_ragged_rows else 0
         plan.packed = {}
         if plan.split:
             ws = [e.wqkv for e in plan.attn.values()] + [e.wqkv_c for e in plan.attn.values() if hasattr(e, "wqkv_c")]
@@ -611,6 +612,7 @@
 
     batch_conditioning = True
     skip_unread_rows = True
+    legacy_ragged_rows = False
     COND_MAX_ROWS = 96
 
     @torch.no_grad()
@@ -650,6 +652,8 @@
         fmt = hip.FMT_BF16 if plan.one_term else hip.FMT_SPLIT if split else hip.FMT_F32
 
         def G(A, W, C, **kw):
+            if not split and plan.f32_flags:
+                kw["flags"] = kw.get("flags", 0) | plan.f32_flags
             return hip.gemm_problem(A, packed[id(W)] if split else W, C, **kw)
 
         def run(problems):
```

Result: no change. 3.200 (-0.6%).
